# jinhan/tacotron2-vae

Hardware: AMD Instinct MI355X
Metric: mel-frames/s (train step, batch=6, 80-mel) (higher is better)
Workload: dtype f32; 1 GPU; configs[1]: Tacotron2-VAE fp32 train step (fwd+loss+bwd+clip+Adam), B=6/GPU fixed shape T_in=84 T_out=400, dropout on, random-init seed 1234; step_mode=hip-graph replay, decoder_forward=persistent, decoder_backward=persistent, startup_steps=43, global_batch=6, parallelism=dp1

## Files before the change

include/t2vae.h:

```cpp
#ifndef T2VAE_H
#define T2VAE_H
#include <stdint.h>
#ifdef __cplusplus
extern "C" {
#endif

#define T2V_OK 0
#define T2V_ERR_DIMS -1
#define T2V_ERR_ARG -2
#define T2V_ERR_LAUNCH -3

const char* t2v_version(void);
const char* t2v_last_error(void);

void t2v_set_phase_profile(unsigned long long* dev_buf32);
int t2v_stamp(unsigned long long* dev_buf, int slot, void* stream);
int t2v_debug_spin(int wgs, int microseconds, void* stream);

typedef struct t2v_step_params {
    uint64_t epoch;
    float lr;
    float bc1;
    float bc2s;
    float kl_weight;
// ... 81 lines not shown
    float* GCUM;
    float* DV;
} t2v_dec_bwd_bufs;

int t2v_attn_bwd_slices(int T_in);

int t2v_decoder_train_bwd(const t2v_dec_weights* w, const t2v_dec_train_bufs* s,
                          const t2v_dec_bwd_bufs* g, int B, int T_in, int T_out,
                          float p_att, float p_dec, uint64_t seed, void* stream);

int t2v_decoder_replay_bwd_kernels(const t2v_dec_weights* w, const t2v_dec_train_bufs* s,
                                   const t2v_dec_bwd_bufs* g, int B, int T_in, int T_out,
                                   float p_att, float p_dec, uint64_t seed, int kernel_mask, void* stream);

int t2v_attn_wgrad_scratch_floats(void);
int t2v_attn_wgrad(const float* dpre, const float* al, const float* acum, const float* loc_conv,
                   const float* loc_dense, float* part_scratch, float* d_loc_dense, float* d_loc_conv,
                   int B, int T_in, int T, void* stream);


int t2v_decoder_bwd_persist_supported(int B, int T_in);
long t2v_decoder_bwd_achain_scratch_floats(int B, int T_in, int T_out);
int t2v_decoder_bwd_persist_slices(int T_in);
typedef struct t2v_achain_dw {
    float* planes;
    float* d_w_ih; int ld_ih;
    float* d_w_hh; int ld_hh;
    int accumulate;
    int tile_cap;
} t2v_achain_dw;
long t2v_decoder_bwd_achain_dw_offset(int B, int T_in, int T_out);
int t2v_decoder_bwd_achain(const t2v_dec_train_persist_weights* w, const t2v_achain_dw* dw, const t2v_dec_train_bufs* s,
                           const float* dHC, float* DGA, float* DGD, float* DCTX, float* DV, float* DQP, float* scratch,
                           uint32_t* err_word, int B, int T_in, int T_out, float p_att, float p_dec, uint64_t seed,
                           void* stream);
int t2v_decoder_bwd_persist16_supported(int B, int T_in);
int t2v_decoder_bwd_persist16_slices(int T_in);
int t2v_decoder_bwd_persist16_fits(int B, int T_in, int T_out);
long t2v_decoder_bwd_persist16_scratch_floats(int B, int T_in, int T_out);
long t2v_decoder_bwd_persist16_dq_offset(int B, int T_in, int T_out);
int t2v_decoder_bwd_persistent16(const t2v_dec_train_persist_weights* w, const t2v_dec_train_bufs* s, const float* dHC,
                                 float* DGA, float* DGD, float* DCTX, float* DV, float* DQP, float* scratch,
                                 uint32_t* err_word, int B, int T_in, int T_out, float p_att, float p_dec, uint64_t seed,
                                 void* stream);
int t2v_decoder_bwd_persistent16_prepare(float* DQP, float* scratch, uint32_t* err_word, int B, int T_in, int T_out, void* stream);
int t2v_decoder_bwd_persistent16_prepared(const t2v_dec_train_persist_weights* w, const t2v_dec_train_bufs* s, const float* dHC,
                                          float* DGA, float* DGD, float* DCTX, float* DV, float* DQP, float* scratch,
                                          uint32_t* err_word, int B, int T_in, int T_out, float p_att, float p_dec, uint64_t seed,
                                          void* stream);

long t2v_decoder_bwd_achain_dq_offset(int B, int T_in, int T_out);
int t2v_decoder_bwd_achain_prepare(const t2v_dec_train_bufs* s, float* DQP, float* scratch, uint32_t* err_word, int B, int T_in,
                                   int T_out, float p_att, float p_dec, uint64_t seed, void* stream);
int t2v_decoder_bwd_achain_prepared(const t2v_dec_train_persist_weights* w, const t2v_achain_dw* dw, const t2v_dec_train_bufs* s,
                           const float* dHC, float* DGA, float* DGD, float* DCTX, float* DV, float* DQP, float* scratch,
                           uint32_t* err_word, int B, int T_in, int T_out, float p_att, float p_dec, uint64_t seed,
                           void* stream);

typedef struct t2v_dec_infer_bufs {
    const float* memory;
    const float* pm;
    const int32_t* lengths;
    float* XS; float* CA; float* CD; float* QP; float* AL; float* ACUM;
    float* PRE;
    float* MEL;
    float* GATE;
    int32_t* stop_flag;
    const float* prenet_w1;
    const float* proj_w;
    const float* proj_b;
} t2v_dec_infer_bufs;

int t2v_decoder_infer_steps(const t2v_dec_weights* w, const t2v_dec_infer_bufs* s, int B, int T_in,
                            int t_begin, int t_end, float gate_threshold, float p_prenet,
                            int external_prenet, uint64_t seed, void* stream);

typedef struct t2v_dec_persist_weights {
    const float* w_ih_att; const float* w_hh_att;
    const float* w_ih_dec; const float* w_hh_dec;
    const float* bias_att; const float* bias_dec;
    const float* wq;
    const float* wcomb;
    const float* v;
    const float* proj_w;
    const float* proj_b;
    const float* prenet_w1;
} t2v_dec_persist_weights;
typedef struct t2v_dec_persist_bufs {
    const float* memory;
    const float* pm;
    const int32_t* lengths;
    const float* pre_first;
    float* MEL;
    float* GATE;
    float* AL;
    int32_t* stop_flag;
    void* exchange;
    uint32_t* err_word;
} t2v_dec_persist_bufs;
long t2v_decoder_persist_scratch_floats(int B, int t_end);
int t2v_decoder_persist_supported(int B, int T_in);
int t2v_decoder_infer_persistent(const t2v_dec_persist_weights* w, const t2v_dec_persist_bufs* s, int B, int T_in,
                                 int t_end, float gate_threshold, float p_prenet, uint64_t seed, void* stream);

typedef struct t2v_dec_items {
    int32_t* stop_item;
    const uint64_t* item_seeds;
} t2v_dec_items;
int t2v_decoder_infer_steps_items(const t2v_dec_weights* w, const t2v_dec_infer_bufs* s, int B, int T_in,
                                  int t_begin, int t_end, float gate_threshold, float p_prenet,
                                  int external_prenet, uint64_t seed, const t2v_dec_items* items, void* stream);
int t2v_decoder_infer_persistent_items(const t2v_dec_persist_weights* w, const t2v_dec_persist_bufs* s, int B, int T_in,
                                       int t_end, float gate_threshold, float p_prenet, uint64_t seed,
                                       const t2v_dec_items* items, void* stream);

int t2v_conv1d_stat_blocks(int B, int T, int Cin, int Cout, int KS);
int t2v_conv1d_stat_blocks_bf16(int B, int T, int Cin, int Cout, int KS);
int t2v_conv1d_fwd(const float* W, const float* X, const float* bias, float* Y, float* stat_part,
                   int B, int Cin, int T, int Cout, int KS, void* stream);
int t2v_conv1d_dw_scratch_floats(int B, int Cin, int T, int Cout, int KS);
int t2v_conv1d_bwd(const float* W, const float* X, const float* dY, float* dX, float* dW, float* Wt_scratch,
                   float* dw_scratch,
                   int B, int Cin, int T, int Cout, int KS, void* stream);
int t2v_conv1d_flip_weights(const float* const* W, float* const* Wt, const int* Cout, const int* Cin, int KS, int n,
                            void* stream);
int t2v_conv1d_fwd_bf16(const float* W, const float* X, const float* bias, float* Y, float* stat_part,
                        void* Wp_scratch, int B, int Cin, int T, int Cout, int KS, void* stream);
int t2v_conv1d_bwd_bf16(const float* W, const float* X, const float* dY, float* dX, float* dW,
                        void* Wp_scratch, float* dw_scratch, int B, int Cin, int T, int Cout, int KS, void* stream);

int t2v_bn_act_fwd(const float* y, const float* stat_part, int nblk, const float* gamma, const float* beta,
                   float* running_mean, float* running_var, float* mean_out, float* rstd_out, float* out,
                   int B, int M, int T, int act, int training, float p_drop, float momentum, float eps,
                   uint64_t seed, uint32_t rng_stream, uint32_t rng_t, void* stream);
int t2v_bn_act_fwd_len(const float* y, const float* gamma, const float* beta, const float* running_mean,
                       const float* running_var, float* out, const int32_t* lengths, int B, int M, int T, int act, float eps,
                       void* stream);
int t2v_bn_act_bwd(const float* y, const float* dout, const float* mean, const float* rstd,
                   const float* gamma, const float* beta, float* dy, float* dgamma, float* dbeta,
                   float* dconv_bias, int B, int M, int T, int act, float p_drop, uint64_t seed,
                   uint32_t rng_stream, uint32_t rng_t, void* stream);
int t2v_bn_act_bwd_eval(const float* y, const float* dout, const float* mean, const float* rstd,
                   const float* gamma, const float* beta, float* dy, float* dgamma, float* dbeta,
                   float* dconv_bias, int B, int M, int T, int act, float p_drop, uint64_t seed,
                   uint32_t rng_stream, uint32_t rng_t, void* stream);

int t2v_embedding_fwd(const long long* ids, const float* W, float* out_bct, int B, int T, int C, int n_symbols, void* stream);
int t2v_embedding_bwd(const long long* ids, const float* dy_bct, float* dW, int B, int T, int C, int n_symbols, void* stream);

int t2v_gemm_epilogue_bwd(const float* dy, const float* y, float* out, size_t n, float scale, void* stream);

long t2v_colsum_scratch_floats(long M, long N);
int t2v_colsum(const float* A, long lda, long M, long N, float* scratch, float* out, void* stream);

int t2v_mask_outputs(float* mel, float* mel_post, float* gate, const int* lengths, int B, int C, int T, float gate_fill,
                     void* stream);
int t2v_mask_time(const float* x, float* out, const int32_t* lengths, int B, int C, int T, void* stream);
int t2v_reparam_fwd(const float* eps, const float* mu, const float* logvar, float* z, long n, void* stream);
int t2v_reparam_bwd(const float* dz, const float* eps, const float* logvar, float* dlogvar, long n, void* stream);
int t2v_gather_words(const void* const* src, void* const* dst, int n, void* stream);
int t2v_concat2_rows(const float* a, long lda, int na, const float* b, long ldb, int nb, float* out, long rows, void* stream);

int t2v_bilstm_fwd(const float* gx, const float* whh, const int32_t* lengths, float* y, float* gates,
                   float* cells, float* hx_scratch, uint32_t* sync3, int B, int T, void* stream);
int t2v_bilstm_bwd(const float* whh, const int32_t* lengths, const float* dy, const float* gates,
                   const float* cells, float* dg, float* dgx_scratch, uint32_t* sync3, int B, int T,
                   void* stream);

int t2v_gemm_f32(const float* A, long sAi, long sAk, const float* B, long sBj, long sBk, const float* bias,
                 float* C, int ldc, int M, int N, int K, int relu, int accumulate, float p_drop,
                 uint64_t seed, uint32_t rng_stream, uint32_t rng_t, void* stream);
long t2v_gemm_splitk_scratch_floats(int M, int N, int K);
int t2v_gemm_f32_splitk(const float* A, long sAi, long sAk, const float* B, long sBj, long sBk, const float* bias,
                        float* C, int ldc, int M, int N, int K, int relu, int accumulate, float p_drop,
                        uint64_t seed, uint32_t rng_stream, uint32_t rng_t, float* splitk_scratch, void* stream);

int t2v_gemm_f32_set_mode(int x3);

typedef struct t2v_gemm_group {
    const float* A;
    long sAi;
    long sAk;
    int nb;
    const float* B[3];
    long sBj[3];
    long sBk[3];
    int N[3];
    float* C[3];
    int ldc[3];
} t2v_gemm_group;
long t2v_gemm_f32_grouped_scratch_floats(const t2v_gemm_group* groups, int ngroups, int M, int K);
int t2v_gemm_f32_grouped(const t2v_gemm_group* groups, int ngroups, int M, int K, int accumulate, float* scratch, void* stream);
long t2v_gemm_f32_grouped_group_offset(const t2v_gemm_group* groups, int ngroups, int M, int K, int g);
int t2v_gemm_f32_grouped_handed(const t2v_gemm_group* groups, int ngroups, int M, int K, int accumulate, float* scratch, int handed,
                                const uint32_t* done_ctr, int done_cap, void* stream);
long t2v_gemm_bf16_grouped_scratch_floats(const t2v_gemm_group* groups, int ngroups, int M, int K);
int t2v_gemm_bf16_grouped(const t2v_gemm_group* groups, int ngroups, int M, int K, int accumulate, float* scratch, void* stream);

int t2v_conv1d_x3_set_mode(int mode);
int t2v_conv1d_takes_x3(int B, int Cin, int T, int Cout, int KS, int bf16);

int t2v_gemm_f32_batched(const float* A, long sAb, long sAi, long sAk, const float* B, long sBb, long sBj, long sBk,
                         float* C, long sCb, int ldc, int nbatch, int M, int N, int K, void* stream);
int t2v_gemm_bf16(const float* A, long sAi, long sAk, const float* B, long sBj, long sBk, const float* bias,
                  float* C, int ldc, int M, int N, int K, int relu, int accumulate, float p_drop,
                  uint64_t seed, uint32_t rng_stream, uint32_t rng_t, void* stream);
long t2v_gemm_bf16_splitk_scratch_floats(int M, int N, int K);
int t2v_gemm_bf16_splitk(const float* A, long sAi, long sAk, const float* B, long sBj, long sBk, const float* bias,
                         float* C, int ldc, int M, int N, int K, int relu, int accumulate, float p_drop,
                         uint64_t seed, uint32_t rng_stream, uint32_t rng_t, float* splitk_scratch, void* stream);


int t2v_conv2d_s2_fwd(const float* x, const float* w, const float* bias, float* y, int B, int Cx, int H, int W,
                      int Cout, int coord, void* stream);
int t2v_conv2d_s2_dw_scratch_floats(int B, int Cx, int H, int W, int Cout, int coord);
int t2v_conv2d_s2_bwd(const float* x, const float* w, const float* dy, float* dx, float* dw, float* dw_scratch,
                      int B, int Cx, int H, int W, int Cout, int coord, void* stream);

long t2v_conv2d_s2_gemm_scratch_floats(int B, int Cx, int H, int W, int Cout, int coord);
int t2v_conv2d_s2_fwd_gemm(const float* x, const float* w, const float* bias, float* y, float* scratch, int B, int Cx, int H, int W,
                           int Cout, int coord, void* stream);
int t2v_conv2d_s2_bwd_gemm(const float* x, const float* w, const float* dy, float* dx, float* dw, float* scratch, int B, int Cx, int H,
                           int W, int Cout, int coord, void* stream);
int t2v_gru_fwd(const float* gi, const float* whh, const float* bhh, float* hs, float* gsave, float* xchg,
                uint32_t* sync2, int B, int T, void* stream);
int t2v_gru_bwd(const float* whh, const float* hs, const float* gsave, const float* dh_last, float* dgi,
                float* dgh, float* xchg, uint32_t* sync2, int B, int T, void* stream);

int t2v_conv2d_s2_fwd_ragged(const float* x, const float* w, const float* bias, float* y, const int32_t* hlen, int B, int Cx,
                             int H, int W, int Cout, int coord, int x_tstride, void* stream);
long t2v_conv2d_s2_gemm_ragged_scratch_floats(int B, int Cx, int H, int W, int Cout, int coord);
int t2v_conv2d_s2_fwd_gemm_ragged(const float* x, const float* w, const float* bias, float* y, float* scratch,
                                  const int32_t* hlen, int B, int Cx, int H, int W, int Cout, int coord, int x_tstride,
                                  void* stream);
int t2v_gru_fwd_len(const float* gi, const float* whh, const float* bhh, float* hs, float* gsave, float* xchg,
                    uint32_t* sync2, const int32_t* steps, float* h_last, int B, int T, void* stream);
int t2v_loss_fwd_bwd(const float* mel, const float* post, const float* mel_t, const float* gate,
                     const float* gate_t, const float* mu, const float* logvar, float* dmel, float* dpost,
                     float* dgate, float* dmu, float* dlogvar, float* part192, float* out4, uint32_t* ticket,
                     uint64_t n_mel, int n_gate, int n_lat, float kl_weight, void* stream);

int t2v_clip_adam_step(float* params, float* grads, float* exp_avg, float* exp_avg_sq, uint64_t n,
                       float lr, float beta1, float beta2, float eps, float weight_decay,
                       float max_norm, float inv_world, float bc1, float bc2, float* partials,
                       float* norm_out, void* stream);
int t2v_clip_adam_step_guarded(float* params, float* grads, float* exp_avg, float* exp_avg_sq, uint64_t n,
                               float lr, float beta1, float beta2, float eps, float weight_decay,
                               float max_norm, float inv_world, float bc1, float bc2, float* partials,
                               float* norm_out, const uint32_t* guard, int guard_n, void* stream);

int t2v_mel_frontend(const float* wav_f32, const int16_t* wav_i16, const int64_t* n_samples, int B,
                     int n_stride, float scale, int n_fft, int hop, int n_mel, const float* window,
                     const float* tw512, const float* tw1024, const int32_t* mel_start,
                     const int32_t* mel_len, const float* mel_w, int maxw, float* mel_out,
                     int t_stride, void* stream);

int t2v_stft_polar(const float* wav, const int64_t* n_samples, int B, int n_stride, int n_fft, int hop,
                   const float* window, const float* tw512, const float* tw1024, float* mag, float* phase,
                   int t_stride, void* stream);
size_t t2v_istft_scratch_bytes(int B, int t_stride);
int t2v_istft(const float* mag, const float* phase, const int32_t* n_frames, int B, int t_stride, int n_fft, int hop,
              const float* window, const float* tw512, const float* tw1024, void* scratch, float* out, int out_stride,
              void* stream);
size_t t2v_griffin_lim_scratch_bytes(int B, int t_stride);
int t2v_griffin_lim(const float* mag, const float* angles, const int32_t* n_frames, int B, int t_stride, int n_fft,
                    int hop, int n_iters, const float* window, const float* tw512, const float* tw1024, void* scratch,
                    float* out, int out_stride, void* stream);
int t2v_mel_to_magnitude(const float* mel, const float* pinv_basis, const int32_t* n_frames, int B, int t_stride,
                         int n_mel, float* mag, void* stream);

#define T2V_DTW_MAX_FRAMES 2048
size_t t2v_mel_dtw_scratch_bytes(int B, int tx_max, int ty_max);
int t2v_mel_dtw(const float* X, const int32_t* nx, int x_stride, const float* Y, const int32_t* ny, int y_stride,
                int B, int n_mel, float* dist, void* scratch, void* stream);

#define T2V_TSNE_MAX_POINTS 16384
#define T2V_TSNE_EXAG_ITERS 250
size_t t2v_tsne_scratch_bytes(int N, int D);
int t2v_tsne_affinities(const float* X, int N, int D, float perplexity, float* P, void* scratch, void* stream);
int t2v_tsne_gradient(const float* P, const float* Y, int N, float exaggeration, float* grad, float* kl_or_null,
                      void* scratch, void* stream);
int t2v_tsne_run(const float* P, float* Y_inout, int N, int n_iter, float learning_rate, float* kl_trace, void* scratch,
                 void* stream);

#ifdef __cplusplus
}
#endif
#endif
```

tacotron2-vae_amd/csrc/colsum.hip:

```cpp
#include "t2v_common.h"
#include "t2v_kernels.h"
#include "t2v_coop.h"

#define CS_COLS 64
#define CS_ROWL 16

static int colsum_slices_(long M, long N) {
    const long cb = (N + CS_COLS - 1) / CS_COLS;
    long rs = (1024 + cb - 1) / cb;
    const long cap = (M + CS_ROWL - 1) / CS_ROWL;
    if (rs > cap) rs = cap;
    if (rs > 64) rs = 64;
    return rs < 1 ? 1 : (int)rs;
}

template <bool VEC>
__global__ __launch_bounds__(256) void k_colsum(const float* __restrict__ A, long lda, int M, int N, int rows_per_slice,
                                                float* __restrict__ dst, float* __restrict__ out, unsigned* __restrict__ ctr) {
    const int tid = threadIdx.x, cq = tid & 15, rl = tid >> 4;
    const int j0 = blockIdx.x * CS_COLS + 4 * cq;
    const int r0 = blockIdx.y * rows_per_slice, r1 = min(M, r0 + rows_per_slice);
    __shared__ float4 red[CS_ROWL][16];
    float4 acc = {0.f, 0.f, 0.f, 0.f};
    if (VEC) {
        if (j0 < N) {
            const float* p = A + (size_t)j0;
            int i = r0 + rl;
            for (; i + 3 * CS_ROWL < r1; i += 4 * CS_ROWL) {
                const float4 v0 = *(const float4*)(p + (size_t)i * lda);
                const float4 v1 = *(const float4*)(p + (size_t)(i + CS_ROWL) * lda);
                const float4 v2 = *(const float4*)(p + (size_t)(i + 2 * CS_ROWL) * lda);
                const float4 v3 = *(const float4*)(p + (size_t)(i + 3 * CS_ROWL) * lda);
                acc.x += (v0.x + v1.x) + (v2.x + v3.x); acc.y += (v0.y + v1.y) + (v2.y + v3.y);
                acc.z += (v0.z + v1.z) + (v2.z + v3.z); acc.w += (v0.w + v1.w) + (v2.w + v3.w);
            }
            for (; i < r1; i += CS_ROWL) {
                const float4 v = *(const float4*)(p + (size_t)i * lda);
                acc.x += v.x; acc.y += v.y; acc.z += v.z; acc.w += v.w;
            }
        }
    } else {
        for (int i = r0 + rl; i < r1; i += CS_ROWL) {
            const float* p = A + (size_t)i * lda + j0;
            if (j0 + 0 < N) acc.x += p[0];
            if (j0 + 1 < N) acc.y += p[1];
            if (j0 + 2 < N) acc.z += p[2];
            if (j0 + 3 < N) acc.w += p[3];
        }
    }
    red[rl][cq] = acc;
    __syncthreads();
    if (tid < CS_COLS) {
        const int j = blockIdx.x * CS_COLS + tid;
        const float* rf = (const float*)&red[0][0];
        float s = 0.f;
#pragma unroll
        for (int r = 0; r < CS_ROWL; ++r) s += rf[r * CS_COLS + tid];
        if (j < N) { if (ctr) st_sc1(dst + (size_t)blockIdx.y * N + j, s); else dst[(size_t)blockIdx.y * N + j] = s; }
    }
    if (!ctr) return;
    __shared__ unsigned last_;
    asm volatile("s_waitcnt vmcnt(0)" ::: "memory");
    __syncthreads();
    if (tid == 0) last_ = __hip_atomic_fetch_add(ctr + blockIdx.x, 1u, __ATOMIC_RELAXED, __HIP_MEMORY_SCOPE_AGENT) == gridDim.y - 1 ? 1u : 0u;
    __syncthreads();
    if (!last_) return;
    if (tid == 0) __hip_atomic_store(ctr + blockIdx.x, 0u, __ATOMIC_RELAXED, __HIP_MEMORY_SCOPE_AGENT);
    if (tid < CS_COLS) {
        const int j = blockIdx.x * CS_COLS + tid;
        if (j < N) {
            float s = 0.f;
            const int RS = (int)gridDim.y;
            for (int r = 0; r < RS; ++r) s += ld_sc1(dst + (size_t)r * N + j);
            out[j] = s;
        }
    }
}

extern "C" long t2v_colsum_scratch_floats(long M, long N) {
    if (M < 1 || N < 1) return 0;
    const int rs = colsum_slices_(M, N);
    return rs > 1 ? (long)rs * N : 0;
}

extern "C" int t2v_colsum(const float* A, long lda, long M, long N, float* scratch, float* out, void* stream_) {
    hipStream_t stream = (hipStream_t)stream_;
    if (!A || !out || M < 1 || N < 1 || lda < N || M > 0x7fffffff || N > 0x7fffffff) return T2V_ERR_ARG;
    const int rs = colsum_slices_(M, N);
    if (rs > 1 && !scratch) return T2V_ERR_ARG;
    const int rows = (int)((M + rs - 1) / rs);
    const bool vec = !(N & 3) && !(lda & 3) && !((uintptr_t)A & 15);
    const dim3 grid((unsigned)((N + CS_COLS - 1) / CS_COLS), (unsigned)rs);
    float* dst = rs > 1 ? scratch : out;
    unsigned* ctr = nullptr;
    if (rs > 1) {
        if (grid.x > 4096) return T2V_ERR_ARG;
        ctr = t2v_arrival_counters((int)grid.x);
        if (!ctr) return T2V_ERR_LAUNCH;
    }
    if (vec) k_colsum<true><<<grid, 256, 0, stream>>>(A, lda, (int)M, (int)N, rows, dst, out, ctr);
    else k_colsum<false><<<grid, 256, 0, stream>>>(A, lda, (int)M, (int)N, rows, dst, out, ctr);
    return t2v_check_launch();
}
```

tacotron2-vae_amd/csrc/gemm.hip:

```cpp
#include <stdlib.h>
#include <string.h>
#include "t2v_common.h"
#include "t2v_kernels.h"
#include "t2v_coop.h"
#include "t2v_x3.h"
#include "t2v_xchg.h"
#include "gemm_x3_tile.h"

#define GM_BM 64
#define GM_BN 64
#define GM_BK 32

struct GemmArgs {
    const float* A; const float* B; const float* bias; float* C;
    long sAi, sAk, sBj, sBk;
    int M, N, K, ldc;
    int relu, accumulate;
    float p_drop; uint64_t seed; uint32_t rng_stream, rng_t;
    const t2v_step_params* step;
    int kz_chunk;
    float* part;
    int nbatch;
    long sAb, sBb, sCb;
    int nsub;
    long sAs, sBs;
    int bias_row;
    unsigned* tile_ctr;
};

__device__ __forceinline__ void gemm64_epilogue(const GemmArgs& a, f32x16& acc, int i0, int j0, int wm, int wn, int lane, int tid) {
    const int j = j0 + 32 * wn + (lane & 31);
    if (a.part) {
        if (j < a.N) {
#pragma unroll
            for (int r = 0; r < 16; ++r) {
                const int i = i0 + 32 * wm + (r & 3) + 8 * (r >> 2) + 4 * (lane >> 5);
                if (i < a.M) st_sc1(a.part + ((size_t)blockIdx.z * a.M + i) * a.N + j, acc[r]);
            }
        }
        __shared__ unsigned last_;
        asm volatile("s_waitcnt vmcnt(0)" ::: "memory");
        __syncthreads();
        unsigned* ctr = a.tile_ctr + blockIdx.y * gridDim.x + blockIdx.x;
        if (tid == 0) last_ = __hip_atomic_fetch_add(ctr, 1u, __ATOMIC_RELAXED, __HIP_MEMORY_SCOPE_AGENT) == gridDim.z - 1 ? 1u : 0u;
        __syncthreads();
        if (!last_) return;
        if (tid == 0) __hip_atomic_store(ctr, 0u, __ATOMIC_RELAXED, __HIP_MEMORY_SCOPE_AGENT);
        const int nz = (int)gridDim.z;
#pragma unroll
        for (int r = 0; r < 16; ++r) acc[r] = 0.f;
        if (j < a.N) {
            for (int z0 = 0; z0 < nz; z0 += 4) {
                float v[4][16];
#pragma unroll
                for (int u = 0; u < 4; ++u) {
                    const int z = min(z0 + u, nz - 1);
#pragma unroll
                    for (int r = 0; r < 16; ++r) {
                        const int i = min(i0 + 32 * wm + (r & 3) + 8 * (r >> 2) + 4 * (lane >> 5), a.M - 1);
                        v[u][r] = ld_sc1(a.part + ((size_t)z * a.M + i) * a.N + j);
                    }
                }
#pragma unroll
                for (int u = 0; u < 4; ++u)
                    if (z0 + u < nz) {
#pragma unroll
                        for (int r = 0; r < 16; ++r) acc[r] += v[u][r];
                    }
            }
        }
    }
    if (j < a.N) {
        const float bv = (a.bias && !a.bias_row) ? a.bias[j] : 0.f;
#pragma unroll
        for (int r = 0; r < 16; ++r) {
            const int i = i0 + 32 * wm + (r & 3) + 8 * (r >> 2) + 4 * (lane >> 5);
            if (i < a.M) {
                const size_t idx = (size_t)i * a.ldc + j;
                float v = acc[r] + ((a.bias && a.bias_row) ? a.bias[i] : bv);
                if (a.accumulate) v += a.C[idx];
                if (a.relu) v = fmaxf(v, 0.f);
                if (a.p_drop > 0.f) v *= t2v_drop_scale(t2v_step_seed(a.seed, a.step), a.rng_stream, a.rng_t, (uint32_t)idx, a.p_drop);
                a.C[idx] = v;
            }
        }
    }
}

template <bool A_KC, bool B_KC>
__global__ __launch_bounds__(256) void k_gemm_f32(GemmArgs a) {
    __shared__ float As[2][GM_BK][GM_BM + 1];
    __shared__ float Bs[2][GM_BK][GM_BN + 1];
    const int tid = threadIdx.x, wave = tid >> 6, lane = tid & 63;
    const int wm = wave >> 1, wn = wave & 1;
    const int i0 = blockIdx.y * GM_BM, j0 = blockIdx.x * GM_BN;
    if (a.nbatch > 1) {
        const int zb = a.nsub > 1 ? blockIdx.z / a.nsub : blockIdx.z, zs = a.nsub > 1 ? blockIdx.z - zb * a.nsub : 0;
        a.A += zb * a.sAb + zs * a.sAs; a.B += zb * a.sBb + zs * a.sBs; a.C += blockIdx.z * a.sCb;
    }
    const int kbeg = a.kz_chunk ? blockIdx.z * a.kz_chunk : 0, kend = a.kz_chunk ? min(a.K, kbeg + a.kz_chunk) : a.K;
    constexpr int NE = GM_BM * GM_BK / 256;
    float ra[NE], rb[NE];
    auto load_tiles = [&](int k0) {
#pragma unroll
        for (int e8 = 0; e8 < NE; ++e8) {
            const int e = tid + 256 * e8;
            {
                const int kk = A_KC ? (e & (GM_BK - 1)) : (e >> 6);
                const int ii = A_KC ? (e >> 5) : (e & (GM_BM - 1));
                const int i = i0 + ii, k = k0 + kk;
                ra[e8] = (i < a.M && k < kend) ? a.A[(long)i * a.sAi + (long)k * a.sAk] : 0.f;
            }
            {
                const int kk = B_KC ? (e & (GM_BK - 1)) : (e >> 6);
                const int jj = B_KC ? (e >> 5) : (e & (GM_BN - 1));
                const int j = j0 + jj, k = k0 + kk;
                rb[e8] = (j < a.N && k < kend) ? a.B[(long)j * a.sBj + (long)k * a.sBk] : 0.f;
            }
        }
    };
    auto store_tiles = [&](int buf) {
#pragma unroll
        for (int e8 = 0; e8 < NE; ++e8) {
            const int e = tid + 256 * e8;
            if (A_KC) As[buf][e & (GM_BK - 1)][e >> 5] = ra[e8]; else As[buf][e >> 6][e & (GM_BM - 1)] = ra[e8];
            if (B_KC) Bs[buf][e & (GM_BK - 1)][e >> 5] = rb[e8]; else Bs[buf][e >> 6][e & (GM_BN - 1)] = rb[e8];
        }
    };
    f32x16 acc;
#pragma unroll
    for (int r = 0; r < 16; ++r) acc[r] = 0.f;
    const int nkt = (kend - kbeg + GM_BK - 1) / GM_BK;
    load_tiles(kbeg);
    store_tiles(0);
    __syncthreads();
    const int ai = 32 * wm + (lane & 31), bj = 32 * wn + (lane & 31), kh = lane >> 5;
    for (int kt = 0; kt < nkt; ++kt) {
        const int buf = kt & 1;
        if (kt + 1 < nkt) load_tiles(kbeg + (kt + 1) * GM_BK);
#pragma unroll
        for (int s = 0; s < GM_BK / 2; ++s)
            acc = __builtin_amdgcn_mfma_f32_32x32x2f32(As[buf][2 * s + kh][ai], Bs[buf][2 * s + kh][bj], acc, 0, 0, 0);
        if (kt + 1 < nkt) store_tiles(buf ^ 1);
        __syncthreads();
    }
    gemm64_epilogue(a, acc, i0, j0, wm, wn, lane, tid);
}

#include <atomic>
#define GM_CTR_RING (1 << 16)
unsigned* t2v_arrival_counters(int tiles) {
    static unsigned* ring = nullptr;
    static std::atomic<unsigned> pos{0};
    static std::atomic<int> state{0};
    if (tiles > GM_CTR_RING) return nullptr;
    int st = state.load(std::memory_order_acquire);
    if (st != 2) {
        int expect = 0;
        if (state.compare_exchange_strong(expect, 1)) {
            unsigned* p = nullptr;
            if (hipMalloc((void**)&p, GM_CTR_RING * sizeof(unsigned)) != hipSuccess || hipMemset(p, 0, GM_CTR_RING * sizeof(unsigned)) != hipSuccess
                || hipDeviceSynchronize() != hipSuccess) { state.store(0); return nullptr; }
            ring = p;
            state.store(2, std::memory_order_release);
        } else {
            while (state.load(std::memory_order_acquire) == 1) { }
            if (state.load() != 2) return nullptr;
        }
    }
    unsigned at = pos.fetch_add((unsigned)tiles);
    at %= GM_CTR_RING;
    if (at + (unsigned)tiles > GM_CTR_RING) {
        pos.store((unsigned)tiles);
        at = 0;
    }
    return ring + at;
}
static int gemm_splits(int M, int N, int K) {
    const long tiles = (long)((M + GM_BM - 1) / GM_BM) * ((N + GM_BN - 1) / GM_BN);
    static const int wide = getenv("T2V_GEMM_SPLIT_POLICY") ? atoi(getenv("T2V_GEMM_SPLIT_POLICY")) : 1;
    if (wide) {
        if (tiles > 256 || K < 8 * GM_BK) return 1;
        long ns2 = (512 + tiles - 1) / tiles;
        const long maxk2 = K / (4 * GM_BK);
        if (ns2 > maxk2) ns2 = maxk2;
        if (ns2 > 32) ns2 = 32;
        return ns2 < 2 ? 1 : (int)ns2;
    }
    if (tiles >= 256 || K < 16 * GM_BK) return 1;
    long ns = 512 / tiles;
    const long maxk = K / (8 * GM_BK);
    if (ns > maxk) ns = maxk;
    if (ns > 32) ns = 32;
    return ns < 2 ? 1 : (int)ns;
}
static bool gemm_x3_shape_ok(int M, int N, int K);
static long gemm_x3_scratch_floats(int M, int N, int K, int np);
static int gemm_x3_mode();
extern "C" long t2v_gemm_splitk_scratch_floats(int M, int N, int K) {
    if (M < 1 || N < 1 || K < 1) return 0;
    if (gemm_x3_mode() && gemm_x3_shape_ok(M, N, K)) return gemm_x3_scratch_floats(M, N, K, 3);
    const int ns = gemm_splits(M, N, K);
    return ns > 1 ? (long)ns * M * N : 0;
}

#define GB_BM 128
#define GB_BK 32
#define GB_LD 160
template <bool A_KC, bool B_KC, int BN>
__global__ __launch_bounds__(256) void k_gemm_f32_big(GemmArgs a) {
    constexpr int NY = BN / 64;
    constexpr int NA = GB_BM * GB_BK / 4 / 256;
    constexpr int NB = BN * GB_BK / 4 / 256;
    constexpr int KQ = GB_BK / 4;
    __shared__ __attribute__((aligned(16))) float As[2][GB_BK][GB_LD];
    __shared__ __attribute__((aligned(16))) float Bs[2][GB_BK][BN + 32];
    const int tid = threadIdx.x, wave = tid >> 6, lane = tid & 63;
    const int wm = wave >> 1, wn = wave & 1;
    int by_ = blockIdx.y, bx_ = blockIdx.x;
    {
        const int nb = gridDim.x * gridDim.y, bid = blockIdx.y * gridDim.x + blockIdx.x;
        const int q = nb >> 3, r = nb & 7, xcd = bid & 7, idx = bid >> 3;
        const int lin = (xcd < r ? xcd * (q + 1) : r * (q + 1) + (xcd - r) * q) + idx;
        by_ = lin / gridDim.x;
        bx_ = lin - by_ * gridDim.x;
    }
    const int i0 = by_ * GB_BM, j0 = bx_ * BN;
    float4 ra[NA], rb[NB];
    auto load_tiles = [&](int k0) {
#pragma unroll
        for (int e = 0; e < NA; ++e) {
            if (A_KC) {
                const int i = min(i0 + tid / KQ + (256 / KQ) * e, a.M - 1), k = min(k0 + 4 * (tid % KQ), a.K - 4);
                ra[e] = *(const float4*)(a.A + (long)i * a.sAi + k);
            } else {
                const int k = min(k0 + (tid >> 5) + 8 * e, a.K - 1), i = min(i0 + 4 * (tid & 31), a.M - 4);
                ra[e] = *(const float4*)(a.A + (long)k * a.sAk + i);
            }
        }
#pragma unroll
        for (int e = 0; e < NB; ++e) {
            if (B_KC) {
                const int j = min(j0 + tid / KQ + (256 / KQ) * e, a.N - 1), k = min(k0 + 4 * (tid % KQ), a.K - 4);
                rb[e] = *(const float4*)(a.B + (long)j * a.sBj + k);
            } else {
                constexpr int RQ = BN / 4;
                const int k = min(k0 + tid / RQ + (256 / RQ) * e, a.K - 1), j = min(j0 + 4 * (tid % RQ), a.N - 4);
                rb[e] = *(const float4*)(a.B + (long)k * a.sBk + j);
            }
        }
    };
    auto store_tiles = [&](int buf, int k0) {
#pragma unroll
        for (int e = 0; e < NA; ++e) {
            if (A_KC) {
                const int m = tid / KQ + (256 / KQ) * e, kk = 4 * (tid % KQ);
                const float z = k0 + kk < a.K ? 1.f : 0.f;
                As[buf][kk + 0][m] = ra[e].x * z; As[buf][kk + 1][m] = ra[e].y * z;
                As[buf][kk + 2][m] = ra[e].z * z; As[buf][kk + 3][m] = ra[e].w * z;
            } else {
                const int kk = (tid >> 5) + 8 * e;
                const float z = k0 + kk < a.K ? 1.f : 0.f;
                *(float4*)&As[buf][kk][4 * (tid & 31)] = make_float4(ra[e].x * z, ra[e].y * z, ra[e].z * z, ra[e].w * z);
            }
        }
#pragma unroll
        for (int e = 0; e < NB; ++e) {
            if (B_KC) {
                const int n = tid / KQ + (256 / KQ) * e, kk = 4 * (tid % KQ);
                const float z = k0 + kk < a.K ? 1.f : 0.f;
                Bs[buf][kk + 0][n] = rb[e].x * z; Bs[buf][kk + 1][n] = rb[e].y * z;
                Bs[buf][kk + 2][n] = rb[e].z * z; Bs[buf][kk + 3][n] = rb[e].w * z;
            } else {
                constexpr int RQ = BN / 4;
                const int kk = tid / RQ + (256 / RQ) * e;
                const float z = k0 + kk < a.K ? 1.f : 0.f;
                *(float4*)&Bs[buf][kk][4 * (tid % RQ)] = make_float4(rb[e].x * z, rb[e].y * z, rb[e].z * z, rb[e].w * z);
            }
        }
    };
    f32x16 acc[2][NY];
#pragma unroll
    for (int x = 0; x < 2; ++x)
#pragma unroll
        for (int y = 0; y < NY; ++y)
#pragma unroll
            for (int r = 0; r < 16; ++r) acc[x][y][r] = 0.f;
    const int nkt = (a.K + GB_BK - 1) / GB_BK;
    load_tiles(0);
    store_tiles(0, 0);
    __syncthreads();
    const int am = 64 * wm + (lane & 31), bn = (BN / 2) * wn + (lane & 31), kh = lane >> 5;
    for (int kt = 0; kt < nkt; ++kt) {
        const int buf = kt & 1;
        if (kt + 1 < nkt) load_tiles((kt + 1) * GB_BK);
#pragma unroll
        for (int h = 0; h < 2; ++h) {
            float av[GB_BK / 4][2], bw[GB_BK / 4][NY];
#pragma unroll
// ... 549 lines not shown
__global__ __launch_bounds__(256) void k_epilogue_bwd(const float4* __restrict__ dy, const float4* __restrict__ y,
                                                      float4* __restrict__ out, size_t n4, float scale) {
    const size_t i = (size_t)blockIdx.x * 256 + threadIdx.x;
    if (i >= n4) return;
    const float4 g = dy[i], v = y[i];
    float4 o;
    o.x = v.x != 0.f ? g.x * scale : 0.f; o.y = v.y != 0.f ? g.y * scale : 0.f;
    o.z = v.z != 0.f ? g.z * scale : 0.f; o.w = v.w != 0.f ? g.w * scale : 0.f;
    out[i] = o;
}
__global__ __launch_bounds__(256) void k_epilogue_bwd_tail(const float* __restrict__ dy, const float* __restrict__ y,
                                                           float* __restrict__ out, size_t lo, size_t n, float scale) {
    const size_t i = lo + threadIdx.x;
    if (i < n) out[i] = y[i] != 0.f ? dy[i] * scale : 0.f;
}

extern "C" int t2v_gemm_epilogue_bwd(const float* dy, const float* y, float* out, size_t n, float scale, void* stream_) {
    hipStream_t stream = (hipStream_t)stream_;
    if (!dy || !y || !out || n < 1) return T2V_ERR_ARG;
    if (((uintptr_t)dy | (uintptr_t)y | (uintptr_t)out) & 15) return T2V_ERR_ARG;
    const size_t n4 = n / 4;
    if (n4) k_epilogue_bwd<<<(unsigned)((n4 + 255) / 256), 256, 0, stream>>>((const float4*)dy, (const float4*)y, (float4*)out, n4, scale);
    if (n & 3) k_epilogue_bwd_tail<<<1, 256, 0, stream>>>(dy, y, out, 4 * n4, n, scale);
    return t2v_check_launch();
}

extern "C" int t2v_gemm_f32(const float* A, long sAi, long sAk, const float* B, long sBj, long sBk, const float* bias,
                            float* C, int ldc, int M, int N, int K, int relu, int accumulate, float p_drop,
                            uint64_t seed, uint32_t rng_stream, uint32_t rng_t, void* stream_);
static int gemm_bf16_impl(const float* A, long sAi, long sAk, const float* B, long sBj, long sBk, const float* bias,
                          float* C, int ldc, int M, int N, int K, int relu, int accumulate, float p_drop,
                          uint64_t seed, uint32_t rng_stream, uint32_t rng_t, float* splitk_scratch, void* stream_);
extern "C" int t2v_gemm_bf16(const float* A, long sAi, long sAk, const float* B, long sBj, long sBk, const float* bias,
                             float* C, int ldc, int M, int N, int K, int relu, int accumulate, float p_drop,
                             uint64_t seed, uint32_t rng_stream, uint32_t rng_t, void* stream_) {
    return gemm_bf16_impl(A, sAi, sAk, B, sBj, sBk, bias, C, ldc, M, N, K, relu, accumulate, p_drop, seed, rng_stream, rng_t, nullptr, stream_);
}
extern "C" int t2v_gemm_bf16_splitk(const float* A, long sAi, long sAk, const float* B, long sBj, long sBk, const float* bias,
                                    float* C, int ldc, int M, int N, int K, int relu, int accumulate, float p_drop,
                                    uint64_t seed, uint32_t rng_stream, uint32_t rng_t, float* splitk_scratch, void* stream_) {
    return gemm_bf16_impl(A, sAi, sAk, B, sBj, sBk, bias, C, ldc, M, N, K, relu, accumulate, p_drop, seed, rng_stream, rng_t, splitk_scratch, stream_);
}
static int gemm_bf16_impl(const float* A, long sAi, long sAk, const float* B, long sBj, long sBk, const float* bias,
                          float* C, int ldc, int M, int N, int K, int relu, int accumulate, float p_drop,
                          uint64_t seed, uint32_t rng_stream, uint32_t rng_t, float* splitk_scratch, void* stream_) {
    hipStream_t stream = (hipStream_t)stream_;
    if (!A || !B || !C || M < 1 || N < 1 || K < 1 || ldc < N) return T2V_ERR_ARG;
    GemmArgs a;
    a.A = A; a.B = B; a.bias = bias; a.C = C; a.sAi = sAi; a.sAk = sAk; a.sBj = sBj; a.sBk = sBk;
    a.M = M; a.N = N; a.K = K; a.ldc = ldc; a.relu = relu; a.accumulate = accumulate;
    a.p_drop = p_drop; a.seed = seed; a.rng_stream = rng_stream; a.rng_t = rng_t; a.step = t2v_step_for(stream);
    a.kz_chunk = 0; a.part = nullptr; a.nbatch = 1; a.sAb = a.sBb = a.sCb = 0; a.nsub = 1; a.sAs = a.sBs = 0; a.bias_row = 0; a.tile_ctr = nullptr;
    if (splitk_scratch && !((uintptr_t)splitk_scratch & 15) && gemm_bf16_planes_ok(M, N, K))
        return gemm_x3_run(a, splitk_scratch, stream, 1);
    bool big_akc = false, big_bkc = false;
    if (gemm_bf16_big_ok(a, &big_akc, &big_bkc)) {
        const int ns = splitk_scratch ? gemm_bf16_big_splits(M, N, K) : 1;
        dim3 gb((N + GBB_BN - 1) / GBB_BN, (M + GBB_BM - 1) / GBB_BM, ns);
        if (ns > 1) {
            const int tiles_k = (K + GBB_BK - 1) / GBB_BK;
            a.kz_chunk = ((tiles_k + ns - 1) / ns) * GBB_BK;
            gb.z = (unsigned)((K + a.kz_chunk - 1) / a.kz_chunk);
            a.part = splitk_scratch;
            a.tile_ctr = t2v_arrival_counters((int)(gb.x * gb.y));
            if (!a.tile_ctr) return T2V_ERR_LAUNCH;
            if (gb.z < 2) { a.kz_chunk = 0; a.part = nullptr; a.tile_ctr = nullptr; gb.z = 1; }
        }
        if (big_akc && big_bkc) k_gemm_bf16_big_rr<true, true><<<gb, 256, 0, stream>>>(a);
        else if (big_akc) k_gemm_bf16_big_rr<true, false><<<gb, 256, 0, stream>>>(a);
        else if (big_bkc) k_gemm_bf16_big_rr<false, true><<<gb, 256, 0, stream>>>(a);
        else k_gemm_bf16_big_rr<false, false><<<gb, 256, 0, stream>>>(a);
        return t2v_check_launch();
    }
    if (gemm_big_ok(a))
        return t2v_gemm_f32(A, sAi, sAk, B, sBj, sBk, bias, C, ldc, M, N, K, relu, accumulate, p_drop, seed, rng_stream, rng_t, stream_);
    const int ns = splitk_scratch ? gemm_splits(M, N, K) : 1;
    dim3 grid((N + GM_BN - 1) / GM_BN, (M + GM_BM - 1) / GM_BM, ns);
    if (ns > 1) {
        const int tiles_k = (K + GM_BK - 1) / GM_BK;
        a.kz_chunk = ((tiles_k + ns - 1) / ns) * GM_BK;
        grid.z = (unsigned)((K + a.kz_chunk - 1) / a.kz_chunk);
        a.part = splitk_scratch;
        a.tile_ctr = t2v_arrival_counters((int)(grid.x * grid.y));
        if (!a.tile_ctr) return T2V_ERR_LAUNCH;
        if (grid.z < 2) { a.kz_chunk = 0; a.part = nullptr; a.tile_ctr = nullptr; grid.z = 1; }
    }
    const bool akc = sAk == 1, bkc = sBk == 1;
    if (akc && bkc) k_gemm_bf16<true, true><<<grid, 256, 0, stream>>>(a);
    else if (akc) k_gemm_bf16<true, false><<<grid, 256, 0, stream>>>(a);
    else if (bkc) k_gemm_bf16<false, true><<<grid, 256, 0, stream>>>(a);
    else k_gemm_bf16<false, false><<<grid, 256, 0, stream>>>(a);
    return t2v_check_launch();
}

static int gemm_f32_impl(const float* A, long sAi, long sAk, const float* B, long sBj, long sBk, const float* bias,
                         float* C, int ldc, int M, int N, int K, int relu, int accumulate, float p_drop,
                         uint64_t seed, uint32_t rng_stream, uint32_t rng_t, float* splitk_scratch, void* stream_);
extern "C" int t2v_gemm_f32(const float* A, long sAi, long sAk, const float* B, long sBj, long sBk, const float* bias,
                            float* C, int ldc, int M, int N, int K, int relu, int accumulate, float p_drop,
                            uint64_t seed, uint32_t rng_stream, uint32_t rng_t, void* stream_) {
    return gemm_f32_impl(A, sAi, sAk, B, sBj, sBk, bias, C, ldc, M, N, K, relu, accumulate, p_drop, seed, rng_stream, rng_t,
                         nullptr, stream_);
}
extern "C" int t2v_gemm_f32_splitk(const float* A, long sAi, long sAk, const float* B, long sBj, long sBk, const float* bias,
                                   float* C, int ldc, int M, int N, int K, int relu, int accumulate, float p_drop,
                                   uint64_t seed, uint32_t rng_stream, uint32_t rng_t, float* splitk_scratch, void* stream_) {
    return gemm_f32_impl(A, sAi, sAk, B, sBj, sBk, bias, C, ldc, M, N, K, relu, accumulate, p_drop, seed, rng_stream, rng_t,
                         splitk_scratch, stream_);
}
static int gemm_f32_impl(const float* A, long sAi, long sAk, const float* B, long sBj, long sBk, const float* bias,
                         float* C, int ldc, int M, int N, int K, int relu, int accumulate, float p_drop,
                         uint64_t seed, uint32_t rng_stream, uint32_t rng_t, float* splitk_scratch, void* stream_) {
    hipStream_t stream = (hipStream_t)stream_;
    if (!A || !B || !C || M < 1 || N < 1 || K < 1 || ldc < N) return T2V_ERR_ARG;
    GemmArgs a;
    a.A = A; a.B = B; a.bias = bias; a.C = C; a.sAi = sAi; a.sAk = sAk; a.sBj = sBj; a.sBk = sBk;
    a.M = M; a.N = N; a.K = K; a.ldc = ldc; a.relu = relu; a.accumulate = accumulate;
    a.p_drop = p_drop; a.seed = seed; a.rng_stream = rng_stream; a.rng_t = rng_t; a.step = t2v_step_for(stream);
    a.kz_chunk = 0; a.part = nullptr; a.nbatch = 1; a.sAb = a.sBb = a.sCb = 0; a.nsub = 1; a.sAs = a.sBs = 0; a.bias_row = 0; a.tile_ctr = nullptr;
    const bool akc = sAk == 1, bkc = sBk == 1;
    if (splitk_scratch && gemm_x3_mode() && gemm_x3_shape_ok(M, N, K) && !((uintptr_t)splitk_scratch & 15))
        return gemm_x3_run(a, splitk_scratch, stream);
    if (gemm_big_ok(a)) {
        static const int narrow = getenv("T2V_GEMM_NARROW") ? atoi(getenv("T2V_GEMM_NARROW")) : 0;
        const bool wide = !narrow && gemm_big_waste(M, N, 128) <= gemm_big_waste(M, N, 64) + 1e-6;
        const int BN = wide ? 128 : 64;
        dim3 gb((N + BN - 1) / BN, (M + GB_BM - 1) / GB_BM);
#define T2V_BIG(AK, BK)                                                             \
        if (wide) k_gemm_f32_big<AK, BK, 128><<<gb, 256, 0, stream>>>(a);           \
        else k_gemm_f32_big<AK, BK, 64><<<gb, 256, 0, stream>>>(a)
        if (akc && bkc) { T2V_BIG(true, true); }
        else if (akc) { T2V_BIG(true, false); }
        else if (bkc) { T2V_BIG(false, true); }
        else { T2V_BIG(false, false); }
#undef T2V_BIG
        return t2v_check_launch();
    }
    const int ns = splitk_scratch ? gemm_splits(M, N, K) : 1;
    dim3 grid((N + GM_BN - 1) / GM_BN, (M + GM_BM - 1) / GM_BM, ns);
    if (ns > 1) {
        const int tiles_k = (K + GM_BK - 1) / GM_BK;
        a.kz_chunk = ((tiles_k + ns - 1) / ns) * GM_BK;
        a.part = splitk_scratch;
        a.tile_ctr = t2v_arrival_counters((int)(grid.x * grid.y));
        if (!a.tile_ctr) return T2V_ERR_LAUNCH;
    }
    if (akc && bkc) k_gemm_f32<true, true><<<grid, 256, 0, stream>>>(a);
    else if (akc) k_gemm_f32<true, false><<<grid, 256, 0, stream>>>(a);
    else if (bkc) k_gemm_f32<false, true><<<grid, 256, 0, stream>>>(a);
    else k_gemm_f32<false, false><<<grid, 256, 0, stream>>>(a);
    return t2v_check_launch();
}

int t2v_gemm_f32_batched_ex(const float* A, long sAb, long sAs, long sAi, long sAk, const float* B, long sBb, long sBs, long sBj, long sBk,
                            const float* bias_row, float* C, long sCb, int ldc, int nbatch, int nsub, int M, int N, int K, hipStream_t stream) {
    if (!A || !B || !C || nbatch < 1 || nsub < 1 || (long)nbatch * nsub > 65535 || M < 1 || N < 1 || K < 1 || ldc < N) return T2V_ERR_ARG;
    GemmArgs a;
    a.A = A; a.B = B; a.bias = bias_row; a.C = C; a.sAi = sAi; a.sAk = sAk; a.sBj = sBj; a.sBk = sBk;
    a.M = M; a.N = N; a.K = K; a.ldc = ldc; a.relu = 0; a.accumulate = 0;
    a.p_drop = 0.f; a.seed = 0; a.rng_stream = 0; a.rng_t = 0; a.step = t2v_step_for(stream);
    a.kz_chunk = 0; a.part = nullptr; a.nbatch = nbatch * nsub > 1 ? nbatch * nsub : 1; a.sAb = sAb; a.sBb = sBb; a.sCb = sCb;
    a.nsub = nsub; a.sAs = sAs; a.sBs = sBs; a.bias_row = bias_row ? 1 : 0; a.tile_ctr = nullptr;
    const bool akc = sAk == 1, bkc = sBk == 1;
    dim3 grid((N + GM_BN - 1) / GM_BN, (M + GM_BM - 1) / GM_BM, nbatch * nsub);
    if (akc && bkc) k_gemm_f32<true, true><<<grid, 256, 0, stream>>>(a);
    else if (akc) k_gemm_f32<true, false><<<grid, 256, 0, stream>>>(a);
    else if (bkc) k_gemm_f32<false, true><<<grid, 256, 0, stream>>>(a);
    else k_gemm_f32<false, false><<<grid, 256, 0, stream>>>(a);
    return t2v_check_launch();
}
extern "C" int t2v_gemm_f32_batched(const float* A, long sAb, long sAi, long sAk, const float* B, long sBb, long sBj, long sBk,
                                    float* C, long sCb, int ldc, int nbatch, int M, int N, int K, void* stream_) {
    return t2v_gemm_f32_batched_ex(A, sAb, 0, sAi, sAk, B, sBb, 0, sBj, sBk, nullptr, C, sCb, ldc, nbatch, 1, M, N, K, (hipStream_t)stream_);
}
```

tacotron2-vae_amd/csrc/refenc.hip:

```cpp
#include "t2v_common.h"
#include "t2v_kernels.h"
#include "t2v_coop.h"

struct Conv2dArgs {
    const float* x;
    const float* w;
    const float* bias;
    const float* dy;
    float* y;
    float* dbias;
    int B, Cx, H, W, Cout, Ho, Wo, coord;
};

__device__ __forceinline__ float refenc_in(const Conv2dArgs& a, int b, int c, int h, int w) {
    if (h < 0 || h >= a.H || w < 0 || w >= a.W) return 0.f;
    if (c < a.Cx) return a.x[(((size_t)b * a.Cx + c) * a.H + h) * a.W + w];
    const float xx = (float)h / (float)(a.H - 1) * 2.f - 1.f;
    const float yy = (float)w / (float)(a.W - 1) * 2.f - 1.f;
    const int k = c - a.Cx;
    if (k == 0) return xx;
    if (k == 1) return yy;
    return sqrtf((xx - 0.5f) * (xx - 0.5f) + (yy - 0.5f) * (yy - 0.5f));
}


struct RaggedSrc {
    const int* hlen;
    int tstride;
};

__device__ __forceinline__ float refenc_in_ragged(const Conv2dArgs& a, const RaggedSrc& r, int b, int c, int h, int w) {
    const int hb = min(r.hlen[b], a.H);
    if (h < 0 || h >= hb || w < 0 || w >= a.W) return 0.f;
    if (c < a.Cx) {
        if (r.tstride > 0) {
            const int f = h * a.W + w;
            return a.x[((size_t)b * a.W + f / hb) * r.tstride + f % hb];
        }
        return a.x[(((size_t)b * a.Cx + c) * a.H + h) * a.W + w];
    }
    const float xx = (float)h / (float)(hb - 1) * 2.f - 1.f;
    const float yy = (float)w / (float)(a.W - 1) * 2.f - 1.f;
    const int k = c - a.Cx;
    if (k == 0) return xx;
    if (k == 1) return yy;
    return sqrtf((xx - 0.5f) * (xx - 0.5f) + (yy - 0.5f) * (yy - 0.5f));
}

#define GRU_H 256
#define GRU_G (3 * GRU_H)
#define GRU_NW 8
#define GRU_UNITS (GRU_H / GRU_NW)

struct GruArgs {
    const float* gi;
    const float* whh;
    const float* bhh;
    float* hs;
    float* gsave;
    const float* dh_last;
    float* dgi;
    float* dgh;
    float* xchg;
    unsigned* sync;
    int B, T;
};

#define REFENC_RAGGED 0
#include "refenc_fwd.inc"
#undef REFENC_RAGGED
#define REFENC_RAGGED 1
#include "refenc_fwd.inc"
#undef REFENC_RAGGED

__global__ __launch_bounds__(256) void k_conv2d_s2_dx(Conv2dArgs a) {
    __shared__ float wsh[128 * 9];
    const int Cin = a.Cx + (a.coord ? 3 : 0);
    const int b = blockIdx.y / a.Cx, c = blockIdx.y % a.Cx;
    for (int i = threadIdx.x; i < a.Cout * 9; i += 256) wsh[i] = a.w[((size_t)(i / 9) * Cin + c) * 9 + (i % 9)];
    __syncthreads();
    const int r = blockIdx.x * 256 + threadIdx.x;
    if (r >= a.H * a.W) return;
    const int h = r / a.W, w = r - h * a.W;
    float acc = 0.f;
    for (int kh = 0; kh < 3; ++kh) {
        const int hh = h + 1 - kh;
        if (hh < 0 || (hh & 1)) continue;
        const int ho = hh >> 1;
        if (ho >= a.Ho) continue;
        for (int kw = 0; kw < 3; ++kw) {
            const int ww = w + 1 - kw;
            if (ww < 0 || (ww & 1)) continue;
            const int wo = ww >> 1;
            if (wo >= a.Wo) continue;
            const float* dyp = a.dy + ((size_t)b * a.Cout * a.Ho + ho) * a.Wo + wo;
            const int tap = kh * 3 + kw;
#pragma unroll 4
            for (int co = 0; co < a.Cout; ++co) acc = fmaf(wsh[co * 9 + tap], dyp[(size_t)co * a.Ho * a.Wo], acc);
        }
    }
    a.y[((size_t)b * a.Cx + c) * a.H * a.W + r] = acc;
}

__global__ __launch_bounds__(256) void k_conv2d_s2_dw(Conv2dArgs a, float* part, int chunk) {
    __shared__ float red[4][9];
    const int Cin = a.Cx + (a.coord ? 3 : 0);
    const int co = blockIdx.x / Cin, c = blockIdx.x % Cin;
    const int tid = threadIdx.x;
    float acc[9];
#pragma unroll
    for (int k = 0; k < 9; ++k) acc[k] = 0.f;
    const int per = a.Ho * a.Wo;
    const int lo = blockIdx.y * chunk, hi = min(a.B * per, lo + chunk);
    for (int i = lo + tid; i < hi; i += 256) {
        const int b = i / per, r = i - b * per, ho = r / a.Wo, wo = r - ho * a.Wo;
        const float g = a.dy[((size_t)b * a.Cout + co) * per + r];
#pragma unroll
        for (int kh = 0; kh < 3; ++kh)
#pragma unroll
            for (int kw = 0; kw < 3; ++kw) acc[kh * 3 + kw] = fmaf(g, refenc_in(a, b, c, 2 * ho - 1 + kh, 2 * wo - 1 + kw), acc[kh * 3 + kw]);
    }
#pragma unroll
    for (int k = 0; k < 9; ++k) {
        const float v = wave_sum(acc[k]);
        if ((tid & 63) == 0) red[tid >> 6][k] = v;
    }
    __syncthreads();
    if (tid < 9) {
        float* dst = gridDim.y > 1 ? part + (size_t)blockIdx.y * a.Cout * Cin * 9 : a.y;
        dst[((size_t)co * Cin + c) * 9 + tid] = (red[0][tid] + red[1][tid]) + (red[2][tid] + red[3][tid]);
    }
}

__global__ void k_conv2d_s2_dw_reduce(const float* __restrict__ part, float* __restrict__ dw, int n, int nsplit) {
    const int i = blockIdx.x * blockDim.x + threadIdx.x;
    if (i >= n) return;
    float s = 0.f;
    int k = 0;
    for (; k + 8 <= nsplit; k += 8) {
        float v[8];
#pragma unroll
        for (int u = 0; u < 8; ++u) v[u] = part[(size_t)(k + u) * n + i];
#pragma unroll
        for (int u = 0; u < 8; ++u) s += v[u];
    }
    for (; k < nsplit; ++k) s += part[(size_t)k * n + i];
    dw[i] = s;
}

static inline int conv2d_dw_splits(int pairs, int positions) {
    int ns = 1;
    while (pairs * ns < 2048 && positions / (2 * ns) >= 1024 && ns < 64) ns *= 2;
    return ns;
}
extern "C" int t2v_conv2d_s2_dw_scratch_floats(int B, int Cx, int H, int W, int Cout, int coord) {
    const int Cin = Cx + (coord ? 3 : 0), Ho = (H - 1) / 2 + 1, Wo = (W - 1) / 2 + 1;
    const int ns = conv2d_dw_splits(Cout * Cin, B * Ho * Wo);
    return ns > 1 ? ns * Cout * Cin * 9 : 0;
}

extern "C" int t2v_conv2d_s2_fwd(const float* x, const float* w, const float* bias, float* y, int B, int Cx, int H, int W,
                                 int Cout, int coord, void* stream_) {
    hipStream_t stream = (hipStream_t)stream_;
    if (!x || !w || !y || B < 1 || Cx < 1 || H < 1 || W < 1 || Cout < 1) return T2V_ERR_ARG;
    if (coord && (H < 2 || W < 2)) return T2V_ERR_ARG;
    Conv2dArgs a;
    a.x = x; a.w = w; a.bias = bias; a.dy = nullptr; a.y = y; a.dbias = nullptr;
    a.B = B; a.Cx = Cx; a.H = H; a.W = W; a.Cout = Cout; a.Ho = (H - 1) / 2 + 1; a.Wo = (W - 1) / 2 + 1; a.coord = coord;
    if (Cx + (coord ? 3 : 0) > 131) return T2V_ERR_DIMS;
    k_conv2d_s2_fwd<<<dim3((a.Ho * a.Wo + 255) / 256, B * Cout), 256, 0, stream>>>(a);
    return t2v_check_launch();
}

extern "C" int t2v_conv2d_s2_bwd(const float* x, const float* w, const float* dy, float* dx, float* dw,
                                 float* dw_scratch, int B, int Cx, int H, int W, int Cout, int coord, void* stream_) {
    hipStream_t stream = (hipStream_t)stream_;
    if (!x || !w || !dy || !dw || B < 1) return T2V_ERR_ARG;
    Conv2dArgs a;
    a.x = x; a.w = w; a.bias = nullptr; a.dy = dy; a.dbias = nullptr;
    a.B = B; a.Cx = Cx; a.H = H; a.W = W; a.Cout = Cout; a.Ho = (H - 1) / 2 + 1; a.Wo = (W - 1) / 2 + 1; a.coord = coord;
    if (dx) {
        a.y = dx;
        if (Cout > 128) return T2V_ERR_DIMS;
        k_conv2d_s2_dx<<<dim3((H * W + 255) / 256, B * Cx), 256, 0, stream>>>(a);
    }
    a.y = dw;
    const int Cin = Cx + (coord ? 3 : 0), npos = B * a.Ho * a.Wo;
    const int ns = conv2d_dw_splits(Cout * Cin, npos);
    if (ns > 1 && !dw_scratch) return T2V_ERR_ARG;
    const int chunk = (npos + ns - 1) / ns;
    k_conv2d_s2_dw<<<dim3(Cout * Cin, ns), 256, 0, stream>>>(a, dw_scratch, chunk);
    if (ns > 1) k_conv2d_s2_dw_reduce<<<(Cout * Cin * 9 + 255) / 256, 256, 0, stream>>>(dw_scratch, dw, Cout * Cin * 9, ns);
    return t2v_check_launch();
}

int t2v_gemm_f32_batched_ex(const float* A, long sAb, long sAs, long sAi, long sAk, const float* B, long sBb, long sBs, long sBj, long sBk,
                            const float* bias_row, float* C, long sCb, int ldc, int nbatch, int nsub, int M, int N, int K, hipStream_t stream);

__global__ __launch_bounds__(256) void k_col2im_s2(Conv2dArgs a, const float* __restrict__ dcol) {
    const int Cin = a.Cx + (a.coord ? 3 : 0), K = Cin * 9, P = a.Ho * a.Wo;
    const size_t n = (size_t)a.B * a.Cx * a.H * a.W;
    for (size_t e = (size_t)blockIdx.x * 256 + threadIdx.x; e < n; e += (size_t)gridDim.x * 256) {
        const int w = (int)(e % a.W);
        size_t r = e / a.W;
        const int h = (int)(r % a.H);
        r /= a.H;
        const int c = (int)(r % a.Cx), b = (int)(r / a.Cx);
        float acc = 0.f;
#pragma unroll
        for (int kh = 0; kh < 3; ++kh) {
            const int hh = h + 1 - kh;
            if (hh < 0 || (hh & 1) || (hh >> 1) >= a.Ho) continue;
#pragma unroll
            for (int kw = 0; kw < 3; ++kw) {
                const int ww = w + 1 - kw;
                if (ww < 0 || (ww & 1) || (ww >> 1) >= a.Wo) continue;
                acc += dcol[((size_t)b * P + (size_t)(hh >> 1) * a.Wo + (ww >> 1)) * K + c * 9 + kh * 3 + kw];
            }
        }
        a.y[e] = acc;
    }
}
static inline int conv2d_gemm_chunks(int P) {
    int ns = 1;
    while (ns < 16 && P % (2 * ns) == 0 && P / (2 * ns) >= 64) ns *= 2;
    return ns;
}
extern "C" long t2v_conv2d_s2_gemm_scratch_floats(int B, int Cx, int H, int W, int Cout, int coord) {
    if (B < 1 || Cx < 1 || H < 1 || W < 1 || Cout < 1) return 0;
    const long Cin = Cx + (coord ? 3 : 0), K = Cin * 9, P = (long)((H - 1) / 2 + 1) * ((W - 1) / 2 + 1);
    return B * P * K + (long)B * conv2d_gemm_chunks((int)P) * Cout * K;
}
static Conv2dArgs conv2d_args(const float* x, const float* w, int B, int Cx, int H, int W, int Cout, int coord) {
    Conv2dArgs a;
    a.x = x; a.w = w; a.bias = nullptr; a.dy = nullptr; a.y = nullptr; a.dbias = nullptr;
    a.B = B; a.Cx = Cx; a.H = H; a.W = W; a.Cout = Cout; a.Ho = (H - 1) / 2 + 1; a.Wo = (W - 1) / 2 + 1; a.coord = coord;
    return a;
}
extern "C" int t2v_conv2d_s2_fwd_gemm(const float* x, const float* w, const float* bias, float* y, float* scratch, int B, int Cx, int H,
                                      int W, int Cout, int coord, void* stream_) {
    hipStream_t stream = (hipStream_t)stream_;
    if (!x || !w || !y || !scratch || B < 1 || Cx < 1 || H < 1 || W < 1 || Cout < 1) return T2V_ERR_ARG;
    if (coord && (H < 2 || W < 2)) return T2V_ERR_ARG;
    Conv2dArgs a = conv2d_args(x, w, B, Cx, H, W, Cout, coord);
    const int K = (Cx + (coord ? 3 : 0)) * 9, P = a.Ho * a.Wo;
    const size_t n = (size_t)B * P * K;
    k_im2col_s2<<<(unsigned)((n + 255) / 256 > 8192 ? 8192 : (n + 255) / 256), 256, 0, stream>>>(a, scratch);
    return t2v_gemm_f32_batched_ex(w, 0, 0, K, 1, scratch, (long)P * K, 0, K, 1, bias, y, (long)Cout * P, P, B, 1, Cout, P, K, stream);
}
static int conv2d_ragged_check(const float* x, const float* w, const float* y, const int* hlen, int B, int Cx, int H, int W,
                               int Cout, int coord, int x_tstride) {
    if (!x || !w || !y || !hlen || B < 1 || Cx < 1 || H < 1 || W < 1 || Cout < 1 || x_tstride < 0) return T2V_ERR_ARG;
    if (coord && (H < 2 || W < 2)) return T2V_ERR_ARG;
    if (x_tstride > 0 && (Cx != 1 || x_tstride < H)) return T2V_ERR_ARG;
    if (Cx + (coord ? 3 : 0) > 131) return T2V_ERR_DIMS;
    return T2V_OK;
}
extern "C" int t2v_conv2d_s2_fwd_ragged(const float* x, const float* w, const float* bias, float* y, const int* hlen, int B, int Cx,
                                        int H, int W, int Cout, int coord, int x_tstride, void* stream_) {
    const int rc = conv2d_ragged_check(x, w, y, hlen, B, Cx, H, W, Cout, coord, x_tstride);
    if (rc != T2V_OK) return rc;
    Conv2dArgs a = conv2d_args(x, w, B, Cx, H, W, Cout, coord);
    a.bias = bias; a.y = y;
    RaggedSrc r;
    r.hlen = hlen; r.tstride = x_tstride;
    k_conv2d_s2_fwd_ragged<<<dim3((a.Ho * a.Wo + 255) / 256, B * Cout), 256, 0, (hipStream_t)stream_>>>(a, r);
    return t2v_check_launch();
}
extern "C" long t2v_conv2d_s2_gemm_ragged_scratch_floats(int B, int Cx, int H, int W, int Cout, int coord) {
    if (B < 1 || Cx < 1 || H < 1 || W < 1 || Cout < 1) return 0;
    const long Cin = Cx + (coord ? 3 : 0), P = (long)((H - 1) / 2 + 1) * ((W - 1) / 2 + 1);
    return B * P * Cin * 9;
}
extern "C" int t2v_conv2d_s2_fwd_gemm_ragged(const float* x, const float* w, const float* bias, float* y, float* scratch,
                                             const int* hlen, int B, int Cx, int H, int W, int Cout, int coord, int x_tstride,
                                             void* stream_) {
    hipStream_t stream = (hipStream_t)stream_;
    int rc = conv2d_ragged_check(x, w, y, hlen, B, Cx, H, W, Cout, coord, x_tstride);
    if (rc != T2V_OK) return rc;
    if (!scratch) return T2V_ERR_ARG;
    Conv2dArgs a = conv2d_args(x, w, B, Cx, H, W, Cout, coord);
    RaggedSrc r;
    r.hlen = hlen; r.tstride = x_tstride;
    const int K = (Cx + (coord ? 3 : 0)) * 9, P = a.Ho * a.Wo;
    const size_t n = (size_t)B * P * K;
    k_im2col_s2_ragged<<<(unsigned)((n + 255) / 256 > 8192 ? 8192 : (n + 255) / 256), 256, 0, stream>>>(a, r, scratch);
    return t2v_gemm_f32_batched_ex(w, 0, 0, K, 1, scratch, (long)P * K, 0, K, 1, bias, y, (long)Cout * P, P, B, 1, Cout, P, K, stream);
}

extern "C" int t2v_conv2d_s2_bwd_gemm(const float* x, const float* w, const float* dy, float* dx, float* dw, float* scratch, int B, int Cx,
                                      int H, int W, int Cout, int coord, void* stream_) {
    hipStream_t stream = (hipStream_t)stream_;
    if (!x || !w || !dy || !dw || !scratch || B < 1) return T2V_ERR_ARG;
    Conv2dArgs a = conv2d_args(x, w, B, Cx, H, W, Cout, coord);
    const int K = (Cx + (coord ? 3 : 0)) * 9, P = a.Ho * a.Wo;
    float* col = scratch;
    float* part = scratch + (size_t)B * P * K;
    const int ns = conv2d_gemm_chunks(P), chunk = P / ns;
    int rc = t2v_gemm_f32_batched_ex(dy, (long)Cout * P, chunk, P, 1, col, (long)P * K, (long)chunk * K, 1, K, nullptr, part, (long)Cout * K, K,
                                     B, ns, Cout, K, chunk, stream);
    if (rc != T2V_OK) return rc;
    k_conv2d_s2_dw_reduce<<<(Cout * K + 255) / 256, 256, 0, stream>>>(part, dw, Cout * K, B * ns);
    if (dx) {
        rc = t2v_gemm_f32_batched_ex(dy, (long)Cout * P, 0, 1, P, w, 0, 0, 1, K, nullptr, col, (long)P * K, K, B, 1, P, K, Cout, stream);
        if (rc != T2V_OK) return rc;
        a.y = dx;
        const size_t n = (size_t)B * Cx * H * W;
        k_col2im_s2<<<(unsigned)((n + 255) / 256 > 8192 ? 8192 : (n + 255) / 256), 256, 0, stream>>>(a, col);
    }
    return t2v_check_launch();
}



__global__ __launch_bounds__(256) void k_gru_bwd(GruArgs a) {
    const int j = blockIdx.x, tid = threadIdx.x, wave = tid >> 6, lane = tid & 63;
    const int b = lane & 15, g = lane >> 4;
    __shared__ float dgbuf[16][GRU_G + 4];
    __shared__ f32x4 red[4][2][64];
    __shared__ float dhrec[16][GRU_UNITS + 1];
    float wreg[2][48];
#pragma unroll
    for (int tt = 0; tt < 2; ++tt) {
        const int col = j * GRU_UNITS + tt * 16 + (lane & 15);
#pragma unroll
        for (int s = 0; s < 48; ++s) wreg[tt][s] = a.whh[(size_t)(192 * wave + 4 * s + g) * GRU_H + col];
    }
    const int uu = tid & 31, U = j * GRU_UNITS + uu;
    for (int i = tid; i < 16 * GRU_UNITS; i += 256) {
        const int bb = i >> 5, u2 = i & 31;
        dhrec[bb][u2] = bb < a.B ? a.dh_last[(size_t)bb * GRU_H + j * GRU_UNITS + u2] : 0.f;
    }
    __syncthreads();

    for (int t = a.T - 1; t >= 0; --t) {
        float* dgx_w = a.xchg + (size_t)(t & 1) * 16 * GRU_G;
        float keep[2] = {0.f, 0.f};
#pragma unroll
        for (int rep = 0; rep < 2; ++rep) {
            const int bb = (tid >> 5) + 8 * rep;
            if (bb < a.B) {
                const float* sv = a.gsave + (((size_t)bb * a.T + t) * 4) * GRU_H + U;
                const float r = sv[0], z = sv[GRU_H], n = sv[2 * GRU_H], hn = sv[3 * GRU_H];
                const float hprev = a.hs[((size_t)bb * (a.T + 1) + t) * GRU_H + U];
                const float d = dhrec[bb][uu];
                const float dn = d * (1.f - z) * (1.f - n * n);
                const float dz = d * (hprev - n) * z * (1.f - z);
                const float dr = dn * hn * r * (1.f - r);
                float* gi = a.dgi + ((size_t)bb * a.T + t) * GRU_G + U;
                gi[0] = dr; gi[GRU_H] = dz; gi[2 * GRU_H] = dn;
                float* gh = a.dgh + ((size_t)bb * a.T + t) * GRU_G + U;
                gh[0] = dr; gh[GRU_H] = dz; gh[2 * GRU_H] = dn * r;
                float* x = dgx_w + (size_t)bb * GRU_G + U;
                st_sc1(x, dr); st_sc1(x + GRU_H, dz); st_sc1(x + 2 * GRU_H, dn * r);
                keep[rep] = d * z;
            }
        }
        if (t == 0) break;
        if (!group_barrier(a.sync, (unsigned)(GRU_NW * (a.T - t)), a.sync + 1)) return;
#pragma unroll
        for (int q3 = 0; q3 < 3; ++q3) {
            float dv[16];
#pragma unroll
            for (int u = 0; u < 16; ++u) dv[u] = ld_sc1(dgx_w + (size_t)min(u, a.B - 1) * GRU_G + 256 * q3 + tid);
#pragma unroll
            for (int u = 0; u < 16; ++u)
                if (u < a.B) dgbuf[u][256 * q3 + tid] = dv[u];
        }
        __syncthreads();
        f32x4 acc0 = {0.f, 0.f, 0.f, 0.f}, acc1 = {0.f, 0.f, 0.f, 0.f};
        const float* drow = &dgbuf[b][192 * wave + g];
#pragma unroll
        for (int s = 0; s < 48; ++s) {
            const float dv = drow[4 * s];
            acc0 = mfma16x4(wreg[0][s], dv, acc0);
            acc1 = mfma16x4(wreg[1][s], dv, acc1);
        }
        red[wave][0][lane] = acc0;
        red[wave][1][lane] = acc1;
        __syncthreads();
        if (wave < 2) {
            const f32x4 s4 = (red[0][wave][lane] + red[1][wave][lane]) + (red[2][wave][lane] + red[3][wave][lane]);
            if (b < a.B) {
#pragma unroll
                for (int r = 0; r < 4; ++r) dhrec[b][16 * wave + 4 * g + r] = s4[r];
            }
        }
        __syncthreads();
#pragma unroll
        for (int rep = 0; rep < 2; ++rep) {
            const int bb = (tid >> 5) + 8 * rep;
            if (bb < a.B) dhrec[bb][uu] += keep[rep];
        }
        __syncthreads();
    }
}

extern "C" int t2v_gru_fwd(const float* gi, const float* whh, const float* bhh, float* hs, float* gsave,
                           float* xchg, uint32_t* sync2, int B, int T, void* stream_) {
    hipStream_t stream = (hipStream_t)stream_;
    if (!gi || !whh || !bhh || !hs || !xchg || !sync2 || B < 1 || B > 16 || T < 1) return T2V_ERR_ARG;
    (void)hipMemsetAsync(sync2, 0, 2 * sizeof(uint32_t), stream);
    GruArgs a;
    a.gi = gi; a.whh = whh; a.bhh = bhh; a.hs = hs; a.gsave = gsave; a.dh_last = nullptr; a.dgi = nullptr; a.dgh = nullptr;
    a.xchg = xchg; a.sync = sync2; a.B = B; a.T = T;
    k_gru_fwd<<<GRU_NW, 256, 0, stream>>>(a);
    return t2v_check_launch();
}

extern "C" int t2v_gru_fwd_len(const float* gi, const float* whh, const float* bhh, float* hs, float* gsave, float* xchg,
                               uint32_t* sync2, const int* steps, float* h_last, int B, int T, void* stream_) {
    hipStream_t stream = (hipStream_t)stream_;
    if (!gi || !whh || !bhh || !hs || !xchg || !sync2 || !steps || !h_last || B < 1 || B > 16 || T < 1) return T2V_ERR_ARG;
    (void)hipMemsetAsync(sync2, 0, 2 * sizeof(uint32_t), stream);
    GruArgs a;
    a.gi = gi; a.whh = whh; a.bhh = bhh; a.hs = hs; a.gsave = gsave; a.dh_last = nullptr; a.dgi = nullptr; a.dgh = nullptr;
    a.xchg = xchg; a.sync = sync2; a.B = B; a.T = T;
    k_gru_fwd_len<<<GRU_NW, 256, 0, stream>>>(a, steps, h_last);
    return t2v_check_launch();
}

extern "C" int t2v_gru_bwd(const float* whh, const float* hs, const float* gsave, const float* dh_last, float* dgi,
                           float* dgh, float* xchg, uint32_t* sync2, int B, int T, void* stream_) {
    hipStream_t stream = (hipStream_t)stream_;
    if (!whh || !hs || !gsave || !dh_last || !dgi || !dgh || !xchg || !sync2 || B < 1 || B > 16 || T < 1)
        return T2V_ERR_ARG;
    (void)hipMemsetAsync(sync2, 0, 2 * sizeof(uint32_t), stream);
    GruArgs a;
    a.gi = nullptr; a.whh = whh; a.bhh = nullptr; a.hs = (float*)hs; a.gsave = (float*)gsave; a.dh_last = dh_last;
    a.dgi = dgi; a.dgh = dgh; a.xchg = xchg; a.sync = sync2; a.B = B; a.T = T;
    k_gru_bwd<<<GRU_NW, 256, 0, stream>>>(a);
    return t2v_check_launch();
}

struct LossArgs {
    const float* mel; const float* post; const float* mel_t; const float* gate; const float* gate_t;
    const float* mu; const float* logvar;
    float* dmel; float* dpost; float* dgate; float* dmu; float* dlogvar;
    float* part;
    float* out;
    size_t n_mel; int n_gate, n_lat, nblk;
    float klw;
    const t2v_step_params* step;
    unsigned* ticket;
};

__global__ __launch_bounds__(256) void k_loss(LossArgs a) {
    __shared__ float scr[4];
    __shared__ int last;
    const int tid = threadIdx.x;
    const float klw = a.step ? a.step->kl_weight : a.klw;
    float s_mel = 0.f, s_gate = 0.f, s_kl = 0.f;
    const float cm = 2.0f / (float)a.n_mel;
    for (size_t i = (size_t)blockIdx.x * 256 + tid; i < a.n_mel; i += (size_t)gridDim.x * 256) {
        const float t = a.mel_t[i];
        const float d0 = a.mel[i] - t, d1 = a.post[i] - t;
        s_mel = fmaf(d0, d0, s_mel);
        s_mel = fmaf(d1, d1, s_mel);
        a.dmel[i] = cm * d0;
        a.dpost[i] = cm * d1;
    }
    for (int i = blockIdx.x * 256 + tid; i < a.n_gate; i += gridDim.x * 256) {
        const float x = a.gate[i], y = a.gate_t[i];
        s_gate += fmaxf(x, 0.f) - x * y + log1pf(expf(-fabsf(x)));
        a.dgate[i] = (1.0f / (1.0f + expf(-x)) - y) / (float)a.n_gate;
// ... 50 lines not shown
```

tacotron2-vae_amd/csrc/t2v_kernels.h:

```cpp
#pragma once
#include <hip/hip_runtime.h>
#include <stdint.h>
#include <initializer_list>
#include "../../include/t2vae.h"
#include "t2v_common.h"

enum { T2V_RNG_ATT_H = 1, T2V_RNG_ATT_C = 2, T2V_RNG_DEC_H = 3, T2V_RNG_DEC_C = 4,
       T2V_RNG_PRENET0 = 5, T2V_RNG_PRENET1 = 6 };

int t2v_check_launch();
unsigned* t2v_arrival_counters(int n);
extern unsigned long long* g_t2v_prof;
const t2v_step_params* t2v_step_for(hipStream_t stream);

struct T2VZeroRegions {
    void* p[10];
    size_t bytes[10];
    int n = 0;
    void add(void* ptr, size_t nbytes) { p[n] = ptr; bytes[n] = nbytes; ++n; }
};
void t2v_zero_regions(T2VZeroRegions& z, hipStream_t stream);

__global__ void k_sentinel_fill(uint4* p, size_t n16);
void t2v_fill_sentinel(void* p, size_t n16, int grid, hipStream_t stream);
bool t2v_persist_cus_ok();
bool t2v_persist_raise_lds(std::initializer_list<const void*> kernels, bool& raised);
int t2v_persist_resident(const void* kernel, int threads, size_t lds, std::initializer_list<const void*> kernels, bool& raised);
struct LstmFwdArgs;
struct AttnFwdArgs;

typedef unsigned long long t2v_u64;
static inline size_t t2v_tcap(int T_in) { return (size_t)((T_in + 15) / 16) * 16; }
static inline size_t t2v_qp_sync_off(int B) { return (size_t)B * 256 * 128; }
static inline size_t t2v_qp_xchg_off(int B) { return t2v_qp_sync_off(B) + 64; }
static inline size_t t2v_qp_ex_off(int B) { return t2v_qp_sync_off(B) + 64 + 4096; }
#define T2V_MAX_T_IN 4096
static inline size_t t2v_qp_floats(int B, int T_in) { return t2v_qp_ex_off(B) + 2 * (size_t)B * 8 * t2v_tcap(T_in); }
static inline int t2v_attn_bwd_js(int T_in) { return T_in <= 128 ? 16 : 32; }
static inline int t2v_attn_bwd_slices_(int T_in) { const int js = t2v_attn_bwd_js(T_in); return (T_in + js - 1) / js; }
void t2v_launch_lstm_fwd(int mode, const LstmFwdArgs& a, hipStream_t stream);
void t2v_launch_attn_fwd(const AttnFwdArgs& f, int B, int T_in, hipStream_t stream);
static inline unsigned* t2v_persist_fwd_begin(const t2v_dec_train_persist_weights* w, const t2v_dec_train_bufs* s, const float* scratch,
                                              int B, int T_in, hipStream_t stream) {
    if (!w->w_ih_att || !w->w_hh_att || !w->w_ih_dec || !w->w_hh_dec || !w->bias_dec || !w->wq || !w->wcomb || !w->v || !s->gpre ||
        !s->memory || !s->pm || !s->XS || !s->CA || !s->CD || !s->QP || !s->AL || !s->ACUM)
        return nullptr;
    if ((uintptr_t)scratch & 15) return nullptr;
    unsigned* sync = (unsigned*)(s->QP + t2v_qp_sync_off(B));
    T2VZeroRegions z;
    z.add(sync, 64 * sizeof(uint32_t));
    z.add(s->XS, sizeof(float) * 2 * B * T2V_XW);
    z.add(s->CA, sizeof(float) * B * T2V_H);
    z.add(s->CD, sizeof(float) * B * T2V_H);
    z.add(s->AL, sizeof(float) * B * T_in);
    z.add(s->ACUM, sizeof(float) * B * T_in);
    t2v_zero_regions(z, stream);
    return sync;
}

#define T2V_AF_THREADS 512
#define T2V_AF_SPIN 1500000u
#define T2V_AF_MAXT 224
#define T2V_AF_MAXT_LONG 560
#define T2V_AF_NTI_LONG 5
static inline size_t t2v_attn_fwd_lds_floats(int T_in, size_t tail) {
    const size_t Tcap = t2v_tcap(T_in);
    const bool lng = T_in > T2V_AF_MAXT;
    return (lng ? 0 : 16 * 1028) + Tcap * 64 + (lng ? 0 : Tcap * 16) + 2 * (Tcap + 32) + Tcap + (lng ? T2V_CTX_PAD : 0) + T2V_H + 16 +
           32 * 16 + 8 * 64 + 32 + 32 + tail + 4;
}

struct LstmFwdArgs {
    const float4* packA;
    const float4* packD;
    int k_att;
    const float* xs_prev;
    float* xs_next;
    const float* gpre_t;
    const float* pre_t;
    const float* bias_att;
    const float* bias_dec;
    const float* ca_prev;
    float* ca_cur;
    const float* cd_prev;
    float* cd_cur;
    float* ga_t;
    float* gd_t;
    const float* wqT;
    float* qp;
    int shared_x;
    int B, t, do_att, do_dec;
    float p_att, p_dec;
    uint64_t seed;
    const t2v_step_params* step;
};

struct AttnFwdArgs {
    const float* qp;
    const float* al_prev;
    const float* acum_prev;
    float* al_cur;
    float* acum_cur;
    const float* memory;
    const float* pm;
    const int32_t* lengths;
    const float* wcomb;
    const float* v;
    float* xs_next;
    float* s_save;
    int T_in;
    unsigned long long* prof;
    t2v_u64* ex;
    unsigned* err;
    unsigned epoch;
};

struct LstmBwdArgs {
    const float4* packBD;
    const float4* packBA;
    const float* dgd_t;
    const float* dga_n;
    float* YD;
    float* YA;
    int B;
    int flip;
};

struct AttnBwdArgs {
    const float* dHC_t;
    const float* YD;
    const float* YA;
    const float* al_cur;
    const float* memory;
    const float* wcomb;
    const float* v;
    float* S_t;
    t2v_u64* DQ_t;
    float* DCTX_t;
    const float* ctx_t;
    const float* GP_in;
    float* GP_out;
    float* GC;
    float* DV;
    int T_in;
    unsigned long long* prof;
};

struct CellBwdArgs {
    const float* YD;
    const float* YA;
    const t2v_u64* DQ_t;
    int S;
    const float* wqT;
    const float* dHC_prev;
    const float* GA_t;
    const float* CA_cur;
    const float* CA_prev;
    const float* GD_p;
    const float* CD_cur;
    const float* CD_prev;
    float* DGA_t;
    float* DGD_p;
    float* DCA;
    float* DCD;
    int B, t, do_att, do_dec;
    float p_att, p_dec;
// ... 6 lines not shown
```

tacotron2-vae_amd/modules.py:

```python
import torch
from torch import nn
from torch.nn import functional as F

from CoordConv import CoordConv2d
from layers import HipLinear


class ReferenceEncoder(nn.Module):

    def __init__(self, hparams):
        super().__init__()
        filters = [1] + list(hparams.ref_enc_filters)
        K = len(hparams.ref_enc_filters)
        convs = [CoordConv2d(filters[0], filters[1], kernel_size=(3, 3), stride=(2, 2), padding=(1, 1),
                             with_r=True)]
        convs += [nn.Conv2d(filters[i], filters[i + 1], kernel_size=(3, 3), stride=(2, 2), padding=(1, 1))
                  for i in range(1, K)]
        self.convs = nn.ModuleList(convs)
        self.bns = nn.ModuleList([nn.BatchNorm2d(hparams.ref_enc_filters[i]) for i in range(K)])
        width = self.calculate_channels(hparams.n_mel_channels, 3, 2, 1, K)
        self.gru = nn.GRU(input_size=hparams.ref_enc_filters[-1] * width, hidden_size=hparams.E // 2,
                          batch_first=True)
        self.n_mels = hparams.n_mel_channels

    @staticmethod
    def calculate_channels(L, kernel_size, stride, pad, n_convs):
        for _ in range(n_convs):
            L = (L - kernel_size + 2 * pad) // stride + 1
        return L

    def forward(self, inputs, lengths=None):
        if lengths is not None:
            return self.forward_ragged(inputs, lengths)
        import t2v_hip
        n = inputs.size(0)
        out = inputs.contiguous().view(n, 1, -1, self.n_mels)
        for i, (conv, bn) in enumerate(zip(self.convs, self.bns)):
            c = conv.conv if i == 0 else conv
            if self.training:
                t2v_hip.note_bn_counter(bn.num_batches_tracked)
            out = t2v_hip.Conv2dBNReLU.apply(out, c.weight, c.bias, bn.weight, bn.bias, bn.running_mean,
                                             bn.running_var, self.training, i == 0)
        t2v_hip.flush_bn_counters()
        out = out.transpose(1, 2)
        out = out.contiguous().view(n, out.size(1), -1)
        g = self.gru
        return t2v_hip.GRULast.apply(out, g.weight_ih_l0, g.weight_hh_l0, g.bias_ih_l0, g.bias_hh_l0)

    def forward_ragged(self, inputs, lengths):
        import t2v_hip
        if self.training:
            raise RuntimeError("ReferenceEncoder: per-item lengths are an eval-mode (inference) path; call .eval() first")
        B, _, T = inputs.shape
        n = [int(x) for x in torch.as_tensor(lengths).reshape(-1).tolist()]
        if len(n) != B or min(n) < 2 or max(n) > T:
            raise ValueError("every item needs 2 <= frames <= %d, got %s (%d items)" % (T, n, B))
        layers = [((conv.conv if i == 0 else conv).weight, (conv.conv if i == 0 else conv).bias, bn.weight, bn.bias,
                   bn.running_mean, bn.running_var) for i, (conv, bn) in enumerate(zip(self.convs, self.bns))]
        g = self.gru
        with torch.no_grad():
            return t2v_hip.refenc_ragged(inputs, n, layers, (g.weight_ih_l0, g.weight_hh_l0, g.bias_ih_l0, g.bias_hh_l0))


class VAE_GST(nn.Module):
    def __init__(self, hparams):
        super().__init__()
        self.ref_encoder = ReferenceEncoder(hparams)
        self.fc1 = HipLinear(hparams.ref_enc_gru_size, hparams.z_latent_dim)
        self.fc2 = HipLinear(hparams.ref_enc_gru_size, hparams.z_latent_dim)
        self.fc3 = HipLinear(hparams.z_latent_dim, hparams.E)
        self.eps_override = None

    def reparameterize(self, mu, logvar):
        if not self.training:
            return mu
        eps = self.eps_override if self.eps_override is not None else torch.randn_like(mu)
        import t2v_hip
        return t2v_hip.Reparam.apply(eps, mu, logvar)

    def forward(self, inputs, lengths=None):
        if lengths is not None:
            with torch.no_grad():
                return self._heads(self.ref_encoder(inputs, lengths))
        return self._heads(self.ref_encoder(inputs))

    def _heads(self, enc_out):
        import t2v_hip
        lin = t2v_hip.LinearHIP.apply
        mu = lin(enc_out, self.fc1.weight, self.fc1.bias, False, 0.0, 0, 0, 0)
        logvar = lin(enc_out, self.fc2.weight, self.fc2.bias, False, 0.0, 0, 0, 0)
        z = self.reparameterize(mu, logvar)
        return lin(z, self.fc3.weight, self.fc3.bias, False, 0.0, 0, 0, 0), mu, logvar, z
```

tacotron2-vae_amd/t2v_hip.py:

```python
import collections
import ctypes as C
import os

import torch

_HERE = os.path.dirname(os.path.abspath(__file__))
_LIB_PATH = os.environ.get('T2V_LIB') or os.path.join(_HERE, 'libt2vae_hip.so')
_lib = None

H, E, PRE, A, F_LOC, KS, XW, KATT, KATT_INF, G4 = 1024, 512, 256, 128, 32, 31, 2560, 1536, 1792, 4096


class T2VHipError(RuntimeError):
    pass


class _DecWeights(C.Structure):
    _fields_ = [(n, C.c_void_p) for n in (
        'packF_att', 'packF_dec', 'packB_att', 'packB_dec', 'bias_att', 'bias_dec', 'wqT', 'wcomb', 'v')] + [
        ('packs_bf16', C.c_int32)]


class _DecTrainBufs(C.Structure):
    _fields_ = [(n, C.c_void_p) for n in (
        'gpre', 'memory', 'pm', 'lengths', 'XS', 'CA', 'CD', 'GA', 'GD', 'QP', 'AL', 'ACUM', 'S')]


class _DecBwdBufs(C.Structure):
    _fields_ = [(n, C.c_void_p) for n in (
        'dHC', 'DGA', 'DGD', 'DQ', 'DCTX', 'YD', 'YA', 'DCA', 'DCD', 'GPREV', 'GCUM', 'DV')]


class _DecPersistWeights(C.Structure):
    _fields_ = [(n, C.c_void_p) for n in (
        'w_ih_att', 'w_hh_att', 'w_ih_dec', 'w_hh_dec', 'bias_att', 'bias_dec', 'wq', 'wcomb', 'v', 'proj_w', 'proj_b',
        'prenet_w1')]


class _DecPersistBufs(C.Structure):
    _fields_ = [(n, C.c_void_p) for n in (
        'memory', 'pm', 'lengths', 'pre_first', 'MEL', 'GATE', 'AL', 'stop_flag', 'exchange', 'err_word')]


class _DecTrainPersistWeights(C.Structure):
    C_NAME = 't2v_dec_train_persist_weights'
    _fields_ = [(n, C.c_void_p) for n in (
        'w_ih_att', 'w_hh_att', 'w_ih_dec', 'w_hh_dec', 'bias_dec', 'wq', 'wcomb', 'v')]


class _GemmGroup(C.Structure):
    C_NAME = 't2v_gemm_group'
    _fields_ = [('A', C.c_void_p), ('sAi', C.c_long), ('sAk', C.c_long), ('nb', C.c_int), ('B', C.c_void_p * 3), ('sBj', C.c_long * 3),
                ('sBk', C.c_long * 3), ('N', C.c_int * 3), ('C', C.c_void_p * 3), ('ldc', C.c_int * 3)]


class _AchainDw(C.Structure):
    C_NAME = 't2v_achain_dw'
    _fields_ = [('planes', C.c_void_p), ('d_w_ih', C.c_void_p), ('ld_ih', C.c_int), ('d_w_hh', C.c_void_p), ('ld_hh', C.c_int),
                ('accumulate', C.c_int), ('tile_cap', C.c_int)]


class _DecInferBufs(C.Structure):
    _fields_ = [(n, C.c_void_p) for n in (
        'memory', 'pm', 'lengths', 'XS', 'CA', 'CD', 'QP', 'AL', 'ACUM', 'PRE', 'MEL', 'GATE', 'stop_flag',
        'prenet_w1', 'proj_w', 'proj_b')]


class _DecItems(C.Structure):
    C_NAME = 't2v_dec_items'
    _fields_ = [(n, C.c_void_p) for n in ('stop_item', 'item_seeds')]


EXPORTS = ('t2v_version', 't2v_last_error', 't2v_stamp', 't2v_debug_spin', 't2v_pack_lstm_weights', 't2v_pack_lstm_weights_bf16', 't2v_decoder_train_fwd',
           't2v_decoder_train_bwd', 't2v_clip_adam_step', 't2v_clip_adam_step_guarded', 't2v_decoder_replay_fwd_kernels', 't2v_mel_frontend', 't2v_set_phase_profile', 't2v_decoder_infer_steps', 't2v_conv1d_stat_blocks', 't2v_conv1d_stat_blocks_bf16', 't2v_conv1d_fwd', 't2v_conv1d_bwd', 't2v_conv1d_fwd_bf16', 't2v_conv1d_bwd_bf16', 't2v_conv1d_dw_scratch_floats', 't2v_conv1d_flip_weights', 't2v_gemm_bf16', 't2v_gemm_bf16_splitk', 't2v_gemm_bf16_splitk_scratch_floats', 't2v_attn_wgrad', 't2v_attn_wgrad_scratch_floats',
           't2v_bn_act_fwd', 't2v_bn_act_bwd', 't2v_bn_act_bwd_eval', 't2v_bilstm_fwd', 't2v_bilstm_bwd', 't2v_gemm_f32', 't2v_conv2d_s2_fwd', 't2v_conv2d_s2_bwd', 't2v_conv2d_s2_dw_scratch_floats', 't2v_conv2d_s2_fwd_gemm', 't2v_conv2d_s2_bwd_gemm',
           't2v_conv2d_s2_gemm_scratch_floats',
           't2v_gru_fwd', 't2v_gru_bwd', 't2v_loss_fwd_bwd', 't2v_fuse_location_weights', 't2v_decoder_qp_floats',
           't2v_set_step_params', 't2v_set_step_params_stream', 't2v_decoder_replay_bwd_kernels', 't2v_embedding_fwd', 't2v_embedding_bwd', 't2v_gemm_f32_splitk', 't2v_gemm_splitk_scratch_floats', 't2v_gemm_f32_batched',
           't2v_decoder_infer_persistent', 't2v_decoder_persist_supported', 't2v_decoder_persist_scratch_floats',
           't2v_attn_bwd_slices', 't2v_colsum', 't2v_colsum_scratch_floats', 't2v_gemm_epilogue_bwd',
           't2v_decoder_train_fwd_persistent', 't2v_decoder_train_persist_supported',
           't2v_decoder_train_persist_scratch_floats', 't2v_decoder_bwd_persist_supported',
           't2v_decoder_bwd_achain_scratch_floats', 't2v_decoder_bwd_achain', 't2v_decoder_bwd_achain_prepare',
           't2v_decoder_bwd_achain_prepared', 't2v_decoder_bwd_persist_slices', 't2v_decoder_bwd_achain_dq_offset',
           't2v_decoder_bwd_achain_dw_offset', 't2v_gemm_f32_grouped_handed', 't2v_gemm_f32_grouped_group_offset', 't2v_mask_outputs', 't2v_reparam_fwd',
           't2v_reparam_bwd', 't2v_gather_words', 't2v_concat2_rows',
           't2v_decoder_train_fwd_persistent16', 't2v_decoder_train_persist16_supported',
           't2v_decoder_train_persist16_scratch_floats', 't2v_decoder_bwd_persistent16', 't2v_decoder_bwd_persist16_supported',
           't2v_decoder_bwd_persist16_scratch_floats', 't2v_decoder_bwd_persist16_dq_offset', 't2v_decoder_bwd_persist16_slices',
           't2v_decoder_bwd_persist16_fits', 't2v_gemm_f32_set_mode', 't2v_conv1d_x3_set_mode', 't2v_gemm_f32_grouped',
           't2v_gemm_f32_grouped_scratch_floats', 't2v_gemm_bf16_grouped', 't2v_gemm_bf16_grouped_scratch_floats',
           't2v_decoder_bwd_persistent16_prepare', 't2v_decoder_bwd_persistent16_prepared',
           't2v_stft_polar', 't2v_istft', 't2v_istft_scratch_bytes', 't2v_griffin_lim', 't2v_griffin_lim_scratch_bytes',
           't2v_mel_to_magnitude', 't2v_decoder_infer_steps_items', 't2v_decoder_infer_persistent_items', 't2v_bn_act_fwd_len',
           't2v_mask_time', 't2v_conv2d_s2_fwd_ragged', 't2v_conv2d_s2_fwd_gemm_ragged', 't2v_conv2d_s2_gemm_ragged_scratch_floats',
           't2v_gru_fwd_len', 't2v_mel_dtw', 't2v_mel_dtw_scratch_bytes', 't2v_tsne_scratch_bytes', 't2v_tsne_affinities',
           't2v_tsne_gradient', 't2v_tsne_run')


def lib_path():
    return _LIB_PATH


def load_library():
    global _lib
    if _lib is not None:
        return _lib
    if not os.path.isfile(_LIB_PATH):
        raise T2VHipError("libt2vae_hip.so not built: run `python -c 'import __graft_entry__ as g; g.build()'` "
                          "(or make -C tacotron2-vae_amd/csrc)")
    lib = C.CDLL(_LIB_PATH)
    lib.t2v_version.restype = C.c_char_p
    lib.t2v_last_error.restype = C.c_char_p
    lib.t2v_pack_lstm_weights.argtypes = [C.c_void_p, C.c_void_p, C.c_void_p, C.c_void_p, C.c_int, C.c_void_p,
                                          C.c_void_p, C.c_void_p, C.c_void_p, C.c_void_p]
    lib.t2v_pack_lstm_weights_bf16.argtypes = [C.c_void_p, C.c_void_p, C.c_void_p, C.c_void_p, C.c_int, C.c_void_p,
                                          C.c_void_p, C.c_void_p, C.c_void_p, C.c_void_p]
    lib.t2v_fuse_location_weights.argtypes = [C.c_void_p, C.c_void_p, C.c_void_p, C.c_void_p]
    lib.t2v_decoder_qp_floats.argtypes = [C.c_int, C.c_int]
    lib.t2v_decoder_qp_floats.restype = C.c_long
    lib.t2v_attn_bwd_slices.argtypes = [C.c_int]
    lib.t2v_decoder_train_fwd.argtypes = [C.POINTER(_DecWeights), C.POINTER(_DecTrainBufs), C.c_int, C.c_int,
                                          C.c_int, C.c_float, C.c_float, C.c_uint64, C.c_void_p]
    lib.t2v_decoder_train_bwd.argtypes = [C.POINTER(_DecWeights), C.POINTER(_DecTrainBufs),
                                          C.POINTER(_DecBwdBufs), C.c_int, C.c_int, C.c_int, C.c_float,
                                          C.c_float, C.c_uint64, C.c_void_p]
    lib.t2v_decoder_train_fwd_persistent.argtypes = [C.POINTER(_DecTrainPersistWeights), C.POINTER(_DecTrainBufs), C.c_void_p,
                                                     C.c_int, C.c_int, C.c_int, C.c_float, C.c_float, C.c_uint64, C.c_void_p]
    lib.t2v_decoder_train_persist_supported.argtypes = [C.c_int, C.c_int]
    lib.t2v_decoder_train_fwd_persistent16.argtypes = lib.t2v_decoder_train_fwd_persistent.argtypes
    lib.t2v_decoder_train_persist16_supported.argtypes = [C.c_int, C.c_int]
    lib.t2v_decoder_train_persist16_scratch_floats.argtypes = [C.c_int, C.c_int, C.c_int]
    lib.t2v_decoder_train_persist16_scratch_floats.restype = C.c_long
    lib.t2v_decoder_bwd_persistent16.argtypes = [C.POINTER(_DecTrainPersistWeights), C.POINTER(_DecTrainBufs)] + [C.c_void_p] * 8 + [
        C.c_int, C.c_int, C.c_int, C.c_float, C.c_float, C.c_uint64, C.c_void_p]
    lib.t2v_decoder_bwd_persistent16_prepared.argtypes = lib.t2v_decoder_bwd_persistent16.argtypes
    lib.t2v_decoder_bwd_persistent16_prepare.argtypes = [C.c_void_p, C.c_void_p, C.c_void_p, C.c_int, C.c_int, C.c_int, C.c_void_p]
    lib.t2v_decoder_bwd_persist16_supported.argtypes = [C.c_int, C.c_int]
    lib.t2v_decoder_bwd_persist16_scratch_floats.argtypes = [C.c_int, C.c_int, C.c_int]
    lib.t2v_decoder_bwd_persist16_scratch_floats.restype = C.c_long
    lib.t2v_decoder_bwd_persist16_dq_offset.argtypes = [C.c_int, C.c_int, C.c_int]
    lib.t2v_decoder_bwd_persist16_dq_offset.restype = C.c_long
    lib.t2v_decoder_bwd_persist16_slices.argtypes = [C.c_int]
    lib.t2v_decoder_bwd_persist16_fits.argtypes = [C.c_int, C.c_int, C.c_int]
    lib.t2v_gemm_f32_set_mode.argtypes = [C.c_int]
    lib.t2v_conv1d_x3_set_mode.argtypes = [C.c_int]
    lib.t2v_gemm_f32_grouped_scratch_floats.argtypes = [C.POINTER(_GemmGroup), C.c_int, C.c_int, C.c_int]
    lib.t2v_gemm_f32_grouped_scratch_floats.restype = C.c_long
    lib.t2v_gemm_f32_grouped.argtypes = [C.POINTER(_GemmGroup), C.c_int, C.c_int, C.c_int, C.c_int, C.c_void_p, C.c_void_p]
    lib.t2v_gemm_bf16_grouped_scratch_floats.argtypes = lib.t2v_gemm_f32_grouped_scratch_floats.argtypes
    lib.t2v_gemm_bf16_grouped_scratch_floats.restype = C.c_long
    lib.t2v_gemm_bf16_grouped.argtypes = lib.t2v_gemm_f32_grouped.argtypes
    lib.t2v_decoder_train_persist_scratch_floats.argtypes = [C.c_int, C.c_int, C.c_int]
    lib.t2v_decoder_train_persist_scratch_floats.restype = C.c_long
    lib.t2v_decoder_bwd_persist_supported.argtypes = [C.c_int, C.c_int]
    lib.t2v_decoder_bwd_achain_scratch_floats.argtypes = [C.c_int, C.c_int, C.c_int]
    lib.t2v_decoder_bwd_achain_scratch_floats.restype = C.c_long
    lib.t2v_gemm_f32_grouped_handed.argtypes = [C.POINTER(_GemmGroup), C.c_int, C.c_int, C.c_int, C.c_int, C.c_void_p, C.c_int, C.c_void_p,
                                                C.c_int, C.c_void_p]
    lib.t2v_gemm_f32_grouped_group_offset.argtypes = [C.POINTER(_GemmGroup), C.c_int, C.c_int, C.c_int, C.c_int]
    lib.t2v_gemm_f32_grouped_group_offset.restype = C.c_long
    lib.t2v_decoder_bwd_achain_dw_offset.argtypes = [C.c_int, C.c_int, C.c_int]
    lib.t2v_decoder_bwd_achain_dw_offset.restype = C.c_long
    lib.t2v_decoder_bwd_achain.argtypes = [C.POINTER(_DecTrainPersistWeights), C.POINTER(_AchainDw), C.POINTER(_DecTrainBufs)] + [C.c_void_p] * 8 + [
        C.c_int, C.c_int, C.c_int, C.c_float, C.c_float, C.c_uint64, C.c_void_p]
    lib.t2v_decoder_bwd_persist_slices.argtypes = [C.c_int]
    lib.t2v_decoder_bwd_achain_dq_offset.argtypes = [C.c_int, C.c_int, C.c_int]
    lib.t2v_decoder_bwd_achain_dq_offset.restype = C.c_long
    lib.t2v_decoder_bwd_achain_prepared.argtypes = lib.t2v_decoder_bwd_achain.argtypes
    lib.t2v_decoder_bwd_achain_prepare.argtypes = [C.POINTER(_DecTrainBufs), C.c_void_p, C.c_void_p, C.c_void_p, C.c_int, C.c_int, C.c_int,
                                                   C.c_float, C.c_float, C.c_uint64, C.c_void_p]
    lib.t2v_decoder_replay_fwd_kernels.argtypes = [C.POINTER(_DecWeights), C.POINTER(_DecTrainBufs), C.c_int,
                                                   C.c_int, C.c_int, C.c_float, C.c_float, C.c_uint64, C.c_int,
                                                   C.c_void_p]
    lib.t2v_decoder_replay_bwd_kernels.argtypes = [C.POINTER(_DecWeights), C.POINTER(_DecTrainBufs),
                                                   C.POINTER(_DecBwdBufs), C.c_int, C.c_int, C.c_int, C.c_float,
                                                   C.c_float, C.c_uint64, C.c_int, C.c_void_p]
    lib.t2v_clip_adam_step.argtypes = [C.c_void_p, C.c_void_p, C.c_void_p, C.c_void_p, C.c_uint64, C.c_float,
                                       C.c_float, C.c_float, C.c_float, C.c_float, C.c_float, C.c_float,
                                       C.c_float, C.c_float, C.c_void_p, C.c_void_p, C.c_void_p]
    lib.t2v_clip_adam_step_guarded.argtypes = lib.t2v_clip_adam_step.argtypes[:-1] + [C.c_void_p, C.c_int, C.c_void_p]
    lib.t2v_mask_outputs.argtypes = [C.c_void_p] * 4 + [C.c_int, C.c_int, C.c_int, C.c_float, C.c_void_p]
    lib.t2v_reparam_fwd.argtypes = [C.c_void_p] * 4 + [C.c_long, C.c_void_p]
    lib.t2v_reparam_bwd.argtypes = [C.c_void_p] * 4 + [C.c_long, C.c_void_p]
    lib.t2v_concat2_rows.argtypes = [C.c_void_p, C.c_long, C.c_int, C.c_void_p, C.c_long, C.c_int, C.c_void_p, C.c_long, C.c_void_p]
    lib.t2v_gather_words.argtypes = [C.POINTER(C.c_void_p), C.POINTER(C.c_void_p), C.c_int, C.c_void_p]
    lib.t2v_embedding_fwd.argtypes = [C.c_void_p, C.c_void_p, C.c_void_p, C.c_int, C.c_int, C.c_int, C.c_int, C.c_void_p]
    lib.t2v_embedding_bwd.argtypes = [C.c_void_p, C.c_void_p, C.c_void_p, C.c_int, C.c_int, C.c_int, C.c_int, C.c_void_p]
    lib.t2v_gemm_epilogue_bwd.argtypes = [C.c_void_p, C.c_void_p, C.c_void_p, C.c_size_t, C.c_float, C.c_void_p]
    lib.t2v_colsum.argtypes = [C.c_void_p, C.c_long, C.c_long, C.c_long, C.c_void_p, C.c_void_p, C.c_void_p]
    lib.t2v_colsum_scratch_floats.argtypes = [C.c_long, C.c_long]
    lib.t2v_colsum_scratch_floats.restype = C.c_long
    lib.t2v_set_step_params.argtypes = [C.c_void_p]
    lib.t2v_set_step_params.restype = None
    lib.t2v_set_step_params_stream.argtypes = [C.c_void_p, C.c_void_p]
    lib.t2v_mel_frontend.argtypes = [C.c_void_p, C.c_void_p, C.c_void_p, C.c_int, C.c_int, C.c_float, C.c_int,
                                     C.c_int, C.c_int, C.c_void_p, C.c_void_p, C.c_void_p, C.c_void_p, C.c_void_p,
                                     C.c_void_p, C.c_int, C.c_void_p, C.c_int, C.c_void_p]
    lib.t2v_set_phase_profile.argtypes = [C.c_void_p]
    lib.t2v_stamp.argtypes = [C.c_void_p, C.c_int, C.c_void_p]
    lib.t2v_debug_spin.argtypes = [C.c_int, C.c_int, C.c_void_p]
    lib.t2v_decoder_infer_persistent.argtypes = [C.POINTER(_DecPersistWeights), C.POINTER(_DecPersistBufs), C.c_int, C.c_int,
                                                 C.c_int, C.c_float, C.c_float, C.c_uint64, C.c_void_p]
    lib.t2v_decoder_infer_persistent_items.argtypes = lib.t2v_decoder_infer_persistent.argtypes[:-1] + [C.POINTER(_DecItems),
                                                                                                        C.c_void_p]
    lib.t2v_decoder_persist_supported.argtypes = [C.c_int, C.c_int]
    lib.t2v_decoder_persist_scratch_floats.argtypes = [C.c_int, C.c_int]
    lib.t2v_decoder_persist_scratch_floats.restype = C.c_long
    lib.t2v_decoder_infer_steps.argtypes = [C.POINTER(_DecWeights), C.POINTER(_DecInferBufs), C.c_int, C.c_int, C.c_int,
                                            C.c_int, C.c_float, C.c_float, C.c_int, C.c_uint64, C.c_void_p]
    lib.t2v_decoder_infer_steps_items.argtypes = lib.t2v_decoder_infer_steps.argtypes[:-1] + [C.POINTER(_DecItems), C.c_void_p]
    vp = C.c_void_p
    lib.t2v_stft_polar.argtypes = [vp, vp, C.c_int, C.c_int, C.c_int, C.c_int, vp, vp, vp, vp, vp, C.c_int, vp]
    lib.t2v_istft_scratch_bytes.argtypes = [C.c_int, C.c_int]
    lib.t2v_istft_scratch_bytes.restype = C.c_size_t
    lib.t2v_istft.argtypes = [vp, vp, vp, C.c_int, C.c_int, C.c_int, C.c_int, vp, vp, vp, vp, vp, C.c_int, vp]
    lib.t2v_griffin_lim_scratch_bytes.argtypes = [C.c_int, C.c_int]
    lib.t2v_griffin_lim_scratch_bytes.restype = C.c_size_t
    lib.t2v_griffin_lim.argtypes = [vp, vp, vp, C.c_int, C.c_int, C.c_int, C.c_int, C.c_int, vp, vp, vp, vp, vp, C.c_int,
                                    vp]
    lib.t2v_mel_to_magnitude.argtypes = [vp, vp, vp, C.c_int, C.c_int, C.c_int, vp, vp]
    lib.t2v_mel_dtw_scratch_bytes.argtypes = [C.c_int, C.c_int, C.c_int]
    lib.t2v_mel_dtw_scratch_bytes.restype = C.c_size_t
    lib.t2v_mel_dtw.argtypes = [vp, vp, C.c_int, vp, vp, C.c_int, C.c_int, C.c_int, vp, vp, vp]
    lib.t2v_tsne_scratch_bytes.argtypes = [C.c_int, C.c_int]
    lib.t2v_tsne_scratch_bytes.restype = C.c_size_t
    lib.t2v_tsne_affinities.argtypes = [vp, C.c_int, C.c_int, C.c_float, vp, vp, vp]
    lib.t2v_tsne_gradient.argtypes = [vp, vp, C.c_int, C.c_float, vp, vp, vp, vp]
    lib.t2v_tsne_run.argtypes = [vp, vp, C.c_int, C.c_int, C.c_float, vp, vp, vp]
    lib.t2v_conv1d_stat_blocks.argtypes = [C.c_int, C.c_int, C.c_int, C.c_int, C.c_int]
    lib.t2v_conv1d_stat_blocks_bf16.argtypes = [C.c_int, C.c_int, C.c_int, C.c_int, C.c_int]
    lib.t2v_conv1d_fwd.argtypes = [vp, vp, vp, vp, vp, C.c_int, C.c_int, C.c_int, C.c_int, C.c_int, vp]
    lib.t2v_conv1d_bwd.argtypes = [vp, vp, vp, vp, vp, vp, vp, C.c_int, C.c_int, C.c_int, C.c_int, C.c_int, vp]
    lib.t2v_conv1d_dw_scratch_floats.argtypes = [C.c_int] * 5
    lib.t2v_conv1d_flip_weights.argtypes = [vp, vp, vp, vp, C.c_int, C.c_int, vp]
    lib.t2v_conv1d_fwd_bf16.argtypes = [vp, vp, vp, vp, vp, vp, C.c_int, C.c_int, C.c_int, C.c_int, C.c_int, vp]
    lib.t2v_conv1d_bwd_bf16.argtypes = [vp, vp, vp, vp, vp, vp, vp, C.c_int, C.c_int, C.c_int, C.c_int, C.c_int, vp]
    lib.t2v_bn_act_fwd.argtypes = [vp, vp, C.c_int, vp, vp, vp, vp, vp, vp, vp, C.c_int, C.c_int, C.c_int, C.c_int,
                                   C.c_int, C.c_float, C.c_float, C.c_float, C.c_uint64, C.c_uint32, C.c_uint32, vp]
    lib.t2v_bn_act_bwd.argtypes = [vp, vp, vp, vp, vp, vp, vp, vp, vp, vp, C.c_int, C.c_int, C.c_int, C.c_int, C.c_float,
                                   C.c_uint64, C.c_uint32, C.c_uint32, vp]
    lib.t2v_bn_act_bwd_eval.argtypes = lib.t2v_bn_act_bwd.argtypes
    lib.t2v_bn_act_fwd_len.argtypes = [vp, vp, vp, vp, vp, vp, vp, C.c_int, C.c_int, C.c_int, C.c_int, C.c_float, vp]
    lib.t2v_mask_time.argtypes = [vp, vp, vp, C.c_int, C.c_int, C.c_int, vp]
    lib.t2v_bilstm_fwd.argtypes = [vp, vp, vp, vp, vp, vp, vp, vp, C.c_int, C.c_int, vp]
    lib.t2v_bilstm_bwd.argtypes = [vp, vp, vp, vp, vp, vp, vp, vp, C.c_int, C.c_int, vp]
    lib.t2v_gemm_f32.argtypes = [vp, C.c_long, C.c_long, vp, C.c_long, C.c_long, vp, vp, C.c_int, C.c_int, C.c_int,
                                 C.c_int, C.c_int, C.c_int, C.c_float, C.c_uint64, C.c_uint32, C.c_uint32, vp]
    lib.t2v_gemm_bf16.argtypes = lib.t2v_gemm_f32.argtypes
    lib.t2v_gemm_bf16_splitk.argtypes = lib.t2v_gemm_f32.argtypes[:-1] + [vp, vp]
    lib.t2v_gemm_bf16_splitk_scratch_floats.argtypes = [C.c_int, C.c_int, C.c_int]
    lib.t2v_gemm_bf16_splitk_scratch_floats.restype = C.c_long
    lib.t2v_gemm_f32_splitk.argtypes = lib.t2v_gemm_f32.argtypes[:-1] + [vp, vp]
    lib.t2v_gemm_f32_batched.argtypes = [vp, C.c_long, C.c_long, C.c_long, vp, C.c_long, C.c_long, C.c_long, vp, C.c_long,
                                         C.c_int, C.c_int, C.c_int, C.c_int, C.c_int, vp]
    lib.t2v_gemm_splitk_scratch_floats.argtypes = [C.c_int, C.c_int, C.c_int]
    lib.t2v_gemm_splitk_scratch_floats.restype = C.c_long
    lib.t2v_attn_wgrad.argtypes = [vp, vp, vp, vp, vp, vp, vp, vp, C.c_int, C.c_int, C.c_int, vp]
    lib.t2v_attn_wgrad_scratch_floats.argtypes = []
    lib.t2v_conv2d_s2_fwd.argtypes = [vp, vp, vp, vp, C.c_int, C.c_int, C.c_int, C.c_int, C.c_int, C.c_int, vp]
    lib.t2v_conv2d_s2_bwd.argtypes = [vp, vp, vp, vp, vp, vp, C.c_int, C.c_int, C.c_int, C.c_int, C.c_int, C.c_int, vp]
    lib.t2v_conv2d_s2_fwd_gemm.argtypes = [vp, vp, vp, vp, vp, C.c_int, C.c_int, C.c_int, C.c_int, C.c_int, C.c_int, vp]
    lib.t2v_conv2d_s2_bwd_gemm.argtypes = [vp, vp, vp, vp, vp, vp, C.c_int, C.c_int, C.c_int, C.c_int, C.c_int, C.c_int, vp]
    lib.t2v_conv2d_s2_gemm_scratch_floats.argtypes = [C.c_int] * 6
    lib.t2v_conv2d_s2_gemm_scratch_floats.restype = C.c_long
    lib.t2v_conv2d_s2_dw_scratch_floats.argtypes = [C.c_int] * 6
    lib.t2v_gru_fwd.argtypes = [vp, vp, vp, vp, vp, vp, vp, C.c_int, C.c_int, vp]
    lib.t2v_gru_bwd.argtypes = [vp, vp, vp, vp, vp, vp, vp, vp, C.c_int, C.c_int, vp]
    lib.t2v_conv2d_s2_fwd_ragged.argtypes = [vp, vp, vp, vp, vp] + [C.c_int] * 7 + [vp]
    lib.t2v_conv2d_s2_fwd_gemm_ragged.argtypes = [vp, vp, vp, vp, vp, vp] + [C.c_int] * 7 + [vp]
    lib.t2v_conv2d_s2_gemm_ragged_scratch_floats.argtypes = [C.c_int] * 6
    lib.t2v_conv2d_s2_gemm_ragged_scratch_floats.restype = C.c_long
    lib.t2v_gru_fwd_len.argtypes = [vp, vp, vp, vp, vp, vp, vp, vp, vp, C.c_int, C.c_int, vp]
    lib.t2v_loss_fwd_bwd.argtypes = [vp] * 15 + [C.c_uint64, C.c_int, C.c_int, C.c_float, vp]
    for name in EXPORTS:
        getattr(lib, name)
    _lib = lib
    return lib


_BF16 = False

_BN_PENDING = []


def note_bn_counter(t):
    _BN_PENDING.append(t)


_BN_DEFER = [0]


def flush_bn_counters():
    if _BN_PENDING and not _BN_DEFER[0]:
        torch._foreach_add_(_BN_PENDING, 1)
        del _BN_PENDING[:]


class defer_bn_counters(object):

    def __enter__(self):
        _BN_DEFER[0] += 1

    def __exit__(self, *exc):
        _BN_DEFER[0] -= 1
        if exc[0] is None:
            flush_bn_counters()
        elif not _BN_DEFER[0]:
            del _BN_PENDING[:]
        return False


def set_bf16(on):
    global _BF16
    _BF16 = bool(on)


def bf16_enabled():
    return _BF16


_DEFAULT_REC = [None]


class StepParams(object):
    RING = 256
    FIELDS = {'lr': 2, 'bc1': 3, 'bc2s': 4, 'kl_weight': 5}

    def __init__(self, device, stream=None):
        lib = load_library()
        self.host = torch.zeros(self.RING, 8, dtype=torch.float32).pin_memory()
        self.dev = torch.zeros(8, dtype=torch.float32, device=device)
        self.cur = dict(epoch=0, lr=0.0, bc1=1.0, bc2s=1.0, kl_weight=0.0)
        self.dirty = True
        self._i = 0
        self.stream = stream
        self.extra_streams = []
        if stream is None:
            lib.t2v_set_step_params(C.c_void_p(self.dev.data_ptr()))
            _DEFAULT_REC[0] = self
        else:
            self.bind()

    def bind(self, extra=None):
        if extra is not None:
            self.extra_streams = list(extra)
        if self.stream is None:
            return
        lib = load_library()
        for st in [self.stream] + self.extra_streams:
            _check(lib.t2v_set_step_params_stream(C.c_void_p(st.cuda_stream), C.c_void_p(self.dev.data_ptr())),
                   't2v_set_step_params_stream')

    def set(self, **kw):
        for k, v in kw.items():
            v = int(v) if k == 'epoch' else float(v)
            if self.cur[k] != v:
                self.cur[k] = v
                self.dirty = True

    def upload(self, force=False):
        if not (self.dirty or force):
            return
        if torch.cuda.is_current_stream_capturing():
            raise T2VHipError("step parameters changed inside a graph capture")
        slot = self.host[self._i % self.RING]
        self._i += 1
        slot.view(torch.int64)[0] = self.cur['epoch']
        for k, i in self.FIELDS.items():
            slot[i] = self.cur[k]
        self.dev.copy_(slot, non_blocking=True)
        self.dirty = False

    def release(self):
        lib = load_library()
        if self.stream is None:
            if _DEFAULT_REC[0] is self:
                lib.t2v_set_step_params(None)
                _DEFAULT_REC[0] = None
        else:
            for st in [self.stream] + self.extra_streams:
                lib.t2v_set_step_params_stream(C.c_void_p(st.cuda_stream), None)


_STEP = None
_STEP_ALL = []


class Overlap(object):
    NAMES = ('vae', 'w', 'g', 'd')

    def __init__(self, device=None):
        self.on = True
        lo = int(os.environ.get('T2V_SIDE_PRIO', '0'))
        self._streams = {n: torch.cuda.Stream(device=device, priority=lo) for n in self.NAMES}
        self._used = []
        self._keep = []

    def streams(self):
        return list(self._streams.values())

    def stream(self, name):
        return self._streams[name]

    class _Inline(object):
        def __enter__(self):
            return False

        def __exit__(self, *exc):
            return False

    class _Fork(object):
        def __init__(self, st):
            self.ctx = torch.cuda.stream(st)

        def __enter__(self):
            self.ctx.__enter__()
            return True

# ... 576 lines not shown
    def forward(ctx, gpre, memory, pm, lengths, w_ih_att, w_hh_att, w_ih_dec, w_hh_dec, bias_dec,
                wq, loc_conv, loc_dense, v, p_att, p_dec, seed, grad_mode=True, pre=None, b_ih_att=None, b_hh_att=None,
                gpre_ready=None):
        lib = _require_gpu(memory, pm, w_ih_att)
        pre2 = None
        if pre is not None:
            assert gpre is None
            pre2 = _f32c(pre).view(-1, PRE)
            if gpre_ready is not None:
                gpre = gpre_ready.view(pre.shape[0], pre.shape[1], G4)
            else:
                gpre = gemm(pre2, w_ih_att.detach()[:, :PRE], (b_ih_att + b_hh_att).detach()).view(pre.shape[0], pre.shape[1], G4)
        T, B, _ = gpre.shape
        T_in = memory.shape[1]
        gpre, memory, pm = _f32c(gpre), _f32c(memory), _f32c(pm)
        need_grad = bool(grad_mode) and any(ctx.needs_input_grad)
        wbf = bool(_BF16)
        plans = DecoderCore.plan(lib, B, T_in, T, need_grad)
        fwd_persist = all(p.fwd != 'steps' for p in plans)
        bwd_persist = need_grad and all(p.bwd != 'steps' for p in plans)
        if fwd_persist and (bwd_persist or not need_grad):
            packs = (None, None, None, None)
        else:
            packs = pack_decoder_weights(w_ih_att, w_hh_att, w_ih_dec, w_hh_dec, KATT, need_grad and not bwd_persist, bf16=wbf,
                                         need_fwd=not fwd_persist)
        raw = tuple(_f32c(t.detach()) for t in (w_ih_att, w_hh_att, w_ih_dec, w_hh_dec, wq))
        wqT = wq.detach().t().contiguous()
        bias_dec = _f32c(bias_dec.detach())
        loc_conv, loc_dense, vv = _f32c(loc_conv.detach()), _f32c(loc_dense.detach()), _f32c(v.detach()).view(-1)
        wcomb = fuse_location_weights(loc_conv, loc_dense)
        chunks = []
        DecoderCore._note(chunk_kernels=[])
        for p in plans:
            if p.b0 == 0 and p.b1 == B:
                g_c, m_c, pm_c, l_c = gpre, memory, pm, lengths
            else:
                g_c, m_c, pm_c = gpre[:, p.b0:p.b1].contiguous(), memory[p.b0:p.b1].contiguous(), pm[p.b0:p.b1].contiguous()
                l_c = None if lengths is None else lengths[p.b0:p.b1].contiguous()
            chunks.append(DecoderCore._fwd_chunk(lib, p, g_c, m_c, pm_c, l_c, packs, bias_dec, wqT, wcomb, vv, need_grad,
                                                 p_att, p_dec, _chunk_seed(seed, p.b0), wbf, raw))
        hcs = []
        for _w, _s, k, _prep in chunks:
            XSc = k[4]
            Bc, XWc = XSc.size(1), XSc.size(2)
            hc_c = torch.empty(T, Bc, XWc - H, device=XSc.device, dtype=torch.float32)
            _check(lib.t2v_concat2_rows(_p(XSc[2:, :, KATT:]), XWc, XWc - KATT, _p(XSc[1:, :, H:KATT]), XWc, KATT - H, _p(hc_c),
                                        T * Bc, _stream()), 't2v_concat2_rows')
            hcs.append(hc_c)
        als = [k[10][1:].permute(1, 0, 2) for _, _, k, _ in chunks]
        HC = hcs[0] if len(hcs) == 1 else torch.cat(hcs, 1)
        align = als[0] if len(als) == 1 else torch.cat(als, 0)
        ctx.dims = (B, T_in, T, float(p_att), float(p_dec), int(seed))
        ctx.consts = (packs, bias_dec, wqT, wcomb, vv, loc_conv, loc_dense)
        ctx.wbf = wbf
        ctx.wrefs = (w_ih_att, w_hh_att, w_ih_dec, w_hh_dec)
        ctx.raw = raw
        ctx.pre2 = pre2
        ctx.pre_on_side = gpre_ready is not None
        ctx.plans = plans
        ctx.chunks = [k for _, _, k, _ in chunks] if need_grad else None
        ctx.prepared = [pr for _, _, _, pr in chunks] if need_grad else None
        ctx.mark_non_differentiable(align)
        if DecoderCore.keep_last:
            W0, S0, k0, _ = chunks[0]
            DecoderCore._note(last_call=(W0, S0, (k0[0].shape[1], T_in, T, float(p_att), float(p_dec), int(seed)),
                                         k0 + (packs, bias_dec, wqT, wcomb, vv)))
        return HC, align

    @staticmethod
    def backward(ctx, dHC, _dalign):
        lib = load_library()
        Bt, T_in, T, p_att, p_dec, seed = ctx.dims
        packs, bias_dec, wqT, wcomb, vv, loc_conv, loc_dense = ctx.consts
        packF_att, packF_dec, packB_att, packB_dec = packs
        if ctx.chunks is None:
            raise T2VHipError("DecoderCore.backward without a saved arena (forward ran under no_grad)")
        dev = dHC.device
        f32 = dict(device=dev, dtype=torch.float32)
        dHC = _f32c(dHC)
        tcap = (T_in + 15) // 16 * 16
        acc = bacc = None
        wg = None
        wg_fresh = False
        dga_l, dmem_l, dpm_l, dpre_l = [], [], [], []
        DecoderCore._note(chunk_bwd_kernels=[])
        for ci, (plan, keep) in enumerate(zip(ctx.plans, ctx.chunks)):
            gpre, memory, pm, lengths, XS, CA, CD, GA, GD, QP, AL, ACUM, S = keep
            b0, B = plan.b0, plan.b1 - plan.b0
            kept = DecoderCore.keep_last and b0 == 0
            dhc_c = dHC if B == Bt else dHC[:, b0:b0 + B].contiguous()
            DGA = torch.empty(T, B, G4, **f32)
            DGD = torch.empty(T, B, G4, **f32)
            DCTX = torch.empty(T, B, E, **f32)
            eng = _BWD_ENGINES.get(plan.bwd)
            NS = lib.t2v_attn_bwd_slices(T_in) if eng is None else getattr(lib, eng.slices)(T_in)
            DV = torch.empty(B, NS, A, **f32)
            Sb = _DecTrainBufs(*(_p(t) for t in keep))
            dwh = None
            if eng is not None:
                PW = _persist_weights(ctx.raw, bias_dec, wcomb, vv)
                prep, ctx.prepared[ci] = ctx.prepared[ci], None
                if prep is not None:
                    DQP, scratch, errw, pev = prep
                    torch.cuda.current_stream().wait_event(pev)
                else:
                    DQP, scratch, errw = DecoderCore._bwd_buffers(lib, eng, B, T_in, T, dev)
                if plan.dw_epilogue and set_f32_gemm_mode(None) and T * B >= 32:
                    if wg is None:
                        wg, wg_fresh = DecoderCore._wgrad_tensors(ctx, f32), True
                    pre_c = None
                    if ctx.pre2 is not None:
                        pre_c = ctx.pre2 if B == Bt else ctx.pre2.view(T, Bt, PRE)[:, b0:b0 + B].reshape(T * B, PRE)
                    groups = DecoderCore._dw_groups(DGA, DGD, XS, wg, pre_c, T, B)
                    dwh = GroupedHandOver(groups, 1, scratch[lib.t2v_decoder_bwd_achain_dw_offset(B, T_in, T):][:1], not wg_fresh,
                                          DecoderCore.dw_tile_cap)
                    if not wg_fresh and overlap() is not None:
                        overlap().wait('g')
                stamp('dec_bwd_begin')
                bufs = (dhc_c, DGA, DGD, DCTX, DV, DQP, scratch, errw)
                _bwd_launch(lib, eng, prep is not None, PW, Sb, bufs, (B, T_in, T, p_att, p_dec, _chunk_seed(seed, b0)),
                            None if dwh is None else dwh.dw)
                _err_note('decoder backward (persistent kernel hand-off)', errw)
                dq_off = getattr(lib, eng.dq_offset)(B, T_in, T)
                rows = eng.dq_rows or B
                dq_sum = scratch[dq_off:dq_off + T * rows * A].view(T, rows, A)[:, :B].reshape(T * B, A)
                DecoderCore._note(bwd=plan.bwd)
                if kept:
                    DecoderCore._note(last_bwd_persist=(PW, Sb, bufs, (B, T_in, T, p_att, p_dec, seed), keep + (ctx.raw, wcomb, vv, bias_dec, dwh)))
            else:
                W = _DecWeights(_p(packF_att), _p(packF_dec), _p(packB_att), _p(packB_dec), None, _p(bias_dec),
                                _p(wqT), _p(wcomb), _p(vv), int(bool(ctx.wbf)))
                DQ = torch.empty(T, B, NS, A, 2, **f32)
                YD = torch.empty(B, XW, **f32); YA = torch.empty(B, KATT, **f32)
                DCA = torch.empty(B, H, **f32); DCD = torch.empty(B, H, **f32)
                GPREV = torch.empty(2, B, NS, 2, 64, **f32); GCUM = torch.empty(B * NS * tcap + 64, **f32)
                Gb = _DecBwdBufs(_p(dhc_c), _p(DGA), _p(DGD), _p(DQ), _p(DCTX), _p(YD), _p(YA), _p(DCA),
                                 _p(DCD), _p(GPREV), _p(GCUM), _p(DV))
                _check(lib.t2v_decoder_train_bwd(C.byref(W), C.byref(Sb), C.byref(Gb), B, T_in, T, p_att, p_dec,
                                                 _chunk_seed(seed, b0), _stream()), 't2v_decoder_train_bwd')
                _err_note('decoder backward (dq hand-off)', GCUM.view(torch.int32)[B * NS * tcap + 1:][:1])
                dq_sum = DQ[..., 0].sum(2).view(T * B, A)
                DecoderCore._note(bwd='steps')
                if kept:
                    DecoderCore._note(last_bwd=(W, Sb, Gb, (B, T_in, T, p_att, p_dec, seed),
                                                keep + (dhc_c, DGA, DGD, DQ, DCTX, YD, YA, DCA, DCD, GPREV, GCUM, DV, packs, bias_dec,
                                                        wqT, wcomb, vv)))
            TB = T * B
            stamp('dec_bwd_end')
            fork = mark()
            d_memory = torch.empty(B, T_in, E, **f32)
            _check(lib.t2v_gemm_f32_batched(_p(AL[1:]), T_in, 1, B * T_in, _p(DCTX), E, 1, B * E, _p(d_memory), T_in * E, E, B,
                                            T_in, E, T, _stream()), 't2v_gemm_f32_batched')
            dpre = S
            d_pm = colsum(dpre.view(T, B * T_in * A)).view(B, T_in, A)
            dmem_l.append(d_memory); dpm_l.append(d_pm)
            if ctx.pre2 is not None and ctx.needs_input_grad[17] and not ctx.pre_on_side:
                dpre_l.append(gemm(DGA.view(TB, G4), ctx.wrefs[0].detach()[:, :PRE].t()).view(T, B, PRE))
            with side('w', keep=(DGA, DGD, DCTX, DV, dq_sum, dhc_c) + tuple(keep), after=fork):
                dga2, dgd2 = DGA.view(TB, G4), DGD.view(TB, G4)
                x_prev = XS[0:T].reshape(TB, XW)
                x_cur = XS[1:T + 1].reshape(TB, XW)
                first = wg is None or wg_fresh
                if wg is None:
                    wg = DecoderCore._wgrad_tensors(ctx, f32)
                wg_fresh = False
                if first and ctx.pre2 is None:
                    wg[0][:, :PRE].zero_()
                d_w_ih_att, d_w_hh_att, d_w_ih_dec, d_w_hh_dec = wg
                grouped = os.environ.get('T2V_DW_GROUPED', '1') != '0'
                if ctx.pre2 is not None:
                    pre_c = ctx.pre2 if B == Bt else ctx.pre2.view(T, Bt, PRE)[:, b0:b0 + B].reshape(TB, PRE)
                    if ctx.needs_input_grad[17] and ctx.pre_on_side:
                        dpre_l.append(gemm(dga2, ctx.wrefs[0].detach()[:, :PRE].t()).view(T, B, PRE))
                    if not grouped:
                        gemm(dga2.t(), pre_c.t(), out=d_w_ih_att[:, :PRE], accumulate=not first)
                with side('g', after=fork, keep=() if dwh is None else (dwh.scr,)):
                    if dwh is not None:
                        gemm_grouped(dwh.groups, accumulate=not first, handed=dwh)
                    elif grouped:
                        att = [(x_prev[:, :H].t(), d_w_hh_att), (x_prev[:, H:KATT].t(), d_w_ih_att[:, PRE:])]
                        if ctx.pre2 is not None:
                            att.insert(0, (pre_c.t(), d_w_ih_att[:, :PRE]))
                        gemm_grouped([(dga2.t(), att),
                                      (dgd2.t(), [(x_cur[:, :KATT].t(), d_w_ih_dec), (x_cur[:, KATT:].t(), d_w_hh_dec)])], accumulate=not first)
                    else:
                        gemm(dga2.t(), x_prev[:, :H].t(), out=d_w_hh_att, accumulate=not first)
                        gemm(dga2.t(), x_prev[:, H:KATT].t(), out=d_w_ih_att[:, PRE:], accumulate=not first)
                        gemm(dgd2.t(), x_cur[:, :KATT].t(), out=d_w_ih_dec, accumulate=not first)
                        gemm(dgd2.t(), x_cur[:, KATT:].t(), out=d_w_hh_dec, accumulate=not first)
                d_wq = gemm(dq_sum.t(), x_cur[:, :H].t())
                d_v = DV.sum((0, 1)).view(1, A)
                d_loc_dense, d_loc_conv = attn_wgrad(dpre, AL, ACUM, loc_conv, loc_dense, B, T_in, T)
                parts = [d_wq, d_loc_conv, d_loc_dense, d_v]
                acc = parts if acc is None else [x + y for x, y in zip(acc, parts)]
            bparts = [colsum(DGD.view(TB, G4))] + ([colsum(DGA.view(TB, G4))] if ctx.pre2 is not None else [])
            bacc = bparts if bacc is None else [x + y for x, y in zip(bacc, bparts)]
            dga_l.append(DGA)
        ctx.chunks = ctx.prepared = None
        d_wq, d_loc_conv, d_loc_dense, d_v = acc
        d_bias_dec = bacc[0]
        d_w_ih_att, d_w_hh_att, d_w_ih_dec, d_w_hh_dec = wg
        d_memory = dmem_l[0] if len(dmem_l) == 1 else torch.cat(dmem_l, 0)
        d_pm = dpm_l[0] if len(dpm_l) == 1 else torch.cat(dpm_l, 0)
        d_pre = d_b_att = None
        if ctx.pre2 is not None:
            DGA = None
            d_b_att = bacc[1]
            if dpre_l and ctx.pre_on_side:
                with side('w'):
                    d_pre = dpre_l[0] if len(dpre_l) == 1 else torch.cat(dpre_l, 1)
            elif dpre_l:
                d_pre = dpre_l[0] if len(dpre_l) == 1 else torch.cat(dpre_l, 1)
        else:
            DGA = dga_l[0] if len(dga_l) == 1 else torch.cat(dga_l, 1)
        return (DGA, d_memory, d_pm, None, d_w_ih_att, d_w_hh_att, d_w_ih_dec, d_w_hh_dec, d_bias_dec,
                d_wq, d_loc_conv, d_loc_dense, d_v, None, None, None, None, d_pre, d_b_att, d_b_att, None)


def attn_wgrad(dpre, AL, ACUM, loc_conv, loc_dense, B, T_in, T):
    lib = _require_gpu(dpre, AL, ACUM, loc_conv, loc_dense)
    f32 = dict(device=dpre.device, dtype=torch.float32)
    part = torch.empty(lib.t2v_attn_wgrad_scratch_floats(), **f32)
    d_dense, d_conv = torch.empty(A, F_LOC, **f32), torch.empty(F_LOC, 2, KS, **f32)
    _check(lib.t2v_attn_wgrad(_p(dpre), _p(AL), _p(ACUM), _p(_f32c(loc_conv)), _p(_f32c(loc_dense)), _p(part),
                              _p(d_dense), _p(d_conv), B, T_in, T, _stream()), 't2v_attn_wgrad')
    return d_dense, d_conv


def mel_frontend(wav, n_samples, tables, scale=1.0, t_stride=None):
    lib = _require_gpu(wav)
    B, N = wav.shape
    wav = wav.contiguous()
    if int(n_samples.min()) <= 512 or int(n_samples.max()) > N:
        raise ValueError("mel_frontend: every utterance needs 512 < n_samples <= %d, got [%d, %d]"
                         % (N, int(n_samples.min()), int(n_samples.max())))
    n_samples = n_samples.to(device=wav.device, dtype=torch.int64).contiguous()
    if t_stride is None:
        t_stride = int(n_samples.max().item()) // 256 + 1
    out = torch.empty(B, 80, t_stride, device=wav.device, dtype=torch.float32)
    is16 = wav.dtype == torch.int16
    if not is16 and wav.dtype != torch.float32:
        raise T2VHipError("mel_frontend takes float32 or int16 samples")
    _check(lib.t2v_mel_frontend(None if is16 else _p(wav), _p(wav) if is16 else None, _p(n_samples), B, N,
                                float(scale), 1024, 256, 80, _p(tables['window']), _p(tables['tw512']),
                                _p(tables['tw1024']), _p(tables['mel_start']), _p(tables['mel_len']),
                                _p(tables['mel_w']), int(tables['maxw']), _p(out), t_stride, _stream()),
           't2v_mel_frontend')
    return out


def _frame_counts(n_frames, B, T, device, min_frames=1):
    n = torch.full((B,), T, dtype=torch.int64) if n_frames is None else torch.as_tensor(n_frames).reshape(-1).cpu()
    if n.numel() != B or int(n.min()) < min_frames or int(n.max()) > T:
        raise ValueError("every utterance needs %d <= frames <= %d, got %s" % (min_frames, T, n.tolist()))
    return n.to(device=device, dtype=torch.int32)


def stft_polar(wav, n_samples, tables, t_stride=None):
    lib = _require_gpu(wav)
    B, N = wav.shape
    wav = _f32c(wav)
    n = torch.full((B,), N, dtype=torch.int64) if n_samples is None else torch.as_tensor(n_samples).reshape(-1).cpu()
    if n.numel() != B or int(n.min()) <= 512 or int(n.max()) > N:
        raise ValueError("stft: every utterance needs 512 < n_samples <= %d, got %s" % (N, n.tolist()))
    if t_stride is None:
        t_stride = int(n.max()) // 256 + 1
    mag = torch.empty(B, 513, t_stride, device=wav.device, dtype=torch.float32)
    phase = torch.empty_like(mag)
    _check(lib.t2v_stft_polar(_p(wav), _p(n.to(wav.device)), B, N, 1024, 256, _p(tables['window']), _p(tables['tw512']),
                              _p(tables['tw1024']), _p(mag), _p(phase), t_stride, _stream()), 't2v_stft_polar')
    return mag, phase


def istft(mag, phase, n_frames, tables):
    lib = _require_gpu(mag, phase)
    B, nb, T = mag.shape
    if nb != 513 or phase.shape != mag.shape:
        raise ValueError("istft: magnitude and phase must both be (B, 513, T)")
    mag, phase = _f32c(mag), _f32c(phase)
    n = _frame_counts(n_frames, B, T, mag.device)
    out = torch.empty(B, 256 * (T - 1), device=mag.device, dtype=torch.float32)
    scratch = torch.empty(lib.t2v_istft_scratch_bytes(B, T), device=mag.device, dtype=torch.uint8)
    _check(lib.t2v_istft(_p(mag), _p(phase), _p(n), B, T, 1024, 256, _p(tables['window']), _p(tables['tw512']),
                         _p(tables['tw1024']), _p(scratch), _p(out), out.size(1), _stream()), 't2v_istft')
    return out


def griffin_lim(mag, angles, n_frames, tables, n_iters):
    lib = _require_gpu(mag, angles)
    B, nb, T = mag.shape
    if nb != 513 or angles.shape != mag.shape:
        raise ValueError("griffin_lim: magnitudes and angles must both be (B, 513, T)")
    mag, angles = _f32c(mag), _f32c(angles)
    n = _frame_counts(n_frames, B, T, mag.device, min_frames=4)
    out = torch.empty(B, 256 * (T - 1), device=mag.device, dtype=torch.float32)
    scratch = torch.empty(lib.t2v_griffin_lim_scratch_bytes(B, T), device=mag.device, dtype=torch.uint8)
    _check(lib.t2v_griffin_lim(_p(mag), _p(angles), _p(n), B, T, 1024, 256, int(n_iters), _p(tables['window']),
                               _p(tables['tw512']), _p(tables['tw1024']), _p(scratch), _p(out), out.size(1), _stream()),
           't2v_griffin_lim')
    return out


def mel_to_magnitude(mel, n_frames, pinv_basis):
    lib = _require_gpu(mel, pinv_basis)
    B, n_mel, T = mel.shape
    mel = _f32c(mel)
    n = _frame_counts(n_frames, B, T, mel.device)
    mag = torch.empty(B, 513, T, device=mel.device, dtype=torch.float32)
    _check(lib.t2v_mel_to_magnitude(_p(mel), _p(_f32c(pinv_basis)), _p(n), B, T, n_mel, _p(mag), _stream()),
           't2v_mel_to_magnitude')
    return mag


DTW_MAX_FRAMES = 2048
DTW_SCRATCH_CAP = 256 << 20


def _dtw_lengths(n, B, stride, what):
    n = torch.as_tensor(n).reshape(-1).cpu()
    if n.dtype.is_floating_point or n.numel() != B:
        raise ValueError("mel_dtw: %s must be %d integer frame counts, got %s" % (what, B, n.tolist()))
    if int(n.min()) < 1 or int(n.max()) > min(stride, DTW_MAX_FRAMES):
        raise ValueError("mel_dtw: every %s must be in 1..%d (%d frames stored, at most %d supported), got %s"
                         % (what, min(stride, DTW_MAX_FRAMES), stride, DTW_MAX_FRAMES, n.tolist()))
    return n.to(torch.int32)


def mel_dtw(x, nx, y, ny):
    lib = _require_gpu(x, y)
    if x.dim() != 3 or y.dim() != 3 or x.dtype != torch.float32 or y.dtype != torch.float32:
        raise ValueError("mel_dtw: x and y must be float32 (B, 80, T) tensors")
    B, n_mel, sx = x.shape
    if y.size(0) != B or B < 1:
        raise ValueError("mel_dtw: %d sequences in x, %d in y" % (B, y.size(0)))
    if n_mel != 80 or y.size(1) != 80:
        raise ValueError("mel_dtw: 80 mel channels only, got %d and %d" % (n_mel, y.size(1)))
    sy = y.size(2)
    if sx < 1 or sy < 1:
        raise ValueError("mel_dtw: empty time axis")
    nx = _dtw_lengths(nx, B, sx, 'nx').to(x.device)
    ny = _dtw_lengths(ny, B, sy, 'ny').to(x.device)
    x, y = _f32c(x), _f32c(y)
    dist = torch.empty(B, device=x.device, dtype=torch.float32)
    per_pair = lib.t2v_mel_dtw_scratch_bytes(1, sx, sy)
    group = max(1, min(B, DTW_SCRATCH_CAP // per_pair))
    for b0 in range(0, B, group):
        nb = min(group, B - b0)
        scratch = torch.empty(lib.t2v_mel_dtw_scratch_bytes(nb, sx, sy), device=x.device, dtype=torch.uint8)
# ... 367 lines not shown
    x = _f32c(x)
    out = torch.empty_like(x)
    B, Cn, T = x.shape
    _check(lib.t2v_mask_time(_p(x), _p(out), _p(lengths_i32), B, Cn, T, _stream()), 't2v_mask_time')
    return out


def conv_bn_act_eval_len(x, weight, bias, gamma, beta, running_mean, running_var, act, lengths_i32):
    lib = _require_gpu(x, weight, lengths_i32)
    assert lengths_i32.dtype == torch.int32 and lengths_i32.numel() == x.size(0)
    x = _f32c(x)
    B, Cin, T = x.shape
    Cout, _, KS = weight.shape
    y = torch.empty(B, Cout, T, device=x.device, dtype=torch.float32)
    w = _f32c(weight.detach())
    if _BF16 and KS == 5 and Cin % 16 == 0 and Cin >= 128 and Cout >= 128:
        wp = torch.empty(w.numel(), device=x.device, dtype=torch.bfloat16)
        _check(lib.t2v_conv1d_fwd_bf16(_p(w), _p(x), _p(bias), _p(y), None, _p(wp), B, Cin, T, Cout, KS, _stream()),
               't2v_conv1d_fwd_bf16')
    else:
        _check(lib.t2v_conv1d_fwd(_p(w), _p(x), _p(bias), _p(y), None, B, Cin, T, Cout, KS, _stream()), 't2v_conv1d_fwd')
    out = torch.empty_like(y)
    _check(lib.t2v_bn_act_fwd_len(_p(y), _p(gamma), _p(beta), _p(running_mean), _p(running_var), _p(out), _p(lengths_i32),
                                  B, Cout, T, int(act), 1e-5, _stream()), 't2v_bn_act_fwd_len')
    return out


class Reparam(torch.autograd.Function):

    @staticmethod
    def forward(ctx, eps, mu, logvar):
        lib = _require_gpu(eps, mu, logvar)
        eps, mu, logvar = _f32c(eps), _f32c(mu), _f32c(logvar)
        z = torch.empty_like(mu)
        _check(lib.t2v_reparam_fwd(_p(eps), _p(mu), _p(logvar), _p(z), mu.numel(), _stream()), 't2v_reparam_fwd')
        ctx.save_for_backward(eps, logvar)
        return z

    @staticmethod
    def backward(ctx, dz):
        eps, logvar = ctx.saved_tensors
        dz = _f32c(dz)
        dlv = torch.empty_like(logvar)
        _check(load_library().t2v_reparam_bwd(_p(dz), _p(eps), _p(logvar), _p(dlv), dz.numel(), _stream()), 't2v_reparam_bwd')
        return None, dz, dlv


class BiLSTM(torch.autograd.Function):

    _prep = {}

    @staticmethod
    def prepare(w_hh, b_ih, b_hh, w_hh_r, b_ih_r, b_hh_r):
        with torch.no_grad():
            whh = torch.stack((w_hh, w_hh_r)).contiguous()
            bias, bias_r = b_ih + b_hh, b_ih_r + b_hh_r
        ev = torch.cuda.Event()
        ev.record()
        BiLSTM._prep[id(w_hh)] = (whh, bias, bias_r, ev)

    @staticmethod
    def forward(ctx, x, lengths, w_ih, w_hh, b_ih, b_hh, w_ih_r, w_hh_r, b_ih_r, b_hh_r, save):
        lib = _require_gpu(x, w_ih)
        B, T, _ = x.shape
        f32 = dict(device=x.device, dtype=torch.float32)
        x = _f32c(x)
        prep = BiLSTM._prep.pop(id(w_hh), None)
        if prep is not None:
            whh, bias, bias_r, ev = prep
            cur = torch.cuda.current_stream()
            cur.wait_event(ev)
            for t in (whh, bias, bias_r):
                t.record_stream(cur)
        else:
            whh = torch.stack((w_hh, w_hh_r)).contiguous()
            bias, bias_r = b_ih + b_hh, b_ih_r + b_hh_r
        y = torch.empty(B, T, 512, **f32)
        chunks = []
        for b0 in range(0, B, MAX_DEC_B):
            b1 = min(B, b0 + MAX_DEC_B)
            Bc = b1 - b0
            gx = torch.empty(2, Bc, T, 1024, **f32)
            gemm(x[b0:b1].view(Bc * T, -1), w_ih, bias, out=gx[0].view(Bc * T, 1024))
            gemm(x[b0:b1].view(Bc * T, -1), w_ih_r, bias_r, out=gx[1].view(Bc * T, 1024))
            gates = torch.empty(2, Bc, T, 1024, **f32) if save else None
            cells = torch.empty(2, Bc, T, 256, **f32) if save else None
            hx = torch.empty(2 * 2 * 2 * 16 * 256, **f32)
            sync = torch.empty(3, device=x.device, dtype=torch.int32)
            _check(lib.t2v_bilstm_fwd(_p(gx), _p(whh), _p(lengths[b0:b1]), _p(y[b0:b1]), _p(gates), _p(cells), _p(hx),
                                      _p(sync), Bc, T, _stream()), 't2v_bilstm_fwd')
            _err_note('BiLSTM forward', sync[2:3])
            chunks.append((b0, b1, gates, cells, sync))
        ctx.keep = (x, lengths, w_ih, w_ih_r, whh, y.detach(), chunks)
        ctx.dims = (B, T)
        return y

    @staticmethod
    def backward(ctx, dy):
        lib = load_library()
        x, lengths, w_ih, w_ih_r, whh, y, chunks = ctx.keep
        B, T = ctx.dims
        if chunks[0][2] is None:
            raise T2VHipError("BiLSTM forward ran without saving activations")
        f32 = dict(device=x.device, dtype=torch.float32)
        dy = _f32c(dy)
        dg = torch.empty(2, B, T, 1024, **f32) if len(chunks) == 1 else None
        dgs = []
        stamp('bilstm_bwd_begin')
        for b0, b1, gates, cells, sync in chunks:
            Bc = b1 - b0
            dg_c = dg if dg is not None else torch.empty(2, Bc, T, 1024, **f32)
            dgx = torch.empty(2 * 2 * 2 * 16 * 16 * 256, **f32)
            _check(lib.t2v_bilstm_bwd(_p(whh), _p(lengths[b0:b1]), _p(dy[b0:b1]), _p(gates), _p(cells), _p(dg_c), _p(dgx),
                                      _p(sync), Bc, T, _stream()), 't2v_bilstm_bwd')
            _err_note('BiLSTM backward', sync[2:3])
            dgs.append(dg_c)
        stamp('bilstm_bwd_end')
        BT = B * T
        if dg is None:
            dg = torch.cat(dgs, 1)
        d0, d1, x2 = dg[0].reshape(BT, 1024), dg[1].reshape(BT, 1024), x.view(BT, -1)
        fork = mark()
        dx = gemm(d0, w_ih.t())
        gemm(d1, w_ih_r.t(), out=dx, accumulate=True)
        dx = dx.view(B, T, -1)
        db0, db1 = colsum(d0), colsum(d1)
        with side('w', keep=(dg, d0, d1, dy), after=fork):
            z = y.new_zeros(B, 1, 256)
            hp0 = torch.cat((z, y[:, :-1, :256]), 1).reshape(BT, 256)
            hp1 = torch.cat((y[:, 1:, 256:], z), 1).reshape(BT, 256)
            g = (gemm(d0.t(), x2.t(), out=grad_slot(w_ih)), gemm(d0.t(), hp0.t()),
                 gemm(d1.t(), x2.t(), out=grad_slot(w_ih_r)), gemm(d1.t(), hp1.t()))
        return (dx, None, g[0], g[1], db0, db0, g[2], g[3], db1, db1, None)


def bilstm_check(sync):
    if int(sync[2].item()) != 0:
        raise T2VHipError("BiLSTM cooperative kernel timed out on its inter-workgroup barrier")


def colsum(x):
    lib = _require_gpu(x)
    assert x.dim() == 2 and x.dtype == torch.float32
    if x.stride(1) != 1 and x.shape[1] > 1:
        x = x.contiguous()
    M, N = x.shape
    out = torch.empty(N, device=x.device, dtype=torch.float32)
    nscr = lib.t2v_colsum_scratch_floats(M, N)
    scr = torch.empty(nscr, device=x.device, dtype=torch.float32) if nscr else None
    _check(lib.t2v_colsum(_p(x), x.stride(0) if M > 1 else N, M, N, _p(scr), _p(out), _stream()), 't2v_colsum')
    return out


_GRAD_SLOTS = {}


def register_grad_slots(slots):
    _GRAD_SLOTS.clear()
    _GRAD_SLOTS.update(slots)


def grad_slot(weight):
    if not weight.is_leaf or weight.grad is not None:
        return None
    ent = _GRAD_SLOTS.get(weight.data_ptr())
    if ent is None:
        return None
    flat, off, shape = ent
    if tuple(shape) != tuple(weight.shape) or flat.device != weight.device:
        return None
    return flat[off:off + weight.numel()].view(shape)


def _small_grads(params, n, f32):
    out = []
    for p in params:
        g = grad_slot(p) if p is not None else None
        out.append(torch.empty(n, **f32) if g is None else g)
    return out


def _group_array(groups):
    arr = (_GemmGroup * len(groups))()
    for g, (A, parts) in zip(arr, groups):
        g.A, g.sAi, g.sAk, g.nb = A.data_ptr(), A.stride(0), A.stride(1), len(parts)
        for p, (Bp, out) in enumerate(parts):
            g.B[p], g.sBj[p], g.sBk[p], g.N[p] = Bp.data_ptr(), Bp.stride(0), Bp.stride(1), Bp.shape[0]
            g.C[p], g.ldc[p] = out.data_ptr(), out.stride(0)
    return arr


class GroupedHandOver(object):

    def __init__(self, groups, g, counter, accumulate, cap=None):
        lib = load_library()
        assert g == 1 and len(groups) == 2 and len(groups[1][1]) == 2
        M, K = groups[0][0].shape
        self.groups, self.g, self.counter = groups, g, counter
        arr = _group_array(groups)
        off = lib.t2v_gemm_f32_grouped_group_offset(arr, len(groups), M, K, g)
        if off < 0:
            raise T2VHipError("GroupedHandOver: these products do not take the grouped plane launch")
        self.scr = torch.empty(lib.t2v_gemm_f32_grouped_scratch_floats(arr, len(groups), M, K), device=counter.device, dtype=torch.float32)
        self.cap = -1 if cap is None else int(cap)
        (_, out_ih), (_, out_hh) = groups[g][1]
        self.dw = _AchainDw(self.scr.data_ptr() + 4 * off, out_ih.data_ptr(), out_ih.stride(0), out_hh.data_ptr(), out_hh.stride(0),
                            int(bool(accumulate)), self.cap)


def gemm_grouped(groups, accumulate=False, handed=None):
    lib = _require_gpu(groups[0][0])
    M, K = groups[0][0].shape
    if handed is not None:
        assert handed.groups is groups and not _BF16
        cap = handed.cap if handed.cap >= 0 else 2 ** 31 - 1
        _check(lib.t2v_gemm_f32_grouped_handed(_group_array(groups), len(groups), M, K, int(bool(accumulate)), _p(handed.scr), handed.g,
                                               _p(handed.counter), cap, _stream()), 't2v_gemm_f32_grouped_handed')
        return
    ok = 1 <= len(groups) <= 2
    for A, parts in groups:
        ok = ok and A.shape == (M, K) and A.dtype == torch.float32 and 1 <= len(parts) <= 3
        for Bp, out in parts:
            ok = ok and Bp.shape[1] == K and Bp.dtype == torch.float32 and out.shape == (M, Bp.shape[0]) and out.stride(1) == 1 and Bp.shape[0] % 128 == 0
    if not ok:
        for A, parts in groups:
            for Bp, out in parts:
                gemm(A, Bp, out=out, accumulate=accumulate)
        return
    arr = _group_array(groups)
    size_fn, run_fn = ((lib.t2v_gemm_bf16_grouped_scratch_floats, lib.t2v_gemm_bf16_grouped) if _BF16 else
                       (lib.t2v_gemm_f32_grouped_scratch_floats, lib.t2v_gemm_f32_grouped))
    nscr = size_fn(arr, len(groups), M, K)
    scr = torch.empty(max(nscr, 4), device=groups[0][0].device, dtype=torch.float32)
    _check(run_fn(arr, len(groups), M, K, int(bool(accumulate)), _p(scr), _stream()), 't2v_gemm_grouped')


def set_f32_gemm_mode(x3):
    return bool(load_library().t2v_gemm_f32_set_mode(-1 if x3 is None else int(bool(x3))))


def gemm(A, B, bias=None, out=None, relu=False, accumulate=False, p_drop=0.0, seed=0, rng_stream=0, rng_t=0):
    lib = _require_gpu(A, B)
    M, K = A.shape
    N, K2 = B.shape
    assert K == K2 and A.dtype == torch.float32 and B.dtype == torch.float32
    if out is None:
        out = torch.empty(M, N, device=A.device, dtype=torch.float32)
    assert out.shape == (M, N) and out.dtype == torch.float32 and (N == 1 or out.stride(1) == 1)
    ldc = out.stride(0) if M > 1 else max(N, out.stride(0))
    assert ldc >= N and (ldc == N or p_drop == 0.0)
    if True:
        nscr = lib.t2v_gemm_splitk_scratch_floats(M, N, K)
        if nscr and _BF16 and ((M + 63) // 64) * ((N + 63) // 64) >= 64:
            nscr = 0
        if nscr:
            scr = torch.empty(nscr, device=A.device, dtype=torch.float32)
            _check(lib.t2v_gemm_f32_splitk(_p(A), A.stride(0), A.stride(1), _p(B), B.stride(0), B.stride(1), _p(bias), _p(out),
                                           ldc, M, N, K, int(relu), int(accumulate), float(p_drop), int(seed), int(rng_stream),
                                           int(rng_t), _p(scr), _stream()), 't2v_gemm_f32_splitk')
            return out
    if _BF16:
        nscr = lib.t2v_gemm_bf16_splitk_scratch_floats(M, N, K)
        if nscr:
            scr = torch.empty(nscr, device=A.device, dtype=torch.float32)
            _check(lib.t2v_gemm_bf16_splitk(_p(A), A.stride(0), A.stride(1), _p(B), B.stride(0), B.stride(1), _p(bias), _p(out),
                                            ldc, M, N, K, int(relu), int(accumulate), float(p_drop), int(seed), int(rng_stream),
                                            int(rng_t), _p(scr), _stream()), 't2v_gemm_bf16_splitk')
            return out
    fn = lib.t2v_gemm_bf16 if _BF16 else lib.t2v_gemm_f32
    _check(fn(_p(A), A.stride(0), A.stride(1), _p(B), B.stride(0), B.stride(1), _p(bias), _p(out), ldc,
              M, N, K, int(relu), int(accumulate), float(p_drop), int(seed), int(rng_stream),
              int(rng_t), _stream()), 't2v_gemm_bf16' if _BF16 else 't2v_gemm_f32')
    return out


class LinearHIP(torch.autograd.Function):

    @staticmethod
    def forward(ctx, x, weight, bias, relu, p_drop, seed, rng_stream, rng_t):
        _require_gpu(x, weight)
        x2 = x.reshape(-1, x.shape[-1])
        x2 = x2 if x2.dtype == torch.float32 else x2.float()
        y = gemm(x2, weight, bias, relu=relu, p_drop=p_drop, seed=seed, rng_stream=rng_stream, rng_t=rng_t)
        ctx.save_for_backward(x2, weight, y if (relu or p_drop > 0) else None)
        ctx.cfg = (x.shape, bool(relu), float(p_drop), bias is not None)
        return y.view(*x.shape[:-1], weight.shape[0])

    @staticmethod
    def backward(ctx, dy):
        x2, weight, y = ctx.saved_tensors
        xshape, relu, p, has_bias = ctx.cfg
        dy2 = _f32c(dy.reshape(-1, weight.shape[0]))
        if relu or p > 0:
            scale = 1.0 / (1.0 - p) if p > 0 else 1.0
            masked = torch.empty_like(dy2)
            _check(load_library().t2v_gemm_epilogue_bwd(_p(dy2), _p(y), _p(masked), dy2.numel(), scale, _stream()),
                   't2v_gemm_epilogue_bwd')
            dy2 = masked
        fork = mark()
        dx = gemm(dy2, weight.t()) if ctx.needs_input_grad[0] else None
        if weight.is_leaf:
            with side('w', keep=(dy2, x2), after=fork):
                dw = gemm(dy2.t(), x2.t(), out=grad_slot(weight))
        else:
            dw = gemm(dy2.t(), x2.t())
        db = colsum(dy2) if has_bias else None
        return (dx.view(xshape) if dx is not None else None), dw, db, None, None, None, None, None


CONV2D_GEMM = os.environ.get('T2V_CONV2D_GEMM', '1') != '0'


class Conv2dBNReLU(torch.autograd.Function):

    @staticmethod
    def forward(ctx, x, weight, bias, gamma, beta, running_mean, running_var, training, coord):
        lib = _require_gpu(x, weight)
        x = _f32c(x)
        B, Cx, Hh, Ww = x.shape
        Cout = weight.shape[0]
        Ho, Wo = (Hh - 1) // 2 + 1, (Ww - 1) // 2 + 1
        f32 = dict(device=x.device, dtype=torch.float32)
        w = weight.contiguous()
        y = torch.empty(B, Cout, Ho, Wo, **f32)
        gscr = None
        if CONV2D_GEMM:
            gscr = torch.empty(lib.t2v_conv2d_s2_gemm_scratch_floats(B, Cx, Hh, Ww, Cout, int(coord)), **f32)
            _check(lib.t2v_conv2d_s2_fwd_gemm(_p(x), _p(w), _p(bias), _p(y), _p(gscr), B, Cx, Hh, Ww, Cout, int(coord), _stream()),
                   't2v_conv2d_s2_fwd_gemm')
        else:
            _check(lib.t2v_conv2d_s2_fwd(_p(x), _p(w), _p(bias), _p(y), B, Cx, Hh, Ww, Cout, int(coord), _stream()),
                   't2v_conv2d_s2_fwd')
        mean = torch.empty(Cout, **f32) if training else None
        rstd = torch.empty(Cout, **f32) if training else None
        out = torch.empty_like(y)
        _check(lib.t2v_bn_act_fwd(_p(y), None, 0, _p(gamma), _p(beta), _p(running_mean), _p(running_var), _p(mean),
                                  _p(rstd), _p(out), B, Cout, Ho * Wo, ACT_RELU, int(bool(training)), 0.0, 0.1, 1e-5,
                                  0, 0, 0, _stream()), 't2v_bn_act_fwd')
        ctx.keep = (x, w, y, mean, rstd, gamma, beta)
        ctx.gscr = gscr
        ctx.running = (running_mean, running_var)
        ctx.small = (gamma, beta, bias)
        ctx.cfg = (B, Cx, Hh, Ww, Cout, Ho, Wo, int(coord), bool(training))
        return out

    @staticmethod
    def backward(ctx, dout):
        lib = load_library()
        x, w, y, mean, rstd, gamma, beta = ctx.keep
        B, Cx, Hh, Ww, Cout, Ho, Wo, coord, training = ctx.cfg
        bn_bwd = lib.t2v_bn_act_bwd
        if not training:
            mean, rstd = ctx.running[0], torch.rsqrt(ctx.running[1] + 1e-5)
            bn_bwd = lib.t2v_bn_act_bwd_eval
        f32 = dict(device=x.device, dtype=torch.float32)
        dout = dout.contiguous()
        dy = torch.empty_like(y)
        dgamma, dbeta, dbias = _small_grads(ctx.small, Cout, f32)
        _check(bn_bwd(_p(y), _p(dout), _p(mean), _p(rstd), _p(gamma), _p(beta), _p(dy), _p(dgamma),
                      _p(dbeta), _p(dbias), B, Cout, Ho * Wo, ACT_RELU, 0.0, 0, 0, 0, _stream()), 't2v_bn_act_bwd')
        dx = torch.empty_like(x) if ctx.needs_input_grad[0] else None
        dw = torch.empty_like(w)
        if ctx.gscr is not None:
            _check(lib.t2v_conv2d_s2_bwd_gemm(_p(x), _p(w), _p(dy), _p(dx), _p(dw), _p(ctx.gscr), B, Cx, Hh, Ww, Cout, coord,
                                              _stream()), 't2v_conv2d_s2_bwd_gemm')
            ctx.gscr = None
        else:
            nscr = lib.t2v_conv2d_s2_dw_scratch_floats(B, Cx, Hh, Ww, Cout, coord)
            scr = torch.empty(nscr, **f32) if nscr else None
            _check(lib.t2v_conv2d_s2_bwd(_p(x), _p(w), _p(dy), _p(dx), _p(dw), _p(scr), B, Cx, Hh, Ww, Cout, coord,
                                         _stream()), 't2v_conv2d_s2_bwd')
        return dx, dw, dbias, dgamma, dbeta, None, None, None, None


class GRULast(torch.autograd.Function):

    @staticmethod
    def forward(ctx, x, w_ih, w_hh, b_ih, b_hh):
        lib = _require_gpu(x, w_ih)
        B, T, I = x.shape
        f32 = dict(device=x.device, dtype=torch.float32)
        x2 = _f32c(x).view(B * T, I)
        gi = gemm(x2, w_ih, b_ih)
        hs = torch.empty(B, T + 1, 256, **f32)
        gsave = torch.empty(B, T, 4, 256, **f32)
        whh = w_hh.contiguous()
        xchg = torch.empty(2 * 16 * 768, **f32)
        syncs = []
        gi3 = gi.view(B, T, 768)
        for b0 in range(0, B, MAX_DEC_B):
            b1 = min(B, b0 + MAX_DEC_B)
            sync = torch.empty(2, device=x.device, dtype=torch.int32)
            _check(lib.t2v_gru_fwd(_p(gi3[b0:b1]), _p(whh), _p(b_hh), _p(hs[b0:b1]), _p(gsave[b0:b1]), _p(xchg), _p(sync),
                                   b1 - b0, T, _stream()), 't2v_gru_fwd')
            _err_note('GRU forward', sync[1:2])
            syncs.append(sync)
        ctx.keep = (x2, w_ih, whh, hs, gsave, xchg, syncs)
        ctx.dims = (B, T, I)
        return hs[:, T].clone()

    @staticmethod
    def backward(ctx, dh):
        lib = load_library()
        x2, w_ih, whh, hs, gsave, xchg, syncs = ctx.keep
        B, T, I = ctx.dims
        f32 = dict(device=x2.device, dtype=torch.float32)
        dgi, dgh = torch.empty(B, T, 768, **f32), torch.empty(B, T, 768, **f32)
        dh = dh.contiguous()
        for i, b0 in enumerate(range(0, B, MAX_DEC_B)):
            b1 = min(B, b0 + MAX_DEC_B)
            _check(lib.t2v_gru_bwd(_p(whh), _p(hs[b0:b1]), _p(gsave[b0:b1]), _p(dh[b0:b1]), _p(dgi[b0:b1]), _p(dgh[b0:b1]),
                                   _p(xchg), _p(syncs[i]), b1 - b0, T, _stream()), 't2v_gru_bwd')
            _err_note('GRU backward', syncs[i][1:2])
        dgi2, dgh2 = dgi.view(B * T, 768), dgh.view(B * T, 768)
        fork = mark()
        dx = gemm(dgi2, w_ih.t()).view(B, T, I)
        with side('w', keep=(dgi, dgh, hs, x2), after=fork):
            hprev = hs[:, :T].reshape(B * T, 256)
            g = (gemm(dgi2.t(), x2.t()), gemm(dgh2.t(), hprev.t()))
        return (dx,) + g + (colsum(dgi2), colsum(dgh2))


def refenc_heights(n_frames, n_layers):
    h = [[int(x) for x in n_frames]]
    for _ in range(n_layers):
        h.append([(x - 1) // 2 + 1 for x in h[-1]])
    return h


def refenc_ragged(mel, n_frames, layers, gru):
    lib = _require_gpu(mel)
    x = _f32c(mel)
    B, n_mels, T = x.shape
    f32 = dict(device=x.device, dtype=torch.float32)
    heights = torch.tensor(refenc_heights(n_frames, len(layers)), dtype=torch.int32).to(x.device)
    Hh, Ww, Cx = T, n_mels, 1
    for i, (weight, bias, gamma, beta, running_mean, running_var) in enumerate(layers):
        coord, tstride = int(i == 0), (T if i == 0 else 0)
        Cout = weight.shape[0]
        Ho, Wo = (Hh - 1) // 2 + 1, (Ww - 1) // 2 + 1
        w = _f32c(weight.detach())
        y = torch.empty(B, Cout, Ho, Wo, **f32)
        hlen = heights[i]
        if CONV2D_GEMM:
            scr = torch.empty(lib.t2v_conv2d_s2_gemm_ragged_scratch_floats(B, Cx, Hh, Ww, Cout, coord), **f32)
            _check(lib.t2v_conv2d_s2_fwd_gemm_ragged(_p(x), _p(w), _p(bias), _p(y), _p(scr), _p(hlen), B, Cx, Hh, Ww, Cout, coord,
                                                     tstride, _stream()), 't2v_conv2d_s2_fwd_gemm_ragged')
        else:
            _check(lib.t2v_conv2d_s2_fwd_ragged(_p(x), _p(w), _p(bias), _p(y), _p(hlen), B, Cx, Hh, Ww, Cout, coord, tstride,
                                                _stream()), 't2v_conv2d_s2_fwd_ragged')
        x = torch.empty_like(y)
        _check(lib.t2v_bn_act_fwd(_p(y), None, 0, _p(gamma), _p(beta), _p(running_mean), _p(running_var), None, None, _p(x),
                                  B, Cout, Ho * Wo, ACT_RELU, 0, 0.0, 0.1, 1e-5, 0, 0, 0, _stream()), 't2v_bn_act_fwd')
        Hh, Ww, Cx = Ho, Wo, Cout
    steps = heights[len(layers)]
    seq = x.transpose(1, 2).contiguous().view(B * Hh, Cx * Ww)
    w_ih, w_hh, b_ih, b_hh = gru
    gi = gemm(seq, w_ih.detach(), b_ih.detach()).view(B, Hh, 768)
    hs = torch.empty(B, Hh + 1, 256, **f32)
    h_last = torch.empty(B, 256, **f32)
    whh = _f32c(w_hh.detach())
    xchg = torch.empty(2 * 16 * 256, **f32)
    for b0 in range(0, B, MAX_DEC_B):
        b1 = min(B, b0 + MAX_DEC_B)
        sync = torch.empty(2, device=x.device, dtype=torch.int32)
        _check(lib.t2v_gru_fwd_len(_p(gi[b0:b1]), _p(whh), _p(b_hh), _p(hs[b0:b1]), None, _p(xchg), _p(sync), _p(steps[b0:b1]),
                                   _p(h_last[b0:b1]), b1 - b0, Hh, _stream()), 't2v_gru_fwd_len')
        _err_note('GRU forward', sync[1:2])
    return h_last


class VAELoss(torch.autograd.Function):
    _scratch = {}

    @staticmethod
    def forward(ctx, mel, post, gate, mu, logvar, mel_t, gate_t, kl_weight):
        lib = _require_gpu(mel, post, gate, mu, logvar)
        dev = mel.device
        key = str(dev)
        if key not in VAELoss._scratch:
            VAELoss._scratch[key] = (torch.empty(192, device=dev), torch.zeros(1, device=dev, dtype=torch.int32))
        part, ticket = VAELoss._scratch[key]
        mel, post, gate, mu, logvar = (_f32c(t) for t in (mel, post, gate, mu, logvar))
        mel_t, gate_t = _f32c(mel_t), _f32c(gate_t)
        out = torch.empty(4, device=dev, dtype=torch.float32)
        sp = step_params(create=False)
        if sp is not None:
            sp.set(kl_weight=kl_weight)
            sp.upload()
        grads = [torch.empty_like(t) for t in (mel, post, gate, mu, logvar)]
        _check(lib.t2v_loss_fwd_bwd(_p(mel), _p(post), _p(mel_t), _p(gate), _p(gate_t), _p(mu), _p(logvar),
                                    *[_p(g) for g in grads], _p(part), _p(out), _p(ticket), mel.numel(),
                                    gate.numel(), mu.numel(), float(kl_weight), _stream()), 't2v_loss_fwd_bwd')
        ctx.grads = grads
        ctx.mark_non_differentiable(out)
        return out[0], out

    @staticmethod
    def backward(ctx, dtotal, _dout):
        g = torch._foreach_mul(ctx.grads, dtotal)
        return (g[0], g[1], g[2], g[3], g[4], None, None, None)
```

Baseline: 228,100 mel-frames/s.

## Batch refencoder conv weight-grad GEMMs and colsums into grouped multi-launch kernels

Adds grouped kernels that run several column sums, several batched GEMMs and several dW reductions in one launch each, using a block-offset table to dispatch. The reference-encoder conv backward is split into a dx GEMM path and a deferred dW job that is collected across layers and flushed as one grouped GEMM plus one reduction on the side stream. Decoder bias column sums are combined into one multi-colsum launch, and the GRU bias colsums move onto the weight-grad side stream. The aim is to cut kernel-launch count and serialization in backward, at the cost of more complex bookkeeping for deferred gradients and grad-slot aliasing.

```diff
diff --git a/include/t2vae.h b/include/t2vae.h
--- a/include/t2vae.h
+++ b/include/t2vae.h
@@ -257,6 +257,8 @@
 
 long t2v_colsum_scratch_floats(long M, long N);
 int t2v_colsum(const float* A, long lda, long M, long N, float* scratch, float* out, void* stream);
+int t2v_colsum_multi(const float* const* A, const long* lda, const long* M, const long* N, float* const* scratch, float* const* out,
+                     int count, void* stream);
 
 int t2v_mask_outputs(float* mel, float* mel_post, float* gate, const int* lengths, int B, int C, int T, float gate_fill,
                      void* stream);
@@ -327,6 +329,21 @@
                            int Cout, int coord, void* stream);
 int t2v_conv2d_s2_bwd_gemm(const float* x, const float* w, const float* dy, float* dx, float* dw, float* scratch, int B, int Cx, int H,
                            int W, int Cout, int coord, void* stream);
+typedef struct t2v_conv2d_dw_job {
+    const float* dy;
+    float* scratch;
+    float* dw;
+    int B;
+    int Cx;
+    int H;
+    int W;
+    int Cout;
+    int coord;
+} t2v_conv2d_dw_job;
+long t2v_conv2d_s2_dcol_floats(int B, int Cx, int H, int W, int coord);
+int t2v_conv2d_s2_dx_gemm(const float* x, const float* w, const float* dy, float* dx, float* dcol, int B, int Cx, int H, int W,
+                          int Cout, int coord, void* stream);
+int t2v_conv2d_s2_dw_gemm_multi(const t2v_conv2d_dw_job* jobs, int njobs, void* stream);
 int t2v_gru_fwd(const float* gi, const float* whh, const float* bhh, float* hs, float* gsave, float* xchg,
                 uint32_t* sync2, int B, int T, void* stream);
 int t2v_gru_bwd(const float* whh, const float* hs, const float* gsave, const float* dh_last, float* dgi,
diff --git a/tacotron2-vae_amd/csrc/colsum.hip b/tacotron2-vae_amd/csrc/colsum.hip
--- a/tacotron2-vae_amd/csrc/colsum.hip
+++ b/tacotron2-vae_amd/csrc/colsum.hip
@@ -15,11 +15,11 @@
 }
 
 template <bool VEC>
-__global__ __launch_bounds__(256) void k_colsum(const float* __restrict__ A, long lda, int M, int N, int rows_per_slice,
-                                                float* __restrict__ dst, float* __restrict__ out, unsigned* __restrict__ ctr) {
+__device__ __forceinline__ void colsum_block(const float* __restrict__ A, long lda, int M, int N, int rows_per_slice, float* __restrict__ dst,
+                                             float* __restrict__ out, unsigned* __restrict__ ctr, const int bx, const int by, const int ny) {
     const int tid = threadIdx.x, cq = tid & 15, rl = tid >> 4;
-    const int j0 = blockIdx.x * CS_COLS + 4 * cq;
-    const int r0 = blockIdx.y * rows_per_slice, r1 = min(M, r0 + rows_per_slice);
+    const int j0 = bx * CS_COLS + 4 * cq;
+    const int r0 = by * rows_per_slice, r1 = min(M, r0 + rows_per_slice);
     __shared__ float4 red[CS_ROWL][16];
     float4 acc = {0.f, 0.f, 0.f, 0.f};
     if (VEC) {
@@ -51,30 +51,54 @@
     red[rl][cq] = acc;
     __syncthreads();
     if (tid < CS_COLS) {
-        const int j = blockIdx.x * CS_COLS + tid;
+        const int j = bx * CS_COLS + tid;
         const float* rf = (const float*)&red[0][0];
         float s = 0.f;
 #pragma unroll
         for (int r = 0; r < CS_ROWL; ++r) s += rf[r * CS_COLS + tid];
-        if (j < N) { if (ctr) st_sc1(dst + (size_t)blockIdx.y * N + j, s); else dst[(size_t)blockIdx.y * N + j] = s; }
+        if (j < N) { if (ctr) st_sc1(dst + (size_t)by * N + j, s); else dst[(size_t)by * N + j] = s; }
     }
     if (!ctr) return;
     __shared__ unsigned last_;
     asm volatile("s_waitcnt vmcnt(0)" ::: "memory");
     __syncthreads();
-    if (tid == 0) last_ = __hip_atomic_fetch_add(ctr + blockIdx.x, 1u, __ATOMIC_RELAXED, __HIP_MEMORY_SCOPE_AGENT) == gridDim.y - 1 ? 1u : 0u;
+    if (tid == 0) last_ = __hip_atomic_fetch_add(ctr + bx, 1u, __ATOMIC_RELAXED, __HIP_MEMORY_SCOPE_AGENT) == (unsigned)ny - 1 ? 1u : 0u;
     __syncthreads();
     if (!last_) return;
-    if (tid == 0) __hip_atomic_store(ctr + blockIdx.x, 0u, __ATOMIC_RELAXED, __HIP_MEMORY_SCOPE_AGENT);
+    if (tid == 0) __hip_atomic_store(ctr + bx, 0u, __ATOMIC_RELAXED, __HIP_MEMORY_SCOPE_AGENT);
     if (tid < CS_COLS) {
-        const int j = blockIdx.x * CS_COLS + tid;
+        const int j = bx * CS_COLS + tid;
         if (j < N) {
             float s = 0.f;
-            const int RS = (int)gridDim.y;
+            const int RS = ny;
             for (int r = 0; r < RS; ++r) s += ld_sc1(dst + (size_t)r * N + j);
             out[j] = s;
         }
     }
+}
+
+template <bool VEC>
+__global__ __launch_bounds__(256) void k_colsum(const float* __restrict__ A, long lda, int M, int N, int rows_per_slice,
+                                                float* __restrict__ dst, float* __restrict__ out, unsigned* __restrict__ ctr) {
+    colsum_block<VEC>(A, lda, M, N, rows_per_slice, dst, out, ctr, blockIdx.x, blockIdx.y, gridDim.y);
+}
+
+#define CS_MULTI_MAX 4
+struct ColsumMulti {
+    const float* A[CS_MULTI_MAX];
+    float* dst[CS_MULTI_MAX];
+    float* out[CS_MULTI_MAX];
+    unsigned* ctr[CS_MULTI_MAX];
+    long lda[CS_MULTI_MAX];
+    int M[CS_MULTI_MAX], N[CS_MULTI_MAX], rows[CS_MULTI_MAX], nx[CS_MULTI_MAX], ny[CS_MULTI_MAX], start[CS_MULTI_MAX + 1];
+    int count;
+};
+__global__ __launch_bounds__(256) void k_colsum_multi(ColsumMulti m) {
+    int p = 0;
+    for (int q = 1; q < m.count; ++q)
+        if ((int)blockIdx.x >= m.start[q]) p = q;
+    const int local = (int)blockIdx.x - m.start[p], nx = m.nx[p];
+    colsum_block<true>(m.A[p], m.lda[p], m.M[p], m.N[p], m.rows[p], m.dst[p], m.out[p], m.ctr[p], local % nx, local / nx, m.ny[p]);
 }
 
 extern "C" long t2v_colsum_scratch_floats(long M, long N) {
@@ -102,3 +126,36 @@
     else k_colsum<false><<<grid, 256, 0, stream>>>(A, lda, (int)M, (int)N, rows, dst, out, ctr);
     return t2v_check_launch();
 }
+
+extern "C" int t2v_colsum_multi(const float* const* A, const long* lda, const long* M, const long* N, float* const* scratch, float* const* out,
+                                int count, void* stream_) {
+    hipStream_t stream = (hipStream_t)stream_;
+    if (!A || !lda || !M || !N || !scratch || !out || count < 1 || count > CS_MULTI_MAX) return T2V_ERR_ARG;
+    ColsumMulti m;
+    m.count = count;
+    long blocks = 0;
+    for (int p = 0; p < count; ++p) {
+        if (!A[p] || !out[p] || M[p] < 1 || N[p] < 1 || lda[p] < N[p] || M[p] > 0x7fffffff || N[p] > 0x7fffffff) return T2V_ERR_ARG;
+        if ((N[p] & 3) || (lda[p] & 3) || ((uintptr_t)A[p] & 15)) return T2V_ERR_ARG;
+        const int rs = colsum_slices_(M[p], N[p]);
+        if (rs > 1 && !scratch[p]) return T2V_ERR_ARG;
+        const long nx = (N[p] + CS_COLS - 1) / CS_COLS;
+        m.A[p] = A[p]; m.lda[p] = lda[p]; m.M[p] = (int)M[p]; m.N[p] = (int)N[p]; m.rows[p] = (int)((M[p] + rs - 1) / rs);
+        m.dst[p] = rs > 1 ? scratch[p] : out[p]; m.out[p] = out[p]; m.ctr[p] = nullptr;
+        m.nx[p] = (int)nx; m.ny[p] = rs; m.start[p] = (int)blocks;
+        if (rs > 1) {
+            if (nx > 4096) return T2V_ERR_ARG;
+            m.ctr[p] = t2v_arrival_counters((int)nx);
+            if (!m.ctr[p]) return T2V_ERR_LAUNCH;
+        }
+        blocks += nx * rs;
+        if (blocks > 0x3fffffff) return T2V_ERR_DIMS;
+    }
+    for (int p = count; p <= CS_MULTI_MAX; ++p) m.start[p] = (int)blocks;
+    for (int p = count; p < CS_MULTI_MAX; ++p) {
+        m.A[p] = nullptr; m.dst[p] = m.out[p] = nullptr; m.ctr[p] = nullptr; m.lda[p] = 0;
+        m.M[p] = m.N[p] = m.rows[p] = 0; m.nx[p] = m.ny[p] = 1;
+    }
+    k_colsum_multi<<<(unsigned)blocks, 256, 0, stream>>>(m);
+    return t2v_check_launch();
+}
diff --git a/tacotron2-vae_amd/csrc/gemm.hip b/tacotron2-vae_amd/csrc/gemm.hip
--- a/tacotron2-vae_amd/csrc/gemm.hip
+++ b/tacotron2-vae_amd/csrc/gemm.hip
@@ -88,17 +88,17 @@
 }
 
 template <bool A_KC, bool B_KC>
-__global__ __launch_bounds__(256) void k_gemm_f32(GemmArgs a) {
+__device__ __forceinline__ void gemm_f32_tile(GemmArgs a, const int bx, const int by, const int bz) {
     __shared__ float As[2][GM_BK][GM_BM + 1];
     __shared__ float Bs[2][GM_BK][GM_BN + 1];
     const int tid = threadIdx.x, wave = tid >> 6, lane = tid & 63;
     const int wm = wave >> 1, wn = wave & 1;
-    const int i0 = blockIdx.y * GM_BM, j0 = blockIdx.x * GM_BN;
+    const int i0 = by * GM_BM, j0 = bx * GM_BN;
     if (a.nbatch > 1) {
-        const int zb = a.nsub > 1 ? blockIdx.z / a.nsub : blockIdx.z, zs = a.nsub > 1 ? blockIdx.z - zb * a.nsub : 0;
-        a.A += zb * a.sAb + zs * a.sAs; a.B += zb * a.sBb + zs * a.sBs; a.C += blockIdx.z * a.sCb;
-    }
-    const int kbeg = a.kz_chunk ? blockIdx.z * a.kz_chunk : 0, kend = a.kz_chunk ? min(a.K, kbeg + a.kz_chunk) : a.K;
+        const int zb = a.nsub > 1 ? bz / a.nsub : bz, zs = a.nsub > 1 ? bz - zb * a.nsub : 0;
+        a.A += zb * a.sAb + zs * a.sAs; a.B += zb * a.sBb + zs * a.sBs; a.C += bz * a.sCb;
+    }
+    const int kbeg = a.kz_chunk ? bz * a.kz_chunk : 0, kend = a.kz_chunk ? min(a.K, kbeg + a.kz_chunk) : a.K;
     constexpr int NE = GM_BM * GM_BK / 256;
     float ra[NE], rb[NE];
     auto load_tiles = [&](int k0) {
@@ -145,6 +145,29 @@
         __syncthreads();
     }
     gemm64_epilogue(a, acc, i0, j0, wm, wn, lane, tid);
+}
+
+template <bool A_KC, bool B_KC>
+__global__ __launch_bounds__(256) void k_gemm_f32(GemmArgs a) {
+    gemm_f32_tile<A_KC, B_KC>(a, blockIdx.x, blockIdx.y, blockIdx.z);
+}
+
+#define GM_MULTI_MAX 8
+struct GemmMultiArgs {
+    GemmArgs g[GM_MULTI_MAX];
+    int start[GM_MULTI_MAX + 1];
+    int gx[GM_MULTI_MAX], gy[GM_MULTI_MAX];
+    int n;
+};
+template <bool A_KC, bool B_KC>
+__global__ __launch_bounds__(256) void k_gemm_f32_multi(GemmMultiArgs m) {
+    const int id = blockIdx.x;
+    int p = 0;
+    for (int q = 1; q < m.n; ++q)
+        if (id >= m.start[q]) p = q;
+    const int local = id - m.start[p], gx = m.gx[p], gy = m.gy[p];
+    const int bx = local % gx, r = local / gx;
+    gemm_f32_tile<A_KC, B_KC>(m.g[p], bx, r % gy, r / gy);
 }
 
 #include <atomic>
@@ -1000,15 +1023,44 @@
     return t2v_check_launch();
 }
 
-int t2v_gemm_f32_batched_ex(const float* A, long sAb, long sAs, long sAi, long sAk, const float* B, long sBb, long sBs, long sBj, long sBk,
-                            const float* bias_row, float* C, long sCb, int ldc, int nbatch, int nsub, int M, int N, int K, hipStream_t stream) {
-    if (!A || !B || !C || nbatch < 1 || nsub < 1 || (long)nbatch * nsub > 65535 || M < 1 || N < 1 || K < 1 || ldc < N) return T2V_ERR_ARG;
-    GemmArgs a;
+static bool gemm_batched_args(GemmArgs& a, const float* A, long sAb, long sAs, long sAi, long sAk, const float* B, long sBb, long sBs, long sBj,
+                              long sBk, const float* bias_row, float* C, long sCb, int ldc, int nbatch, int nsub, int M, int N, int K,
+                              hipStream_t stream) {
+    if (!A || !B || !C || nbatch < 1 || nsub < 1 || (long)nbatch * nsub > 65535 || M < 1 || N < 1 || K < 1 || ldc < N) return false;
     a.A = A; a.B = B; a.bias = bias_row; a.C = C; a.sAi = sAi; a.sAk = sAk; a.sBj = sBj; a.sBk = sBk;
     a.M = M; a.N = N; a.K = K; a.ldc = ldc; a.relu = 0; a.accumulate = 0;
     a.p_drop = 0.f; a.seed = 0; a.rng_stream = 0; a.rng_t = 0; a.step = t2v_step_for(stream);
     a.kz_chunk = 0; a.part = nullptr; a.nbatch = nbatch * nsub > 1 ? nbatch * nsub : 1; a.sAb = sAb; a.sBb = sBb; a.sCb = sCb;
     a.nsub = nsub; a.sAs = sAs; a.sBs = sBs; a.bias_row = bias_row ? 1 : 0; a.tile_ctr = nullptr;
+    return true;
+}
+int t2v_gemm_f32_batched_multi(const T2vBatchedGemm* d, int n, hipStream_t stream) {
+    if (!d || n < 1 || n > GM_MULTI_MAX) return T2V_ERR_ARG;
+    GemmMultiArgs m;
+    m.n = n;
+    long total = 0;
+    for (int p = 0; p < n; ++p) {
+        const T2vBatchedGemm& q = d[p];
+        if (q.sAk != 1 || q.sBk == 1) return T2V_ERR_ARG;
+        if (!gemm_batched_args(m.g[p], q.A, q.sAb, q.sAs, q.sAi, q.sAk, q.B, q.sBb, q.sBs, q.sBj, q.sBk, nullptr, q.C, q.sCb, q.ldc, q.nbatch,
+                               q.nsub, q.M, q.N, q.K, stream))
+            return T2V_ERR_ARG;
+        m.gx[p] = (q.N + GM_BN - 1) / GM_BN;
+        m.gy[p] = (q.M + GM_BM - 1) / GM_BM;
+        m.start[p] = (int)total;
+        total += (long)m.gx[p] * m.gy[p] * q.nbatch * q.nsub;
+        if (total > 0x3fffffff) return T2V_ERR_DIMS;
+    }
+    for (int p = n; p <= GM_MULTI_MAX; ++p) m.start[p] = (int)total;
+    for (int p = n; p < GM_MULTI_MAX; ++p) { m.g[p] = m.g[0]; m.gx[p] = m.gy[p] = 1; }
+    k_gemm_f32_multi<true, false><<<(unsigned)total, 256, 0, stream>>>(m);
+    return t2v_check_launch();
+}
+
+int t2v_gemm_f32_batched_ex(const float* A, long sAb, long sAs, long sAi, long sAk, const float* B, long sBb, long sBs, long sBj, long sBk,
+                            const float* bias_row, float* C, long sCb, int ldc, int nbatch, int nsub, int M, int N, int K, hipStream_t stream) {
+    GemmArgs a;
+    if (!gemm_batched_args(a, A, sAb, sAs, sAi, sAk, B, sBb, sBs, sBj, sBk, bias_row, C, sCb, ldc, nbatch, nsub, M, N, K, stream)) return T2V_ERR_ARG;
     const bool akc = sAk == 1, bkc = sBk == 1;
     dim3 grid((N + GM_BN - 1) / GM_BN, (M + GM_BM - 1) / GM_BM, nbatch * nsub);
     if (akc && bkc) k_gemm_f32<true, true><<<grid, 256, 0, stream>>>(a);
diff --git a/tacotron2-vae_amd/csrc/refenc.hip b/tacotron2-vae_amd/csrc/refenc.hip
--- a/tacotron2-vae_amd/csrc/refenc.hip
+++ b/tacotron2-vae_amd/csrc/refenc.hip
@@ -148,6 +148,33 @@
     dw[i] = s;
 }
 
+#define DW_MULTI_MAX 8
+struct DwReduceMulti {
+    const float* part[DW_MULTI_MAX];
+    float* dw[DW_MULTI_MAX];
+    int n[DW_MULTI_MAX], nsplit[DW_MULTI_MAX], start[DW_MULTI_MAX + 1];
+    int count;
+};
+__global__ __launch_bounds__(256) void k_conv2d_s2_dw_reduce_multi(DwReduceMulti m) {
+    int p = 0;
+    for (int q = 1; q < m.count; ++q)
+        if ((int)blockIdx.x >= m.start[q]) p = q;
+    const int i = ((int)blockIdx.x - m.start[p]) * 256 + threadIdx.x, n = m.n[p], nsplit = m.nsplit[p];
+    if (i >= n) return;
+    const float* __restrict__ part = m.part[p];
+    float s = 0.f;
+    int k = 0;
+    for (; k + 8 <= nsplit; k += 8) {
+        float v[8];
+#pragma unroll
+        for (int u = 0; u < 8; ++u) v[u] = part[(size_t)(k + u) * n + i];
+#pragma unroll
+        for (int u = 0; u < 8; ++u) s += v[u];
+    }
+    for (; k < nsplit; ++k) s += part[(size_t)k * n + i];
+    m.dw[p][i] = s;
+}
+
 static inline int conv2d_dw_splits(int pairs, int positions) {
     int ns = 1;
     while (pairs * ns < 2048 && positions / (2 * ns) >= 1024 && ns < 64) ns *= 2;
@@ -311,6 +338,53 @@
     return t2v_check_launch();
 }
 
+
+extern "C" long t2v_conv2d_s2_dcol_floats(int B, int Cx, int H, int W, int coord) {
+    if (B < 1 || Cx < 1 || H < 1 || W < 1) return 0;
+    return (long)B * ((H - 1) / 2 + 1) * ((W - 1) / 2 + 1) * (Cx + (coord ? 3 : 0)) * 9;
+}
+extern "C" int t2v_conv2d_s2_dx_gemm(const float* x, const float* w, const float* dy, float* dx, float* dcol, int B, int Cx, int H, int W,
+                                     int Cout, int coord, void* stream_) {
+    hipStream_t stream = (hipStream_t)stream_;
+    if (!x || !w || !dy || !dx || !dcol || B < 1 || Cx < 1 || H < 1 || W < 1 || Cout < 1) return T2V_ERR_ARG;
+    Conv2dArgs a = conv2d_args(x, w, B, Cx, H, W, Cout, coord);
+    const int K = (Cx + (coord ? 3 : 0)) * 9, P = a.Ho * a.Wo;
+    int rc = t2v_gemm_f32_batched_ex(dy, (long)Cout * P, 0, 1, P, w, 0, 0, 1, K, nullptr, dcol, (long)P * K, K, B, 1, P, K, Cout, stream);
+    if (rc != T2V_OK) return rc;
+    a.y = dx;
+    const size_t n = (size_t)B * Cx * H * W;
+    k_col2im_s2<<<(unsigned)((n + 255) / 256 > 8192 ? 8192 : (n + 255) / 256), 256, 0, stream>>>(a, dcol);
+    return t2v_check_launch();
+}
+extern "C" int t2v_conv2d_s2_dw_gemm_multi(const t2v_conv2d_dw_job* jobs, int njobs, void* stream_) {
+    hipStream_t stream = (hipStream_t)stream_;
+    if (!jobs || njobs < 1 || njobs > DW_MULTI_MAX) return T2V_ERR_ARG;
+    T2vBatchedGemm g[DW_MULTI_MAX];
+    DwReduceMulti m;
+    m.count = njobs;
+    int blocks = 0;
+    for (int p = 0; p < njobs; ++p) {
+        const t2v_conv2d_dw_job& j = jobs[p];
+        if (!j.dy || !j.scratch || !j.dw || j.B < 1 || j.Cx < 1 || j.H < 1 || j.W < 1 || j.Cout < 1) return T2V_ERR_ARG;
+        const int K = (j.Cx + (j.coord ? 3 : 0)) * 9, P = ((j.H - 1) / 2 + 1) * ((j.W - 1) / 2 + 1), Cout = j.Cout;
+        const int ns = conv2d_gemm_chunks(P), chunk = P / ns;
+        float* part = j.scratch + (size_t)j.B * P * K;
+        T2vBatchedGemm& q = g[p];
+        q.A = j.dy; q.sAb = (long)Cout * P; q.sAs = chunk; q.sAi = P; q.sAk = 1;
+        q.B = j.scratch; q.sBb = (long)P * K; q.sBs = (long)chunk * K; q.sBj = 1; q.sBk = K;
+        q.C = part; q.sCb = (long)Cout * K; q.ldc = K;
+        q.nbatch = j.B; q.nsub = ns; q.M = Cout; q.N = K; q.K = chunk;
+        m.part[p] = part; m.dw[p] = j.dw; m.n[p] = Cout * K; m.nsplit[p] = j.B * ns;
+        m.start[p] = blocks;
+        blocks += (Cout * K + 255) / 256;
+    }
+    for (int p = njobs; p <= DW_MULTI_MAX; ++p) m.start[p] = blocks;
+    for (int p = njobs; p < DW_MULTI_MAX; ++p) { m.part[p] = nullptr; m.dw[p] = nullptr; m.n[p] = 0; m.nsplit[p] = 0; }
+    int rc = t2v_gemm_f32_batched_multi(g, njobs, stream);
+    if (rc != T2V_OK) return rc;
+    k_conv2d_s2_dw_reduce_multi<<<blocks, 256, 0, stream>>>(m);
+    return t2v_check_launch();
+}
 
 
 __global__ __launch_bounds__(256) void k_gru_bwd(GruArgs a) {
diff --git a/tacotron2-vae_amd/csrc/t2v_kernels.h b/tacotron2-vae_amd/csrc/t2v_kernels.h
--- a/tacotron2-vae_amd/csrc/t2v_kernels.h
+++ b/tacotron2-vae_amd/csrc/t2v_kernels.h
@@ -12,6 +12,14 @@
 unsigned* t2v_arrival_counters(int n);
 extern unsigned long long* g_t2v_prof;
 const t2v_step_params* t2v_step_for(hipStream_t stream);
+
+struct T2vBatchedGemm {
+    const float* A; long sAb, sAs, sAi, sAk;
+    const float* B; long sBb, sBs, sBj, sBk;
+    float* C; long sCb; int ldc;
+    int nbatch, nsub, M, N, K;
+};
+int t2v_gemm_f32_batched_multi(const T2vBatchedGemm* d, int n, hipStream_t stream);
 
 struct T2VZeroRegions {
     void* p[10];
diff --git a/tacotron2-vae_amd/modules.py b/tacotron2-vae_amd/modules.py
--- a/tacotron2-vae_amd/modules.py
+++ b/tacotron2-vae_amd/modules.py
@@ -35,12 +35,13 @@
         import t2v_hip
         n = inputs.size(0)
         out = inputs.contiguous().view(n, 1, -1, self.n_mels)
+        dw_group = t2v_hip.ConvDwGroup()
         for i, (conv, bn) in enumerate(zip(self.convs, self.bns)):
             c = conv.conv if i == 0 else conv
             if self.training:
                 t2v_hip.note_bn_counter(bn.num_batches_tracked)
             out = t2v_hip.Conv2dBNReLU.apply(out, c.weight, c.bias, bn.weight, bn.bias, bn.running_mean,
-                                             bn.running_var, self.training, i == 0)
+                                             bn.running_var, self.training, i == 0, dw_group)
         t2v_hip.flush_bn_counters()
         out = out.transpose(1, 2)
         out = out.contiguous().view(n, out.size(1), -1)
diff --git a/tacotron2-vae_amd/t2v_hip.py b/tacotron2-vae_amd/t2v_hip.py
--- a/tacotron2-vae_amd/t2v_hip.py
+++ b/tacotron2-vae_amd/t2v_hip.py
@@ -54,6 +54,11 @@
                 ('sBk', C.c_long * 3), ('N', C.c_int * 3), ('C', C.c_void_p * 3), ('ldc', C.c_int * 3)]
 
 
+class _Conv2dDwJob(C.Structure):
+    C_NAME = 't2v_conv2d_dw_job'
+    _fields_ = [('dy', C.c_void_p), ('scratch', C.c_void_p), ('dw', C.c_void_p)] + [(n, C.c_int) for n in ('B', 'Cx', 'H', 'W', 'Cout', 'coord')]
+
+
 class _AchainDw(C.Structure):
     C_NAME = 't2v_achain_dw'
     _fields_ = [('planes', C.c_void_p), ('d_w_ih', C.c_void_p), ('ld_ih', C.c_int), ('d_w_hh', C.c_void_p), ('ld_hh', C.c_int),
@@ -74,7 +79,7 @@
 EXPORTS = ('t2v_version', 't2v_last_error', 't2v_stamp', 't2v_debug_spin', 't2v_pack_lstm_weights', 't2v_pack_lstm_weights_bf16', 't2v_decoder_train_fwd',
            't2v_decoder_train_bwd', 't2v_clip_adam_step', 't2v_clip_adam_step_guarded', 't2v_decoder_replay_fwd_kernels', 't2v_mel_frontend', 't2v_set_phase_profile', 't2v_decoder_infer_steps', 't2v_conv1d_stat_blocks', 't2v_conv1d_stat_blocks_bf16', 't2v_conv1d_fwd', 't2v_conv1d_bwd', 't2v_conv1d_fwd_bf16', 't2v_conv1d_bwd_bf16', 't2v_conv1d_dw_scratch_floats', 't2v_conv1d_flip_weights', 't2v_gemm_bf16', 't2v_gemm_bf16_splitk', 't2v_gemm_bf16_splitk_scratch_floats', 't2v_attn_wgrad', 't2v_attn_wgrad_scratch_floats',
            't2v_bn_act_fwd', 't2v_bn_act_bwd', 't2v_bn_act_bwd_eval', 't2v_bilstm_fwd', 't2v_bilstm_bwd', 't2v_gemm_f32', 't2v_conv2d_s2_fwd', 't2v_conv2d_s2_bwd', 't2v_conv2d_s2_dw_scratch_floats', 't2v_conv2d_s2_fwd_gemm', 't2v_conv2d_s2_bwd_gemm',
-           't2v_conv2d_s2_gemm_scratch_floats',
+           't2v_conv2d_s2_gemm_scratch_floats', 't2v_conv2d_s2_dcol_floats', 't2v_conv2d_s2_dx_gemm', 't2v_conv2d_s2_dw_gemm_multi', 't2v_colsum_multi',
            't2v_gru_fwd', 't2v_gru_bwd', 't2v_loss_fwd_bwd', 't2v_fuse_location_weights', 't2v_decoder_qp_floats',
            't2v_set_step_params', 't2v_set_step_params_stream', 't2v_decoder_replay_bwd_kernels', 't2v_embedding_fwd', 't2v_embedding_bwd', 't2v_gemm_f32_splitk', 't2v_gemm_splitk_scratch_floats', 't2v_gemm_f32_batched',
            't2v_decoder_infer_persistent', 't2v_decoder_persist_supported', 't2v_decoder_persist_scratch_floats',
@@ -191,6 +196,8 @@
     lib.t2v_colsum.argtypes = [C.c_void_p, C.c_long, C.c_long, C.c_long, C.c_void_p, C.c_void_p, C.c_void_p]
     lib.t2v_colsum_scratch_floats.argtypes = [C.c_long, C.c_long]
     lib.t2v_colsum_scratch_floats.restype = C.c_long
+    lib.t2v_colsum_multi.argtypes = [C.POINTER(C.c_void_p), C.POINTER(C.c_long), C.POINTER(C.c_long), C.POINTER(C.c_long),
+                                     C.POINTER(C.c_void_p), C.POINTER(C.c_void_p), C.c_int, C.c_void_p]
     lib.t2v_set_step_params.argtypes = [C.c_void_p]
     lib.t2v_set_step_params.restype = None
     lib.t2v_set_step_params_stream.argtypes = [C.c_void_p, C.c_void_p]
@@ -265,6 +272,10 @@
     lib.t2v_conv2d_s2_gemm_scratch_floats.argtypes = [C.c_int] * 6
     lib.t2v_conv2d_s2_gemm_scratch_floats.restype = C.c_long
     lib.t2v_conv2d_s2_dw_scratch_floats.argtypes = [C.c_int] * 6
+    lib.t2v_conv2d_s2_dcol_floats.argtypes = [C.c_int] * 5
+    lib.t2v_conv2d_s2_dcol_floats.restype = C.c_long
+    lib.t2v_conv2d_s2_dx_gemm.argtypes = [vp, vp, vp, vp, vp, C.c_int, C.c_int, C.c_int, C.c_int, C.c_int, C.c_int, vp]
+    lib.t2v_conv2d_s2_dw_gemm_multi.argtypes = [C.POINTER(_Conv2dDwJob), C.c_int, vp]
     lib.t2v_gru_fwd.argtypes = [vp, vp, vp, vp, vp, vp, vp, C.c_int, C.c_int, vp]
     lib.t2v_gru_bwd.argtypes = [vp, vp, vp, vp, vp, vp, vp, vp, C.c_int, C.c_int, vp]
     lib.t2v_conv2d_s2_fwd_ragged.argtypes = [vp, vp, vp, vp, vp] + [C.c_int] * 7 + [vp]
@@ -1147,7 +1158,11 @@
             _check(lib.t2v_gemm_f32_batched(_p(AL[1:]), T_in, 1, B * T_in, _p(DCTX), E, 1, B * E, _p(d_memory), T_in * E, E, B,
                                             T_in, E, T, _stream()), 't2v_gemm_f32_batched')
             dpre = S
-            d_pm = colsum(dpre.view(T, B * T_in * A)).view(B, T_in, A)
+            if REFENC_BWD_LEGACY:
+                d_pm, bsums = colsum(dpre.view(T, B * T_in * A)).view(B, T_in, A), None
+            else:
+                bsums = colsum_multi([dpre.view(T, B * T_in * A), DGD.view(TB, G4)] + ([DGA.view(TB, G4)] if ctx.pre2 is not None else []))
+                d_pm = bsums.pop(0).view(B, T_in, A)
             dmem_l.append(d_memory); dpm_l.append(d_pm)
             if ctx.pre2 is not None and ctx.needs_input_grad[17] and not ctx.pre_on_side:
                 dpre_l.append(gemm(DGA.view(TB, G4), ctx.wrefs[0].detach()[:, :PRE].t()).view(T, B, PRE))
@@ -1188,7 +1203,8 @@
                 d_loc_dense, d_loc_conv = attn_wgrad(dpre, AL, ACUM, loc_conv, loc_dense, B, T_in, T)
                 parts = [d_wq, d_loc_conv, d_loc_dense, d_v]
                 acc = parts if acc is None else [x + y for x, y in zip(acc, parts)]
-            bparts = [colsum(DGD.view(TB, G4))] + ([colsum(DGA.view(TB, G4))] if ctx.pre2 is not None else [])
+            bparts = bsums if bsums is not None else \
+                [colsum(DGD.view(TB, G4))] + ([colsum(DGA.view(TB, G4))] if ctx.pre2 is not None else [])
             bacc = bparts if bacc is None else [x + y for x, y in zip(bacc, bparts)]
             dga_l.append(DGA)
         ctx.chunks = ctx.prepared = None
@@ -1862,6 +1878,55 @@
     return out
 
 
+def colsum_multi(mats):
+    lib = _require_gpu(*mats)
+    ok = 1 < len(mats) <= 4 and all(x.dim() == 2 and x.dtype == torch.float32 and x.stride(1) == 1 and x.shape[1] % 4 == 0 and
+                                    (x.stride(0) if x.shape[0] > 1 else x.shape[1]) % 4 == 0 and x.data_ptr() % 16 == 0 for x in mats)
+    if not ok:
+        return [colsum(x) for x in mats]
+    n = len(mats)
+    dev = mats[0].device
+    outs = [torch.empty(x.shape[1], device=dev, dtype=torch.float32) for x in mats]
+    nscr = [lib.t2v_colsum_scratch_floats(*x.shape) for x in mats]
+    scrs = [torch.empty(k, device=dev, dtype=torch.float32) if k else None for k in nscr]
+    longs = lambda v: (C.c_long * n)(*v)
+    ptrs = lambda v: (C.c_void_p * n)(*[t.data_ptr() if t is not None else None for t in v])
+    _check(lib.t2v_colsum_multi(ptrs(mats), longs([x.stride(0) if x.shape[0] > 1 else x.shape[1] for x in mats]),
+                                longs([x.shape[0] for x in mats]), longs([x.shape[1] for x in mats]), ptrs(scrs), ptrs(outs), n, _stream()),
+           't2v_colsum_multi')
+    return outs
+
+
+REFENC_BWD_LEGACY = os.environ.get('T2V_REFENC_BWD', '') == 'legacy'
+
+
+class ConvDwGroup(object):
+
+    def __init__(self):
+        self.expect = 0
+        self.jobs = []
+
+    def add(self, dy, gscr, dw_ptr, dw_base, dims):
+        self.jobs.append((dy, gscr, dw_ptr, dw_base, dims))
+        if len(self.jobs) >= self.expect:
+            self.flush()
+
+    def flush(self):
+        jobs, self.jobs = self.jobs, []
+        if not jobs:
+            return
+        lib = load_library()
+        keep = tuple(t for j in jobs for t in (j[0], j[1], j[3]) if t is not None)
+        with side('w', keep=keep):
+            for i in range(0, len(jobs), 8):
+                part = jobs[i:i + 8]
+                arr = (_Conv2dDwJob * len(part))()
+                for a, (dy, gscr, dw_ptr, _, dims) in zip(arr, part):
+                    a.dy, a.scratch, a.dw = dy.data_ptr(), gscr.data_ptr(), dw_ptr
+                    a.B, a.Cx, a.H, a.W, a.Cout, a.coord = dims
+                _check(lib.t2v_conv2d_s2_dw_gemm_multi(arr, len(part), _stream()), 't2v_conv2d_s2_dw_gemm_multi')
+
+
 _GRAD_SLOTS = {}
 
 
@@ -2024,7 +2089,7 @@
 class Conv2dBNReLU(torch.autograd.Function):
 
     @staticmethod
-    def forward(ctx, x, weight, bias, gamma, beta, running_mean, running_var, training, coord):
+    def forward(ctx, x, weight, bias, gamma, beta, running_mean, running_var, training, coord, dw_group=None):
         lib = _require_gpu(x, weight)
         x = _f32c(x)
         B, Cx, Hh, Ww = x.shape
@@ -2049,6 +2114,12 @@
                                   0, 0, 0, _stream()), 't2v_bn_act_fwd')
         ctx.keep = (x, w, y, mean, rstd, gamma, beta)
         ctx.gscr = gscr
+        ctx.dw_group = None
+        if (dw_group is not None and gscr is not None and not REFENC_BWD_LEGACY and any(ctx.needs_input_grad) and
+                weight.is_leaf and weight.requires_grad and w is weight):
+            ctx.dw_group = dw_group
+            dw_group.expect += 1
+        ctx.wparam = weight
         ctx.running = (running_mean, running_var)
         ctx.small = (gamma, beta, bias)
         ctx.cfg = (B, Cx, Hh, Ww, Cout, Ho, Wo, int(coord), bool(training))
@@ -2071,7 +2142,35 @@
                       _p(dbeta), _p(dbias), B, Cout, Ho * Wo, ACT_RELU, 0.0, 0, 0, 0, _stream()), 't2v_bn_act_bwd')
         dx = torch.empty_like(x) if ctx.needs_input_grad[0] else None
         dw = torch.empty_like(w)
-        if ctx.gscr is not None:
+        if ctx.gscr is not None and not REFENC_BWD_LEGACY:
+            dims = (B, Cx, Hh, Ww, Cout, coord)
+            if dx is not None:
+                dcol = torch.empty(lib.t2v_conv2d_s2_dcol_floats(B, Cx, Hh, Ww, coord), **f32)
+                _check(lib.t2v_conv2d_s2_dx_gemm(_p(x), _p(w), _p(dy), _p(dx), _p(dcol), B, Cx, Hh, Ww, Cout, coord, _stream()),
+                       't2v_conv2d_s2_dx_gemm')
+            group = ctx.dw_group
+            if group is not None and ctx.wparam.grad is None:
+                slot = grad_slot(ctx.wparam)
+                base = None
+                if slot is None:
+                    base = torch.empty(w.numel(), **f32)
+                    dw = base.view(w.shape)
+                else:
+                    dw = slot
+                ptr = dw.data_ptr()
+                slot = None
+                group.add(dy, ctx.gscr, ptr, base, dims)
+            else:
+                if group is not None:
+                    group.expect -= 1
+                    if group.jobs and len(group.jobs) >= group.expect:
+                        group.flush()
+                job = (_Conv2dDwJob * 1)()
+                job[0].dy, job[0].scratch, job[0].dw = dy.data_ptr(), ctx.gscr.data_ptr(), dw.data_ptr()
+                job[0].B, job[0].Cx, job[0].H, job[0].W, job[0].Cout, job[0].coord = dims
+                _check(lib.t2v_conv2d_s2_dw_gemm_multi(job, 1, _stream()), 't2v_conv2d_s2_dw_gemm_multi')
+            ctx.gscr = None
+        elif ctx.gscr is not None:
             _check(lib.t2v_conv2d_s2_bwd_gemm(_p(x), _p(w), _p(dy), _p(dx), _p(dw), _p(ctx.gscr), B, Cx, Hh, Ww, Cout, coord,
                                               _stream()), 't2v_conv2d_s2_bwd_gemm')
             ctx.gscr = None
@@ -2080,7 +2179,7 @@
             scr = torch.empty(nscr, **f32) if nscr else None
             _check(lib.t2v_conv2d_s2_bwd(_p(x), _p(w), _p(dy), _p(dx), _p(dw), _p(scr), B, Cx, Hh, Ww, Cout, coord,
                                          _stream()), 't2v_conv2d_s2_bwd')
-        return dx, dw, dbias, dgamma, dbeta, None, None, None, None
+        return dx, dw, dbias, dgamma, dbeta, None, None, None, None, None
 
 
 class GRULast(torch.autograd.Function):
@@ -2106,6 +2205,7 @@
             _err_note('GRU forward', sync[1:2])
             syncs.append(sync)
         ctx.keep = (x2, w_ih, whh, hs, gsave, xchg, syncs)
+        ctx.bias_leaf = b_ih.is_leaf and b_hh.is_leaf
         ctx.dims = (B, T, I)
         return hs[:, T].clone()
 
@@ -2128,7 +2228,11 @@
         with side('w', keep=(dgi, dgh, hs, x2), after=fork):
             hprev = hs[:, :T].reshape(B * T, 256)
             g = (gemm(dgi2.t(), x2.t()), gemm(dgh2.t(), hprev.t()))
-        return (dx,) + g + (colsum(dgi2), colsum(dgh2))
+            if ctx.bias_leaf and not REFENC_BWD_LEGACY:
+                g += (colsum(dgi2), colsum(dgh2))
+        if len(g) == 2:
+            g += (colsum(dgi2), colsum(dgh2))
+        return (dx,) + g
 
 
 def refenc_heights(n_frames, n_layers):
```

Result: no change. 227,000 mel-frames/s (-0.5%).
